# facebookresearch/MidasTouch

Measured on AMD Instinct MI355X. Metric: filter_steps_per_sec, higher is better.
Workload: dtype f64

## Files before the change

### include/midas_hip.h

```cpp
#ifndef MIDAS_HIP_H
#define MIDAS_HIP_H

#include <stdint.h>

#ifdef __cplusplus
extern "C" {
#endif

#define MIDAS_OK 0
#define MIDAS_ERR_INVALID (-1)
#define MIDAS_ERR_HIP (-2)
#define MIDAS_ERR_NOMEM (-3)
#define MIDAS_ERR_NODEVICE (-4)

#define MIDAS_F32 0
#define MIDAS_F64 1

#define MIDAS_RESAMPLE_MULTINOMIAL 0
#define MIDAS_RESAMPLE_SYSTEMATIC 1

typedef struct midas_ctx midas_ctx;
typedef struct midas_codebook midas_codebook;
typedef struct midas_tree midas_tree;

// ... 111 lines not shown
int midas_tsne_knn(midas_ctx* ctx, const void* X_dev, int32_t dtype, int64_t K, int64_t F, int64_t ld, int32_t nan_to_num,
                   int32_t k, int64_t rows_per_panel, int32_t* idx_dev, double* d2_dev);
int midas_tsne_perplexity(midas_ctx* ctx, const float* d2_dev, int64_t K, int32_t k, float perplexity, double* P_dev);
int midas_tsne_gradient(midas_ctx* ctx, int64_t K, const float* y_dev, const int64_t* crow_dev, const int32_t* col_dev,
                        const float* val_dev, float* grad_dev, double* kl_dev);
int midas_tsne_optimize(midas_ctx* ctx, int64_t K, float* y_dev, const int64_t* crow_dev, const int32_t* col_dev,
                        const float* val_dev, int32_t it, int32_t max_iter, double momentum, double learning_rate,
                        int32_t lr_float32, int32_t n_iter_check, int32_t n_iter_without_progress, double min_grad_norm,
                        double* result);

int midas_topn_pose_error(midas_ctx* ctx, int32_t B, int64_t K, const double* scores_dev, int64_t row0, int32_t n,
                          const double* feat_dev, int32_t d, double* err_dev, int32_t* idx_dev);

typedef struct midas_step_args {
    int64_t N;
    const float* poses_in_dev;
    float* poses_prop_dev;
    float* poses_out_dev;
    double* weights_dev;
    double* weights_out_dev;
    const int32_t* hint_in_dev;
    int32_t* nn_idx_dev;
    int32_t* hint_out_dev;
    int32_t* ridx_dev;
    const float* odom16_dev;
    const double* code_dev;
    const float* gt16_dev;
    double* rmse_dev;
    const float* tn_dev;
    const float* rot_dev;
    const double* u_dev;
    float u32;
    float std_t, std_r;
    uint64_t seed, step;
    double prune_thr;
    int32_t softmax;
    int32_t resample_mode;
    int32_t* status_dev;
    uint64_t* telemetry_dev;
    uint32_t* score_stamps_dev;
    uint32_t score_epoch;
} midas_step_args;

int midas_filter_step(midas_ctx* ctx, const midas_codebook* cb, const midas_tree* tree6,
                      const midas_tree* tree3, const midas_step_args* args);


typedef struct midas_lazy_args {
    int64_t N;
    const float* poses_prop_prev_dev;
    const int32_t* nn_idx_prev_dev;
    const int32_t* status_prev_dev;
    float* poses_prop_dev;
    int32_t* nn_idx_dev;
    uint8_t* valid_dev;
    int32_t* status_dev;
    double* tables_dev;
    double* scores_dev;
    double* part_rmse_dev;
    int32_t resample_prev;
    const float* poses_in_dev;
    const int32_t* hint_in_dev;
    int32_t resample_mode;
    const double* u_prev_dev;
    float u32_prev;
    uint64_t step_prev;
    int32_t* ridx_dev;
    const float* odom16_dev;
    const double* code_dev;
    const float* gt16_dev;
    const float* tn_dev;
    const float* rot_dev;
    float std_t, std_r;
    uint64_t seed, step;
    double prune_thr;
    int32_t softmax;
    uint64_t* telemetry_dev;
    uint32_t* score_stamps_dev;
    uint32_t score_epoch;
    double* rmse_dev;
    int32_t* score_list_dev;
    uint8_t* guide_dev;
} midas_lazy_args;
int64_t midas_lazy_guide_bytes(int64_t N);
int midas_lazy_guide_layout(int32_t* bins_out, int32_t* unit_out, int32_t* stride_out);
int midas_lazy_step(midas_ctx* ctx, const midas_codebook* cb, const midas_tree* tree6, const midas_tree* tree3,
                    const midas_lazy_args* args);
int midas_score_list_seed(midas_ctx* ctx, int64_t K, uint32_t* score_stamps_dev, uint32_t score_epoch, int32_t* score_list_dev,
                          int64_t N, const int32_t* nn_idx_dev);
int midas_lazy_run(midas_ctx* ctx, const midas_codebook* cb, const midas_tree* tree6, const midas_tree* tree3,
                   const midas_lazy_args* first, int32_t T, double* rmse_log_dev);

typedef struct midas_estimate_args {
    int64_t N;
    int32_t B;
    const float* poses_prop_dev;
    const double* weights_dev;
    const double* tables_dev;
    const uint8_t* valid_dev;
    int32_t softmax;
    float* centers_dev;
    float* stds_dev;
} midas_estimate_args;
int midas_pose_estimate(midas_ctx* ctx, const midas_estimate_args* args);
int midas_lazy_run_estimate(midas_ctx* ctx, const midas_codebook* cb, const midas_tree* tree6, const midas_tree* tree3,
                            const midas_lazy_args* first, int32_t T, double* rmse_log_dev,
                            float* est_centers_dev, float* est_stds_dev);

typedef struct midas_lazy_flush_args {
    int64_t N;
    const double* tables_dev;
    const uint8_t* valid_dev;
    const int32_t* nn_idx_dev;
    const float* poses_prop_dev;
    int32_t* status_dev;
    const double* part_rmse_dev;
    int32_t softmax, resample_mode;
    const double* u_dev;
    float u32;
    uint64_t seed, step;
    double* weights_dev;
    int32_t* ridx_dev;
    float* poses_out_dev;
    double* weights_out_dev;
    int32_t* hint_out_dev;
    double* rmse_dev;
} midas_lazy_flush_args;
int midas_lazy_flush(midas_ctx* ctx, const midas_lazy_flush_args* args);

int64_t midas_lazy_tables_doubles(int64_t N);
int midas_lazy_step_batch(midas_ctx* ctx, const midas_codebook* cb, const midas_tree* tree6, const midas_tree* tree3,
                          const midas_lazy_args* args, int32_t B);
int midas_lazy_flush_batch(midas_ctx* ctx, const midas_lazy_flush_args* args, int32_t B);


typedef struct midas_shard_front_args {
    int64_t N;
    int64_t slot_base;
    const float* poses_in_dev;
    float* poses_prop_dev;
    const int32_t* hint_in_dev;
    int32_t* nn_idx_dev;
    uint8_t* valid_dev;
    const float* odom16_dev;
    const double* code_dev;
    double* scores_dev;
    int32_t scores_ready;
    const float* gt16_dev;
    double* rmse_sums_dev;
    const float* tn_dev;
    const float* rot_dev;
    float std_t, std_r;
    uint64_t seed, step;
    double prune_thr;
    uint64_t* telemetry_dev;
    int32_t* status_dev;
    double* flags_dev;
    uint32_t* score_stamps_dev;
    uint32_t score_epoch;
} midas_shard_front_args;
int midas_shard_front(midas_ctx* ctx, const midas_codebook* cb, const midas_tree* tree6, const midas_tree* tree3,
                      const midas_shard_front_args* args);
int midas_shard_tail_a(midas_ctx* ctx, int64_t N, const double* scores_dev, const int32_t* nn_idx_dev,
                       const uint8_t* valid_dev, int32_t softmax, double* tables_dev, double* r1_dev, int32_t* status_dev);
typedef struct midas_shard_route_args {
    int64_t N;
// ... 222 lines not shown
```

### midastouch_amd/_lib.py

```python
from __future__ import annotations

import ctypes as C
import sys
import os
import subprocess

_HERE = os.path.dirname(os.path.abspath(__file__))
CSRC = os.path.join(_HERE, "csrc")
LIB_PATH = os.environ.get("MIDAS_HIP_LIB") or os.path.join(CSRC, "libmidas_hip.so")

MIDAS_F32, MIDAS_F64 = 0, 1
RESAMPLE_MULTINOMIAL, RESAMPLE_SYSTEMATIC = 0, 1
PROF_SLOTS = 8


class MidasError(RuntimeError):
    pass


class StepArgs(C.Structure):

    _fields_ = [
        ("N", C.c_int64),
        ("poses_in", C.c_void_p),
# ... 158 lines not shown
        ("unit_weights", C.c_int32), ("telemetry", C.c_void_p),
        ("score_stamps", C.c_void_p), ("score_epoch", C.c_uint32),
        ("host_mirror", C.c_void_p), ("grid_n", C.c_int64), ("anneal_small", C.c_int32), ("topk_ties", C.c_int32),
        ("anneal_frozen", C.c_int32), ("stream_draws", C.c_int32), ("dbscan_batched", C.c_int32),
    ]


LOOP_FRONT, LOOP_DBSCAN, LOOP_ANNEAL, LOOP_RESAMPLE = 1, 2, 4, 8
MT19937_HIST_WORDS = 20560
TOPK_TIES_INDEX, TOPK_TIES_ATEN_CPU = 0, 1
LOOP_MAX_CLUSTERS, LOOP_LOG_DOUBLES = 64, 168
LOOP_BATCH_MAX_CAP = 16384
LOOP_BATCH_WIDE_MAX_CAP = 131072
DBSCAN_BATCH_MAX_POINTS = 1 << 20
(LOOP_I_N, LOOP_I_NSET, LOOP_I_MODE, LOOP_I_K, LOOP_I_INIT, LOOP_I_VARSET, LOOP_I_KEPT, LOOP_I_DRIFT, LOOP_I_STATUS,
 LOOP_I_RAW, LOOP_I_NCL, LOOP_I_NPRES, LOOP_I_FRAME, LOOP_I_NAN, LOOP_I_ERR, LOOP_I_NDRAW) = range(16)
LOOP_ERR_NDRAW = 256
(LOOP_D_S, LOOP_D_VARPREV, LOOP_D_VAR, LOOP_D_RMSE_T, LOOP_D_RMSE_R, LOOP_D_XMAX, LOOP_D_XMIN, LOOP_D_TOTAL) = range(8)

_P, _I32, _I64, _U64, _F, _D = C.c_void_p, C.c_int32, C.c_int64, C.c_uint64, C.c_float, C.c_double
SIGNATURES = {
    "midas_ctx_create": (C.c_int, [C.c_int, _P, C.POINTER(_P)]),
    "midas_ctx_destroy": (C.c_int, [_P]),
    "midas_ctx_set_stream": (C.c_int, [_P, _P]),
    "midas_sync": (C.c_int, [_P]),
    "midas_selftest_wave_sums": (C.c_int, [_P, _P, _P]),
    "midas_scratch_reserve": (C.c_int, [_P, C.c_int64]),
    "midas_strerror": (C.c_char_p, [C.c_int]),
    "midas_last_error": (C.c_char_p, [_P]),
    "midas_version": (C.c_char_p, []),
    "midas_codebook_create": (C.c_int, [_P, _I64, _I32, _P, _I32, C.POINTER(_P)]),
    "midas_codebook_destroy": (C.c_int, [_P]),
    "midas_score": (C.c_int, [_P, _P, _I32, _P, _P]),
    "midas_score_batch": (C.c_int, [_P, _P, _I32, _P, _P]),
    "midas_score_batch_f64": (C.c_int, [_P, _P, _I32, _P, _P]),
    "midas_codebook_set_batch_precision": (C.c_int, [_P, _I32]),
    "midas_se3_feature": (C.c_int, [_P, _I64, _P, _F, _P]),
    "midas_tree_build": (C.c_int, [_P, _I32, _I64, _P, C.POINTER(_P)]),
    "midas_tree_destroy": (C.c_int, [_P]),
    "midas_tree_attach_mesh": (C.c_int, [_P, _P, _P, _P]),
    "midas_nn6": (C.c_int, [_P, _P, _I64, _P, _P, _P, _P]),
    "midas_knn6": (C.c_int, [_P, _P, _I64, _P, C.c_int32, _P, _P]),
    "midas_tree_export": (C.c_int, [_P, _P, C.c_int32, _P, _I64]),
    "midas_nn6_stats": (C.c_int, [_P, _P, _I64, _P, _P, _P, _P]),
    "midas_nn3": (C.c_int, [_P, _P, _I64, _P, _P]),
    "midas_propagate": (C.c_int, [_P, _I64, _P, _P, _P, _P, _P, _F, _F, _U64, _U64]),
    "midas_check_poses": (C.c_int, [_P, _I64, _P, _P, _P]),
    "midas_gather_f64": (C.c_int, [_P, _I64, _P, _P, _P]),
    "midas_softmax": (C.c_int, [_P, _I64, _P, _I32, _P]),
    "midas_prune": (C.c_int, [_P, _I64, _P, _P, _D, _P]),
    "midas_cdf": (C.c_int, [_P, _I64, _P, _P, _P]),
    "midas_score_list_seed": (C.c_int, [_P, _I64, _P, C.c_uint32, _P, _I64, _P]),
    "midas_mt19937_seed": (C.c_int, [_P, _U64, _P]),
    "midas_mt19937_rand64": (C.c_int, [_P, _P, _I64, _I64, _P]),
    "midas_mt19937_rand64_chunked": (C.c_int, [_P, _P, _I64, _I64, _P, _P, _P, _I32]),
    "midas_mt19937_normal32": (C.c_int, [_P, _P, _I64, _I64, _F, _F, _P, _P, _P, _P, _P, _P, _I32]),
    "midas_mt19937_draws": (C.c_int, [_P, _P, _I64, _I32, _P, _P, _P, _P, _P, _P, _I32]),
    "midas_mt19937_draws_batch": (C.c_int, [_P, _I32, _P, _I64, _I32, _P, _P, _P, _P, _P, _P, _I32]),
    "midas_mt19937_draws_counted": (C.c_int, [_P, _P, _I64, _I32, _P, _P, _P, _P, _P]),
    "midas_mt19937_draws_counted_batch": (C.c_int, [_P, _I32, _P, _I64, _I32, _P, _I64, _P, _P, _P, _P, _I64]),
    "midas_resample_search": (C.c_int, [_P, _I64, _P, _I64, _I32, _P, _F, _U64, _U64, _P]),
    "midas_gather_rows": (C.c_int, [_P, _I64, _P, _P, _P, _I32]),
    "midas_rmse": (C.c_int, [_P, _I64, _P, _P, _P]),
    "midas_topn_pose_error": (C.c_int, [_P, _I32, _I64, _P, _I64, _I32, _P, _I32, _P, _P]),
    "midas_selfsim_topn": (C.c_int, [_P, _P, _I32, _P, _I32, _I64, _P, _P]),
    "midas_selfsim_panel": (C.c_int, [_P, _P, _I64, _I64, _P, _I64]),
    "midas_selfsim_topn_f64": (C.c_int, [_P, _P, _I32, _P, _I32, _I64, _P, _P]),
    "midas_selfsim_panel_f64": (C.c_int, [_P, _P, _I64, _I64, _P, _I64]),
    "midas_tsne_knn": (C.c_int, [_P, _P, _I32, _I64, _I64, _I64, _I32, _I32, _I64, _P, _P]),
    "midas_tsne_perplexity": (C.c_int, [_P, _P, _I64, _I32, _F, _P]),
    "midas_tsne_gradient": (C.c_int, [_P, _I64, _P, _P, _P, _P, _P, _P]),
    "midas_tsne_optimize": (C.c_int, [_P, _I64, _P, _P, _P, _P, _I32, _I32, _D, _D, _I32, _I32, _I32, _D, _P]),
    "midas_cluster_centers": (C.c_int, [_P, _I64, _P, _P, _P, _P, _I32, _P, _P, _P, _P]),
    "midas_filter_step": (C.c_int, [_P, _P, _P, _P, C.POINTER(StepArgs)]),
    "midas_filter_step_batch": (C.c_int, [_P, _P, _P, _P, C.POINTER(StepArgs), _I32]),
    "midas_lazy_step": (C.c_int, [_P, _P, _P, _P, C.POINTER(LazyArgs)]),
    "midas_lazy_run": (C.c_int, [_P, _P, _P, _P, C.POINTER(LazyArgs), _I32, _P]),
    "midas_lazy_run_estimate": (C.c_int, [_P, _P, _P, _P, C.POINTER(LazyArgs), _I32, _P, _P, _P]),
    "midas_pose_estimate": (C.c_int, [_P, C.POINTER(EstimateArgs)]),
    "midas_lazy_flush": (C.c_int, [_P, C.POINTER(LazyFlushArgs)]),
    "midas_lazy_tables_doubles": (C.c_int64, [_I64]),
    "midas_lazy_guide_bytes": (C.c_int64, [_I64]),
    "midas_lazy_guide_layout": (C.c_int, [_P, _P, _P]),
    "midas_lazy_step_batch": (C.c_int, [_P, _P, _P, _P, C.POINTER(LazyArgs), _I32]),
    "midas_lazy_flush_batch": (C.c_int, [_P, C.POINTER(LazyFlushArgs), _I32]),
    "midas_loop_step": (C.c_int, [_P, _P, _P, _P, C.POINTER(LoopArgs), _I32]),
    "midas_loop_step_batch": (C.c_int, [_P, _P, _P, _P, C.POINTER(LoopArgs), _I32, _I32, _I64]),
    "midas_loop_step_batch_draws": (C.c_int, [_P, _P, _P, _P, C.POINTER(LoopArgs), _I32, _I32, _I64]),
    "midas_loop_step_batch_wide": (C.c_int, [_P, _P, _P, _P, C.POINTER(LoopArgs), _I32, _I32, _I64]),
    "midas_dbscan": (C.c_int, [_P, _I64, _P, _D, _I64, _P, _P]),
    "midas_dbscan_batch": (C.c_int, [_P, _I32, _I64, _P, _I64, _P, _D, _I64, _P, _P, _I32]),
    "midas_dbscan_points": (C.c_int, [_P, _I64, C.c_int32, _P, _D, _I64, _P, _P]),
    "midas_anneal_select": (C.c_int, [_P, _I64, _P, _I32, _I64, _P]),
    "midas_anneal_select_ties": (C.c_int, [_P, _I64, _P, _I32, _I64, _I32, _P, _P]),
    "midas_shard_front": (C.c_int, [_P, _P, _P, _P, C.POINTER(ShardFrontArgs)]),
    "midas_shard_tail_a": (C.c_int, [_P, _I64, _P, _P, _P, _I32, _P, _P, _P]),
    "midas_shard_tail_fin": (C.c_int, [_P, _I64, _P, _P, _P, _P, _I32, _P, _I32, _I64, _I32, _P, _P]),
    "midas_shard_route_count": (C.c_int, [_P, C.POINTER(ShardRouteArgs)]),
    "midas_shard_route_pack": (C.c_int, [_P, C.POINTER(ShardRouteArgs)]),
    "midas_shard_unpack": (C.c_int, [_P, _I64, _P, _P, _P, _P, _P]),
    "midas_shard_unpack_rows": (C.c_int, [_P, _I64, _P, _I32, _P, _P, _P, _P]),
    "midas_shard_unpack_fixed": (C.c_int, [_P, _I64, _P, _I64, _P, _I32, _I64, _P, _P, _P, _P, _P]),
    "midas_shard_unpack_peer": (C.c_int, [_P, _I64, _P, _P, _P, _P, _P]),
    "midas_comm_unique_id": (C.c_int, [_P, C.c_char_p, _P]),
    "midas_comm_create": (C.c_int, [_P, C.c_char_p, _P, _I32, _I32, C.POINTER(C.c_void_p)]),
    "midas_comm_destroy": (C.c_int, [_P]),
    "midas_comm_all_gather": (C.c_int, [_P, _P, _P, _I64]),
    "midas_shard_step": (C.c_int, [_P, _P, _P, _P, _P, C.POINTER(ShardStepArgs), _I32]),
    "midas_shard_run": (C.c_int, [_P, _P, _P, _P, _P, C.POINTER(ShardStepArgs), _I32]),
    "midas_shard_estimate_moments": (C.c_int, [_P, _I64, _P, _P, _P]),
    "midas_shard_estimate_finish": (C.c_int, [_P, _I64, _P, _P, _P]),
    "midas_shard_step_estimate": (C.c_int, [_P, _P, _P, _P, _P, C.POINTER(ShardStepArgs), _P, _P, _P, _P]),
    "midas_shard_run_estimate": (C.c_int, [_P, _P, _P, _P, _P, C.POINTER(ShardStepArgs), _I32, _P, _P, _P, _P]),
    "midas_peer_alloc": (C.c_int, [_P, _I64, C.POINTER(C.c_void_p), _P]),
    "midas_peer_free": (C.c_int, [_P, _P]),
    "midas_peer_open": (C.c_int, [_P, _P, C.POINTER(C.c_void_p)]),
    "midas_peer_close": (C.c_int, [_P, _P]),
    "midas_peer_probe_write": (C.c_int, [_P, _P, _I32, _I32, _I32]),
    "midas_peer_probe_check": (C.c_int, [_P, _P, _I32, _I32, _P]),
    "midas_tail_resample": (C.c_int, [_P, C.POINTER(TailResampleArgs)]),
    "midas_profile_enable": (C.c_int, [_P, _I32]),
    "midas_profile_read": (C.c_int, [_P, C.POINTER(C.c_double), C.POINTER(_I64), _I32]),
    "midas_profile_slot_name": (C.c_char_p, [_I32]),
}


def build(force: bool = False) -> str:
    srcs = [os.path.join(CSRC, f) for f in os.listdir(CSRC) if f.endswith((".hip", ".hpp"))]
    srcs.append(os.path.join(_HERE, "..", "include", "midas_hip.h"))
    stale = (not os.path.exists(LIB_PATH)) or any(os.path.getmtime(s) > os.path.getmtime(LIB_PATH) for s in srcs)
    if force or stale:
        subprocess.run(["make", "-C", CSRC, "-j4", "-s"] + (["-B"] if force else []), check=True)
    return LIB_PATH


_lib = None


def load():
    global _lib
    if _lib is not None:
        return _lib
    if not os.path.exists(LIB_PATH):
        raise MidasError(
            f"{LIB_PATH} not found: build it with `python -c 'import __graft_entry__ as g; g.build()'` "
            "(hipcc --offload-arch=gfx950). There is no CPU fallback."
        )
    import torch

    try:
        lib = C.CDLL(LIB_PATH)
    except OSError as e:
        raise MidasError(f"cannot load {LIB_PATH}: {e}") from e
    for name, (res, args) in SIGNATURES.items():
        try:
            fn = getattr(lib, name)
        except AttributeError as e:
            raise MidasError(f"{LIB_PATH} does not export {name}") from e
        fn.restype = res
        fn.argtypes = args
    _lib = lib
    return lib


def _ptr(t):
    if t is None:
# ... 79 lines not shown
```

### midastouch_amd/csrc/api.hip

```cpp
#include <cstdio>
#include <cstdlib>
#include <cstring>
#include <new>
#include <vector>

#include "api_entry.hpp"

using namespace midas;

namespace midas {
int tree_build_impl(midas_ctx* ctx, int32_t dim, int64_t K, const void* points_dev, midas_tree* out);
int attach_mesh_impl(midas_ctx* ctx, midas_tree* t6, const midas_tree* t3, const float* cb_poses_dev);
void tree_free_host(midas_tree* t);
}

struct ScratchChunk { void* p; size_t cap; };
struct ScratchState {
    std::vector<ScratchChunk> chunks;
    size_t cur = 0;
    size_t used = 0;
    size_t total = 0;
};
static ScratchState* scratch_of(midas_ctx* ctx) { return reinterpret_cast<ScratchState*>(ctx->scratch); }

// ... 27 lines not shown
    }
    *out = (char*)s->chunks[s->cur].p + s->used;
    s->used += bytes;
    return MIDAS_OK;
}

midas_scratch_pos midas_scratch_mark(midas_ctx* ctx) {
    const ScratchState* s = scratch_of(ctx);
    return {s->cur, s->used, s->total};
}

void midas_scratch_rewind(midas_ctx* ctx, const midas_scratch_pos& pos) {
    ScratchState* s = scratch_of(ctx);
    s->cur = pos.cur; s->used = pos.used; s->total = pos.total;
}

int midas_set_error(midas_ctx* ctx, int code, const char* what, const char* detail) {
    if (ctx) {
        ctx->last_error = std::string(midas_strerror(code)) + ": " + (what ? what : "") + " (" + (detail ? detail : "") + ")";
    }
    return code;
}

namespace midas {
void prof_mark(midas_ctx* ctx, int slot) {
    if (!ctx->prof || !ctx->ev_ready || slot > MIDAS_PROF_SLOTS) return;
    if (ctx->prof_only >= 0 && slot != ctx->prof_only && slot != ctx->prof_only + 1) return;
    (void)hipEventRecord(ctx->ev[slot], ctx->stream);
}
}

static const char* kSlotNames[MIDAS_PROF_SLOTS] = {
    "score_codebook", "particle_update", "tail_a", "tail_b", "", "", "", "event_pair_overhead"};

extern "C" {

MIDAS_EXPORT const char* midas_version(void) { return "midas-hip 0.1 (gfx950)"; }

MIDAS_EXPORT const char* midas_strerror(int code) {
    switch (code) {
        case MIDAS_OK: return "ok";
        case MIDAS_ERR_INVALID: return "invalid argument";
        case MIDAS_ERR_HIP: return "HIP runtime error";
        case MIDAS_ERR_NOMEM: return "out of device memory";
        case MIDAS_ERR_NODEVICE: return "no usable HIP device";
        default: return "unknown error";
    }
}

MIDAS_EXPORT const char* midas_last_error(const midas_ctx* ctx) { return ctx ? ctx->last_error.c_str() : ""; }

MIDAS_EXPORT int midas_ctx_create(int device, void* hip_stream, midas_ctx** out) {
    if (!out) return MIDAS_ERR_INVALID;
    *out = nullptr;
    int count = 0;
    if (hipGetDeviceCount(&count) != hipSuccess || count <= 0 || device < 0 || device >= count) return MIDAS_ERR_NODEVICE;
    if (hipSetDevice(device) != hipSuccess) return MIDAS_ERR_NODEVICE;
    midas_ctx* ctx = new (std::nothrow) midas_ctx();
    if (!ctx) return MIDAS_ERR_NOMEM;
    ctx->device = device;
    ctx->scratch = new (std::nothrow) ScratchState();
    ctx->stream = (hipStream_t)hip_stream;
    ctx->own_stream = false;
    if (const char* ov = getenv("MIDAS_OVERLAP")) ctx->overlap = atoi(ov) != 0;
    const char* lazy = getenv("MIDAS_LAZY_MODULES");
    if (!(lazy && lazy[0] == '1')) {
        int (*const warm[])() = {warm_score, warm_particles, warm_resample, warm_cluster, warm_topn, warm_selfsim, warm_loop,
                                 warm_dbscan, warm_dbscan_nd, warm_index_build, warm_mt19937, warm_topk_aten, warm_score_f64,
                                 warm_selfsim_f64, warm_tsne};
        for (auto w : warm)
            if (w() != 0) { (void)hipGetLastError(); }
    }
    {
        void* p = nullptr;
        const int blocks = midas::TAIL_GROUP_MAX_BLOCKS;
        if (hipMalloc(&p, (size_t)blocks * midas::TAIL_GROUP_BLOCK_BYTES) == hipSuccess && hipMemset(p, 0, (size_t)blocks * midas::TAIL_GROUP_BLOCK_BYTES) == hipSuccess &&
            hipDeviceSynchronize() == hipSuccess) {
            ctx->tail_rec = (unsigned long long*)p;
            ctx->tail_rec_blocks = blocks;
        } else {
            if (p) (void)hipFree(p);
            (void)hipGetLastError();
        }
    }
    *out = ctx;
    return MIDAS_OK;
}

MIDAS_EXPORT int midas_scratch_reserve(midas_ctx* ctx, int64_t bytes) {
    if (!ctx || bytes < 0) return MIDAS_ERR_INVALID;
    MIDAS_HIP_CHECK(ctx, hipSetDevice(ctx->device));
    ScratchState* s = scratch_of(ctx);
    size_t have = 0;
    for (const auto& c : s->chunks) have = c.cap > have ? c.cap : have;
    const size_t want = ((size_t)bytes + 255) & ~(size_t)255;
    if (s->chunks.size() == 1 && have >= want) return MIDAS_OK;
    if (s->chunks.size() >= 1 && have >= want && s->chunks[0].cap == have) return MIDAS_OK;
    MIDAS_HIP_CHECK(ctx, hipStreamSynchronize(ctx->stream));
    if (ctx->side) MIDAS_HIP_CHECK(ctx, hipStreamSynchronize(ctx->side));
    void* p = nullptr;
    const size_t cap = want > have ? want : have;
    if (hipMalloc(&p, cap) != hipSuccess) return midas_set_error(ctx, MIDAS_ERR_NOMEM, "hipMalloc(scratch reserve)", "out of device memory");
    for (auto& c : s->chunks) (void)hipFree(c.p);
    s->chunks.clear();
    s->chunks.push_back({p, cap});
    s->cur = 0; s->used = 0; s->total = 0;
    static const bool log = getenv("MIDAS_SCRATCH_LOG") != nullptr;
    if (log) fprintf(stderr, "[midas] scratch: reserved one chunk of %zu bytes\n", cap);
    return MIDAS_OK;
}

MIDAS_EXPORT int midas_ctx_destroy(midas_ctx* ctx) {
    if (!ctx) return MIDAS_OK;
    (void)hipSetDevice(ctx->device);
    (void)hipStreamSynchronize(ctx->stream);
    ScratchState* s = scratch_of(ctx);
    for (auto& c : s->chunks) (void)hipFree(c.p);
    delete s;
    if (ctx->tail_rec) (void)hipFree(ctx->tail_rec);
    if (ctx->ev_ready)
        for (auto& e : ctx->ev) (void)hipEventDestroy(e);
    if (ctx->own_stream) (void)hipStreamDestroy(ctx->stream);
    if (ctx->side) {
        (void)hipStreamSynchronize(ctx->side);
        (void)hipEventDestroy(ctx->ev_fork);
        (void)hipEventDestroy(ctx->ev_join);
        (void)hipStreamDestroy(ctx->side);
    }
    delete ctx;
    return MIDAS_OK;
}

MIDAS_EXPORT int midas_ctx_set_stream(midas_ctx* ctx, void* hip_stream) {
    if (!ctx) return MIDAS_ERR_INVALID;
    MIDAS_HIP_CHECK(ctx, hipStreamSynchronize(ctx->stream));
    if (ctx->own_stream) {
        (void)hipStreamDestroy(ctx->stream);
        ctx->own_stream = false;
    }
    ctx->stream = (hipStream_t)hip_stream;
    return MIDAS_OK;
}

MIDAS_EXPORT int midas_sync(midas_ctx* ctx) {
    if (!ctx) return MIDAS_ERR_INVALID;
    MIDAS_HIP_CHECK(ctx, hipStreamSynchronize(ctx->stream));
    return MIDAS_OK;
}

MIDAS_EXPORT int midas_codebook_create(midas_ctx* ctx, int64_t K, int32_t D, const void* emb_dev, int32_t dtype,
                                       midas_codebook** out) {
    MIDAS_ENTER(ctx);
    MIDAS_REQUIRE(ctx, out && emb_dev && K > 0 && D > 0 && (dtype == MIDAS_F32 || dtype == MIDAS_F64));
    midas_codebook* cb = new (std::nothrow) midas_codebook();
    if (!cb) return midas_set_error(ctx, MIDAS_ERR_NOMEM, "new midas_codebook", "");
    cb->ctx = ctx; cb->K = K; cb->D = D; cb->dtype = dtype; cb->emb = emb_dev; cb->norms = nullptr;
    if (hipMalloc((void**)&cb->norms, (size_t)K * sizeof(double)) != hipSuccess) {
        delete cb;
        return midas_set_error(ctx, MIDAS_ERR_NOMEM, "hipMalloc(norms)", "");
    }
    int rc = launch_row_norms(ctx, K, D, emb_dev, dtype, cb->norms);
    if (rc) { (void)hipFree(cb->norms); delete cb; return rc; }
    *out = cb;
    return MIDAS_OK;
}

MIDAS_EXPORT int midas_codebook_destroy(midas_codebook* cb) {
    if (!cb) return MIDAS_OK;
    (void)hipStreamSynchronize(cb->ctx->stream);
    (void)hipFree(cb->norms);
    delete cb;
    return MIDAS_OK;
}

MIDAS_EXPORT int midas_score(midas_ctx* ctx, const midas_codebook* cb, int32_t B, const double* codes_dev,
                             double* scores_dev) {
    MIDAS_ENTER(ctx);
    MIDAS_REQUIRE(ctx, cb && B >= 1 && codes_dev && scores_dev);
    return launch_score(ctx, cb, B, codes_dev, scores_dev);
}

MIDAS_EXPORT int midas_score_batch(midas_ctx* ctx, const midas_codebook* cb, int32_t B, const double* codes_dev,
                                   double* scores_dev) {
    MIDAS_ENTER(ctx);
    MIDAS_REQUIRE(ctx, cb && B >= 1 && codes_dev && scores_dev);
    return launch_score_batch(ctx, cb, B, codes_dev, scores_dev);
}

MIDAS_EXPORT int midas_score_batch_f64(midas_ctx* ctx, const midas_codebook* cb, int32_t B, const double* codes_dev,
                                       double* scores_dev) {
    MIDAS_ENTER(ctx);
    MIDAS_REQUIRE(ctx, cb && B >= 1 && codes_dev && scores_dev);
    return launch_score_batch_f64(ctx, cb, B, codes_dev, scores_dev);
}

MIDAS_EXPORT int midas_codebook_set_batch_precision(midas_codebook* cb, int32_t dtype) {
    if (!cb) return MIDAS_ERR_INVALID;
    midas_ctx* ctx = cb->ctx;
    MIDAS_REQUIRE(ctx, dtype == MIDAS_F32 || dtype == MIDAS_F64);
    cb->batch_precision = dtype;
    return MIDAS_OK;
}
// ... 349 lines not shown
```

### midastouch_amd/csrc/api_step.hip

```cpp
#include "api_entry.hpp"

using namespace midas;

static void prof_begin(midas_ctx* ctx) {
    if (!(ctx->prof && ctx->ev_ready)) return;
    (void)hipEventRecord(ctx->ev[6], ctx->stream);
    (void)hipEventRecord(ctx->ev[7], ctx->stream);
}
static int prof_end(midas_ctx* ctx, int lo, int hi, bool skip_slot0) {
    if (!(ctx->prof && ctx->ev_ready)) return MIDAS_OK;
    const int first = ctx->prof_only >= 0 ? ctx->prof_only : lo, last = ctx->prof_only >= 0 ? ctx->prof_only + 1 : hi;
    if (first >= lo && last <= hi) {
        MIDAS_HIP_CHECK(ctx, hipEventSynchronize(ctx->ev[last]));
        for (int i = first; i < last; ++i) {
            float ms = 0.f;
            if (i == 0 && skip_slot0) continue;
            MIDAS_HIP_CHECK(ctx, hipEventElapsedTime(&ms, ctx->ev[i], ctx->ev[i + 1]));
            ctx->prof_ms[i] += (double)ms;
        }
    } else {
        MIDAS_HIP_CHECK(ctx, hipEventSynchronize(ctx->ev[7]));
    }
    float cal = 0.f;
    MIDAS_HIP_CHECK(ctx, hipEventElapsedTime(&cal, ctx->ev[6], ctx->ev[7]));
    ctx->prof_ms[7] += (double)cal;
    ctx->prof_calls += 1;
    return MIDAS_OK;
}

extern "C" {

static int filter_step_impl(midas_ctx* ctx, const midas_codebook* cb, const midas_tree* tree6, const midas_tree* tree3,
                            const midas_step_args* args, int32_t B) {
    MIDAS_REQUIRE(ctx, cb && tree6 && tree3 && args && tree6->dim == 6 && tree3->dim == 3);
    const midas_step_args& s = *args;
    MIDAS_REQUIRE(ctx, s.N > 0 && s.poses_in_dev && s.poses_prop_dev && s.poses_out_dev && s.weights_dev &&
                           s.weights_out_dev && s.nn_idx_dev && s.hint_out_dev && s.ridx_dev && s.odom16_dev &&
                           s.code_dev && s.status_dev);
    MIDAS_REQUIRE(ctx, s.poses_prop_dev != s.poses_in_dev && s.poses_prop_dev != s.poses_out_dev);
    MIDAS_REQUIRE(ctx, (s.tn_dev == nullptr) == (s.rot_dev == nullptr));
    MIDAS_REQUIRE(ctx, tree6->K == cb->K);
    const int64_t N = s.N;
    const int npart = particle_update_blocks(N);
    void *scores, *x, *e, *valid, *pmax, *pmin, *prm = nullptr, *cdf;
    int rc;
    const size_t Bz = (size_t)B;
    if ((rc = midas_scratch(ctx, Bz * cb->K * sizeof(double), &scores))) return rc;
    if ((rc = midas_scratch(ctx, Bz * N * sizeof(double), &x))) return rc;
    if ((rc = midas_scratch(ctx, Bz * N * sizeof(double), &e))) return rc;
    if ((rc = midas_scratch(ctx, Bz * N, &valid))) return rc;
    if ((rc = midas_scratch(ctx, Bz * npart * sizeof(double), &pmax))) return rc;
    if ((rc = midas_scratch(ctx, Bz * npart * sizeof(double), &pmin))) return rc;
    if (s.gt16_dev && s.rmse_dev)
        if ((rc = midas_scratch(ctx, Bz * npart * 2 * sizeof(double), &prm))) return rc;
    if ((rc = midas_scratch(ctx, Bz * N * sizeof(double), &cdf))) return rc;
    void* lp_raw = nullptr;
    const bool mfma = B > 1 && (cb->batch_precision == MIDAS_F64 ||
                                (cb->dtype == MIDAS_F32 && cb->D % 16 == 0 && (uintptr_t)cb->emb % 16 == 0));
    const bool defer_batch = mfma && ctx->overlap;
    if ((B == 1 && ctx->overlap) || defer_batch || (B > 1 && s.score_stamps_dev))
        if ((rc = midas_scratch(ctx, Bz * N * sizeof(double), &lp_raw))) return rc;
    if (defer_batch && !ctx->side) {
        MIDAS_HIP_CHECK(ctx, hipStreamCreateWithFlags(&ctx->side, hipStreamNonBlocking));
        MIDAS_HIP_CHECK(ctx, hipEventCreateWithFlags(&ctx->ev_fork, hipEventDisableTiming));
        MIDAS_HIP_CHECK(ctx, hipEventCreateWithFlags(&ctx->ev_join, hipEventDisableTiming));
    }

    prof_begin(ctx);
    ParticleUpdateArgs pa;
    fill_particle_update(pa, s, tree6, tree3, N, s.poses_in_dev, s.hint_in_dev, (uint8_t*)valid, B == 1 ? s.score_stamps_dev : nullptr,
                         prm ? s.gt16_dev : nullptr, (double*)prm);
    pa.batch = B;
    pa.score_stride = cb->K;
    pa.scores = (const double*)scores;
    pa.x = (double*)x;
    pa.e = (double*)e;
    pa.status_reset = s.status_dev;
    pa.part_max = (double*)pmax;
    pa.part_min = (double*)pmin;
    bool defer = false;
    const bool sparse_batch = B > 1 && s.score_stamps_dev && s.score_epoch && sparse_score_ok(cb, s.code_dev);
    if (sparse_batch) {
        pa.sp.stamps = s.score_stamps_dev; pa.sp.epoch = s.score_epoch;
        pa.sp.emb = (const float*)cb->emb; pa.sp.norms = cb->norms; pa.sp.code = s.code_dev; pa.sp.scores = (double*)scores;
        pa.sp.nj = cb->D / 64;
        pa.scores = nullptr;
        prof_mark(ctx, 1);
        if ((rc = launch_particle_update(ctx, tree6, tree3, pa))) return rc;
        defer = true;
    }
    if (B == 1 && ctx->overlap) {
        prof_mark(ctx, 1);
        if ((rc = launch_frame_front(ctx, tree6, tree3, pa, cb, s.code_dev, (double*)scores, &defer))) return rc;
    }
    if (defer_batch && !sparse_batch) {
        hipStream_t main_stream = ctx->stream;
        MIDAS_HIP_CHECK(ctx, hipEventRecord(ctx->ev_fork, main_stream));
        MIDAS_HIP_CHECK(ctx, hipStreamWaitEvent(ctx->side, ctx->ev_fork, 0));
        ctx->stream = ctx->side;
        rc = launch_score_dense_batch(ctx, cb, B, s.code_dev, (double*)scores);
        ctx->stream = main_stream;
        if (rc) return rc;
        MIDAS_HIP_CHECK(ctx, hipEventRecord(ctx->ev_join, ctx->side));
        prof_mark(ctx, 1);
        pa.scores = nullptr;
        if ((rc = launch_particle_update(ctx, tree6, tree3, pa))) return rc;
        MIDAS_HIP_CHECK(ctx, hipStreamWaitEvent(main_stream, ctx->ev_join, 0));
        defer = true;
    } else if (!defer) {
        prof_mark(ctx, 0);
        if ((rc = mfma ? launch_score_dense_batch(ctx, cb, B, s.code_dev, (double*)scores)
                       : launch_score(ctx, cb, B, s.code_dev, (double*)scores)))
            return rc;
        prof_mark(ctx, 1);
        pa.sp.stamps = nullptr;
        if ((rc = launch_particle_update(ctx, tree6, tree3, pa))) return rc;
    }
    prof_mark(ctx, 2);

    StepTailArgs ta;
    fill_step_tail(ta, s);
    ta.batch = B;
    ta.npart = npart;
    ta.x = defer ? nullptr : (const double*)x;
    ta.scores = (const double*)scores;
    ta.score_stride = cb->K;
    ta.x_raw = (double*)x;
    ta.lp_raw = (double*)lp_raw;
    ta.e = (double*)e;
    ta.valid = (const uint8_t*)valid;
    ta.part_max = (const double*)pmax;
    ta.part_min = (const double*)pmin;
    ta.cdf = (double*)cdf;
    ta.part_rmse = (const double*)prm;
    if ((rc = launch_step_tail(ctx, ta, 2))) return rc;
    return prof_end(ctx, 0, 4, defer);
}

MIDAS_EXPORT int midas_filter_step(midas_ctx* ctx, const midas_codebook* cb, const midas_tree* tree6,
                                   const midas_tree* tree3, const midas_step_args* args) {
    MIDAS_ENTER(ctx);
    return filter_step_impl(ctx, cb, tree6, tree3, args, 1);
}

MIDAS_EXPORT int midas_filter_step_batch(midas_ctx* ctx, const midas_codebook* cb, const midas_tree* tree6,
                                         const midas_tree* tree3, const midas_step_args* args, int32_t B) {
    MIDAS_ENTER(ctx);
    MIDAS_REQUIRE(ctx, B >= 1 && B <= 65535);
    return filter_step_impl(ctx, cb, tree6, tree3, args, B);
}

static int lazy_step_impl(midas_ctx* ctx, const midas_codebook* cb, const midas_tree* tree6, const midas_tree* tree3,
                          const midas_lazy_args& s, double* rmse_out, int32_t B = 1, int64_t tstride = 0) {
    MIDAS_REQUIRE(ctx, s.N > 0 && ceil_div(s.N, SCAN_BLOCK) <= LAZY_MAX_BLOCKS && s.poses_prop_dev && s.nn_idx_dev && s.valid_dev &&
                           s.status_dev && s.tables_dev && (uintptr_t)s.tables_dev % 128 == 0 && s.scores_dev && s.odom16_dev && s.code_dev);
    MIDAS_REQUIRE(ctx, s.resample_prev ? (s.poses_prop_prev_dev && s.nn_idx_prev_dev && s.status_prev_dev &&
                                          s.poses_prop_prev_dev != s.poses_prop_dev && s.nn_idx_prev_dev != s.nn_idx_dev &&
                                          s.status_prev_dev != s.status_dev)
                                       : (s.poses_in_dev && s.poses_in_dev != s.poses_prop_dev));
    MIDAS_REQUIRE(ctx, (s.tn_dev == nullptr) == (s.rot_dev == nullptr));
    MIDAS_REQUIRE(ctx, s.resample_mode == MIDAS_RESAMPLE_MULTINOMIAL || s.resample_mode == MIDAS_RESAMPLE_SYSTEMATIC);
    const int64_t N = s.N;
    TailTables tb = tables_of(s.tables_dev, N);
    if (s.guide_dev && B == 1) {
        MIDAS_REQUIRE(ctx, (uintptr_t)s.guide_dev % 16 == 0);
        tb.guide = reinterpret_cast<guide_t*>(s.guide_dev);
        tb.guide_raw = tb.guide + ceil_div(N, SCAN_BLOCK) * GUIDE_STRIDE;
    }
    ParticleUpdateArgs pa;
    fill_particle_update(pa, s, tree6, tree3, N, s.poses_in_dev, s.hint_in_dev, s.valid_dev, s.score_stamps_dev,
                         (s.gt16_dev && s.part_rmse_dev) ? s.gt16_dev : nullptr, s.part_rmse_dev);
    pa.batch = B;
    pa.score_stride = cb->K;
    pa.scores = nullptr;
    pa.status_reset = s.status_dev;
    ScorePredict predict;
    if (pa.sp.stamps && s.score_list_dev && B == 1 && s.score_epoch >= 2 && N >= SCAN_CHUNK) {
        MIDAS_REQUIRE(ctx, s.score_epoch < MIDAS_EPOCH_LIMIT);
        predict = wire_score_list(pa.sp, s.score_list_dev, cb->K);
    }
    if (s.resample_prev) {
        LazyResample& r = pa.rs;
        r.enabled = true;
        r.e = tb.e; r.x_raw = tb.x_raw; r.lp = tb.lp; r.lp_raw = tb.lp_raw; r.gend = tb.gend; r.gend_raw = tb.gend_raw;
        r.ggend = tb.ggend; r.ggend_raw = tb.ggend_raw;
        r.guide = tb.guide; r.guide_raw = tb.guide_raw;
        r.bsum_e = tb.bsum_e; r.btot = tb.btot; r.btot_raw = tb.btot_raw; r.bmax = tb.bmax; r.bmin = tb.bmin;
        r.poses_prev = s.poses_prop_prev_dev; r.nn_prev = s.nn_idx_prev_dev; r.status_prev = s.status_prev_dev;
        r.ridx_out = s.ridx_dev;
        r.nb = (int)ceil_div(N, SCAN_BLOCK); r.ng = (int)ceil_div(N, SCAN_CHUNK);
        r.softmax = s.softmax; r.mode = s.resample_mode; r.u = s.u_prev_dev; r.u32 = s.u32_prev;
        r.seed = s.seed; r.step = s.step_prev;
        r.tstride = tstride;
    }
    prof_begin(ctx);
    prof_mark(ctx, 1);
    bool launched = false;
    int rc;
    if (B > 1 && !s.resample_prev) {
        MIDAS_REQUIRE(ctx, pa.sp.stamps && sparse_score_ok(cb, s.code_dev));
        pa.sp.emb = (const float*)cb->emb; pa.sp.norms = cb->norms; pa.sp.code = s.code_dev; pa.sp.scores = s.scores_dev; pa.sp.nj = cb->D / 64;
        if ((rc = launch_particle_update(ctx, tree6, tree3, pa))) return rc;
    } else {
        if ((rc = launch_frame_front(ctx, tree6, tree3, pa, cb, s.code_dev, s.scores_dev, &launched))) return rc;
        if (!launched)
            return midas_set_error(ctx, MIDAS_ERR_INVALID, "codebook", B > 1 ? "the pipelined batch step needs a float32 codebook with D in {128,256,512,1024}, score stamps and N <= 262144"
                                                                              : "the pipelined step needs a float32 codebook with D in {128,256,512,1024}");
    }
    prof_mark(ctx, 2);
    if ((rc = launch_tail_a2(ctx, N, s.scores_dev, s.nn_idx_dev, s.valid_dev, s.softmax, tb, s.status_dev, B, cb->K, true,
                             pa.gt16 ? s.part_rmse_dev : nullptr, rmse_out, B > 1 ? tstride : 0, predict.stamps ? &predict : nullptr)))
        return rc;
    prof_mark(ctx, 3);
    return prof_end(ctx, 1, 3, false);
}

MIDAS_EXPORT int midas_lazy_step(midas_ctx* ctx, const midas_codebook* cb, const midas_tree* tree6, const midas_tree* tree3,
                                 const midas_lazy_args* args) {
    MIDAS_ENTER(ctx);
    MIDAS_REQUIRE(ctx, cb && tree6 && tree3 && args && tree6->dim == 6 && tree3->dim == 3 && tree6->K == cb->K);
    return lazy_step_impl(ctx, cb, tree6, tree3, *args, (args->gt16_dev && args->part_rmse_dev) ? args->rmse_dev : nullptr);
}

static int pose_estimate_impl(midas_ctx* ctx, const midas_estimate_args& s) {
    MIDAS_REQUIRE(ctx, s.N > 0 && s.B >= 1 && s.B <= 65535 && s.poses_prop_dev && s.centers_dev && s.stds_dev &&
                           (uintptr_t)s.poses_prop_dev % 16 == 0);
    MIDAS_REQUIRE(ctx, (s.weights_dev == nullptr) != (s.tables_dev == nullptr));
    if (s.weights_dev)
        return launch_pose_estimate(ctx, s.N, s.B, s.poses_prop_dev, s.weights_dev, nullptr, 0, nullptr, s.softmax, s.centers_dev,
                                    s.stds_dev);
    MIDAS_REQUIRE(ctx, s.valid_dev && (uintptr_t)s.tables_dev % 128 == 0 && ceil_div(s.N, SCAN_BLOCK) <= LAZY_MAX_BLOCKS);
    const TailTables tb = tables_of(const_cast<double*>(s.tables_dev), s.N);
    return launch_pose_estimate(ctx, s.N, s.B, s.poses_prop_dev, nullptr, &tb, tables_doubles(s.N), s.valid_dev, s.softmax,
                                s.centers_dev, s.stds_dev);
}

MIDAS_EXPORT int midas_pose_estimate(midas_ctx* ctx, const midas_estimate_args* args) {
    MIDAS_ENTER(ctx);
    MIDAS_REQUIRE(ctx, args != nullptr);
    return pose_estimate_impl(ctx, *args);
}

static int lazy_run_impl(midas_ctx* ctx, const midas_codebook* cb, const midas_tree* tree6, const midas_tree* tree3,
                         const midas_lazy_args* first, int32_t T, double* rmse_log_dev, float* est_centers, float* est_stds) {
    MIDAS_REQUIRE(ctx, cb && tree6 && tree3 && first && tree6->dim == 6 && tree3->dim == 3 && tree6->K == cb->K && T >= 1);
    MIDAS_REQUIRE(ctx, first->poses_prop_prev_dev && first->nn_idx_prev_dev && first->status_prev_dev && !first->tn_dev &&
                           !first->rot_dev && !first->u_prev_dev);
    MIDAS_REQUIRE(ctx, !rmse_log_dev || (first->gt16_dev && first->part_rmse_dev));
    midas_lazy_args a = *first;
    if (a.score_stamps_dev) {
        const uint64_t inc = a.score_list_dev ? 2u : 1u;
        MIDAS_REQUIRE(ctx, (uint64_t)a.score_epoch + inc * (uint64_t)(T - 1) < (a.score_list_dev ? (uint64_t)MIDAS_EPOCH_LIMIT : 0xFFFFFFF0ull));
    }
    for (int32_t f = 0; f < T; ++f) {
        int rc = f ? scratch_reset(ctx) : MIDAS_OK;
        if (rc) return rc;
        rc = lazy_step_impl(ctx, cb, tree6, tree3, a, rmse_log_dev ? rmse_log_dev + 3 * f : nullptr);
        if (rc) return rc;
        if (est_centers) {
            midas_estimate_args e;
            e.N = a.N; e.B = 1; e.poses_prop_dev = a.poses_prop_dev; e.weights_dev = nullptr; e.tables_dev = a.tables_dev;
            e.valid_dev = a.valid_dev; e.softmax = a.softmax;
            e.centers_dev = est_centers + 16 * (size_t)f; e.stds_dev = est_stds + 3 * (size_t)f;
            if ((rc = pose_estimate_impl(ctx, e))) return rc;
        }
        float* pp = const_cast<float*>(a.poses_prop_prev_dev);
        int32_t* np = const_cast<int32_t*>(a.nn_idx_prev_dev);
        int32_t* sp = const_cast<int32_t*>(a.status_prev_dev);
        a.poses_prop_prev_dev = a.poses_prop_dev; a.nn_idx_prev_dev = a.nn_idx_dev; a.status_prev_dev = a.status_dev;
        a.poses_prop_dev = pp; a.nn_idx_dev = np; a.status_dev = sp;
        a.resample_prev = 1;
        a.u32_prev = -1.0f;
        a.step_prev = a.step;
        a.step += 1;
        if (a.score_stamps_dev) {
            a.score_epoch += a.score_list_dev ? 2u : 1u;
        }
        a.odom16_dev += 16;
        a.code_dev += cb->D;
        if (a.gt16_dev) a.gt16_dev += 16;
    }
    return MIDAS_OK;
}

MIDAS_EXPORT int midas_lazy_run(midas_ctx* ctx, const midas_codebook* cb, const midas_tree* tree6, const midas_tree* tree3,
                                const midas_lazy_args* first, int32_t T, double* rmse_log_dev) {
    MIDAS_ENTER(ctx);
    return lazy_run_impl(ctx, cb, tree6, tree3, first, T, rmse_log_dev, nullptr, nullptr);
}

MIDAS_EXPORT int midas_lazy_run_estimate(midas_ctx* ctx, const midas_codebook* cb, const midas_tree* tree6, const midas_tree* tree3,
                                         const midas_lazy_args* first, int32_t T, double* rmse_log_dev, float* est_centers_dev,
                                         float* est_stds_dev) {
    MIDAS_ENTER(ctx);
    MIDAS_REQUIRE(ctx, est_centers_dev && est_stds_dev);
    return lazy_run_impl(ctx, cb, tree6, tree3, first, T, rmse_log_dev, est_centers_dev, est_stds_dev);
}

static int lazy_flush_impl(midas_ctx* ctx, const midas_lazy_flush_args& s, int32_t B, int64_t tstride) {
    MIDAS_REQUIRE(ctx, s.N > 0 && s.tables_dev && s.valid_dev && s.nn_idx_dev && s.poses_prop_dev && s.status_dev && s.weights_dev &&
                           s.ridx_dev && s.poses_out_dev && s.weights_out_dev && s.hint_out_dev && s.poses_out_dev != s.poses_prop_dev);
    MIDAS_REQUIRE(ctx, s.resample_mode == MIDAS_RESAMPLE_MULTINOMIAL || s.resample_mode == MIDAS_RESAMPLE_SYSTEMATIC);
    const TailTables tb = tables_of(const_cast<double*>(s.tables_dev), s.N);
    StepTailArgs ta;
    fill_step_tail(ta, s);
    ta.batch = B;
    ta.tstride = B > 1 ? tstride : 0;
    ta.npart = 0;
    ta.x = nullptr; ta.e = nullptr; ta.cdf = nullptr; ta.part_max = nullptr; ta.part_min = nullptr;
    ta.valid = s.valid_dev;
    ta.part_rmse = (s.part_rmse_dev && s.rmse_dev) ? s.part_rmse_dev : nullptr;
    return launch_tail_b2(ctx, ta, tb);
}

MIDAS_EXPORT int midas_lazy_flush(midas_ctx* ctx, const midas_lazy_flush_args* args) {
    MIDAS_ENTER(ctx);
    MIDAS_REQUIRE(ctx, args != nullptr);
    return lazy_flush_impl(ctx, *args, 1, 0);
}

MIDAS_EXPORT int midas_score_list_seed(midas_ctx* ctx, int64_t K, uint32_t* score_stamps_dev, uint32_t score_epoch, int32_t* score_list_dev,
                                       int64_t N, const int32_t* nn_idx_dev) {
    MIDAS_ENTER(ctx);
    MIDAS_REQUIRE(ctx, K > 0 && score_stamps_dev && score_epoch >= 2 && score_epoch < MIDAS_EPOCH_LIMIT && score_list_dev && N > 0 && nn_idx_dev);
    return launch_predict_seed(ctx, N, nn_idx_dev, next_score_list(score_stamps_dev, score_epoch, score_list_dev, K));
}

MIDAS_EXPORT int64_t midas_lazy_tables_doubles(int64_t N) { return N > 0 ? tables_doubles(N) : 0; }
MIDAS_EXPORT int midas_lazy_guide_layout(int32_t* bins_out, int32_t* unit_out, int32_t* stride_out) {
    if (bins_out) *bins_out = GUIDE_BINS;
    if (unit_out) *unit_out = GUIDE_UNIT;
    if (stride_out) *stride_out = GUIDE_STRIDE;
    return MIDAS_OK;
}
MIDAS_EXPORT int64_t midas_lazy_guide_bytes(int64_t N) { return N > 0 ? 2 * ceil_div(N, SCAN_BLOCK) * (int64_t)GUIDE_STRIDE * (int64_t)sizeof(guide_t) : 0; }

MIDAS_EXPORT int midas_lazy_step_batch(midas_ctx* ctx, const midas_codebook* cb, const midas_tree* tree6, const midas_tree* tree3,
                                       const midas_lazy_args* args, int32_t B) {
    MIDAS_ENTER(ctx);
    MIDAS_REQUIRE(ctx, cb && tree6 && tree3 && args && tree6->dim == 6 && tree3->dim == 3 && tree6->K == cb->K && B >= 1);
    MIDAS_REQUIRE(ctx, args->score_stamps_dev && args->score_epoch && ceil_div(args->N, SCAN_BLOCK) <= 64 && args->N >= SCAN_CHUNK);
    return lazy_step_impl(ctx, cb, tree6, tree3, *args, (args->gt16_dev && args->part_rmse_dev) ? args->rmse_dev : nullptr, B,
                          tables_doubles(args->N));
}

MIDAS_EXPORT int midas_lazy_flush_batch(midas_ctx* ctx, const midas_lazy_flush_args* args, int32_t B) {
    MIDAS_ENTER(ctx);
    MIDAS_REQUIRE(ctx, args != nullptr && B >= 1);
    return lazy_flush_impl(ctx, *args, B, tables_doubles(args->N));
}

}
```

### midastouch_amd/csrc/front.hip

```cpp
#include "front_wave.hpp"

namespace midas {

template <bool STATS>
__global__ __launch_bounds__(64) void k_particle_update(TreeView<Kd6> t6, TreeView<Kd3> t3, ParticleUpdateArgs a) {
    __shared__ double s_cd[KD_MAX_LEVELS * 64];
    particle_update_wave<false, false, false, STATS, false, true>(t6, t3, a, blockIdx.x, gridDim.x, blockIdx.y, s_cd);
}

int launch_particle_update(midas_ctx* ctx, const midas_tree* t6, const midas_tree* t3, const ParticleUpdateArgs& a_in) {
    if (a_in.N == 0) return MIDAS_OK;
    ParticleUpdateArgs a = a_in;
    static const int ablate = getenv("MIDAS_ABLATE") ? atoi(getenv("MIDAS_ABLATE")) : 0;
    a.ablate = ablate;
    const dim3 grid((unsigned)particle_update_blocks(a.N), (unsigned)(a.batch > 1 ? a.batch : 1));
    if (ablate) hipLaunchKernelGGL(k_particle_update<true>, grid, dim3(64), 0, ctx->stream, view_of<Kd6>(t6), view_of<Kd3>(t3), a);
    else hipLaunchKernelGGL(k_particle_update<false>, grid, dim3(64), 0, ctx->stream, view_of<Kd6>(t6), view_of<Kd3>(t3), a);
    MIDAS_HIP_CHECK(ctx, hipGetLastError());
    return MIDAS_OK;
}


MD void particle_front_wave(ParticleUpdateArgs a, int64_t wave, const double* rs_lds, PuFeat* __restrict__ feat) {
    const int lane = threadIdx.x & 63;
// ... 188 lines not shown
        hits |= dpp_u32<DPP_XOR1>(hits); stops |= dpp_u32<DPP_XOR1>(stops);
        if (LPP == 4) { hits |= dpp_u32<DPP_XOR2>(hits); stops |= dpp_u32<DPP_XOR2>(stops); }
        if (live && mv < 0 && (hits | stops)) {
            const int fh = hits ? __builtin_ctz(hits) : 32, fs = stops ? __builtin_ctz(stops) : 32;
            mv = fh < fs ? 1 : 0;
        }
        mesh_coop(a.vlist, nn, q3, a.t2, lim, owner && live && mv < 0, mv);
    }
    double bestd = a.t2;
    int64_t vi = 0;
    const bool fb3 = owner && live && mv < 0;
    bool ok = wave_search<Kd3, true>(t3, q3, bestd, vi, fb3, s_cd[w]);
    if (a.telemetry) {
        const unsigned long long m = __ballot(fb3);
        if (lane == 0 && m) atomicAdd(&a.telemetry[1], (unsigned long long)__popcll(m));
    }
    if (mv >= 0) ok = mv == 1;
    if (owner && live) {
        a.nn_idx[p] = nn;
        a.valid[p] = ok ? 1 : 0;
    }
}

template <int LPP>
__global__ __launch_bounds__(256, MIDAS_NNP_OCC) void k_particle_nn_prune(TreeView<Kd6> t6, TreeView<Kd3> t3, ParticleUpdateArgs a,
                                                                          const PuFeat* __restrict__ feat) {
    particle_nn_prune_wg<LPP>(t6, t3, a, feat);
}

__global__ __launch_bounds__(256, MIDAS_NNP_OCC) void k_front_small(TreeView<Kd6> t6, TreeView<Kd3> t3, ParticleUpdateArgs a, int nwaves,
                                                                    PuFeat* __restrict__ feat) {
    if (blockIdx.y) {
        const int64_t b = blockIdx.y, o = b * a.N;
        a.n_live += b * LOOP_CTL_I;
        a.poses_in += o * 16; a.poses_prop += o * 16; a.odom16 += b * 16;
        if (a.hint_in) a.hint_in += o;
        a.nn_idx += o; a.valid += o;
        if (a.gt16) { a.gt16 += b * 16; a.part_rmse += 2 * b * nwaves; }
        a.sp.stamps += b * a.score_stride; a.sp.scores += b * a.score_stride; a.sp.code += b * (int64_t)(a.sp.nj * 64);
        a.seed += (uint64_t)b;
        if (a.tn) { a.tn += o * 3; a.rot += o * 3; }
        feat += o;
    }
    if (threadIdx.x < 64 && (int)blockIdx.x < nwaves) particle_front_wave(a, (int64_t)blockIdx.x, nullptr, feat);
    __syncthreads();
    particle_nn_prune_wg<4>(t6, t3, a, feat);
}

template <int NJ, bool LAZY>
static void launch_front_a(const FrontLaunch& L, PuFeat* feat) {
    hipLaunchKernelGGL((k_frame_front_a<float, NJ, LAZY>), L.grid, dim3(256), 0, L.ctx->stream, L.a, L.n_pu, L.nwaves, feat,
                       (const float*)L.cb->emb, L.cb->norms, L.code, L.scores, L.cb->K);
}

bool launch_front_plain(const FrontLaunch& L, const FrontForm& f) {
    return launch_if_form<0, 1, true, true>(L, f) || launch_if_form<0, 1, true, false>(L, f) || launch_if_form<0, 4, true, false>(L, f) ||
           launch_if_form<0, 1, true, false, true>(L, f);
}

int launch_frame_front(midas_ctx* ctx, const midas_tree* t6, const midas_tree* t3, const ParticleUpdateArgs& a_in,
                       const midas_codebook* cb, const double* code, double* scores, bool* launched) {
    *launched = false;
    if (a_in.N == 0 || cb->dtype != MIDAS_F32) return MIDAS_OK;
    if (a_in.batch > 1 && !(a_in.rs.enabled && a_in.rs.nb <= LAZY_WAVE_LD && a_in.sp.stamps)) return MIDAS_OK;
    if ((uintptr_t)cb->emb % 16 != 0 || (uintptr_t)code % 16 != 0) return MIDAS_OK;
    if (cb->D != 512 && cb->D != 256 && cb->D != 128 && cb->D != 1024) return MIDAS_OK;
    ParticleUpdateArgs a = a_in;
    static const int ablate = getenv("MIDAS_ABLATE") ? atoi(getenv("MIDAS_ABLATE")) : 0;
    a.ablate = ablate;
    a.scores = nullptr;
    const int nwaves = particle_update_blocks(a.N), n_pu = (nwaves + 3) / 4;
    if (a.sp.stamps) {
        a.sp.emb = (const float*)cb->emb; a.sp.norms = cb->norms; a.sp.code = code; a.sp.scores = scores; a.sp.nj = cb->D / 64;
    }
    static const int list_wgs_env = getenv("MIDAS_LIST_WAVES") ? atoi(getenv("MIDAS_LIST_WAVES")) : 1024;
    const bool use_list = a.sp.stamps && a.sp.list && a.batch <= 1 && list_wgs_env > 0;
    const char* dense_env = getenv("MIDAS_DENSE_ROWS");
    a.sp.K = cb->K;
    a.sp.dense_thr = use_list && dense_env ? atoi(dense_env) : 0;
    const unsigned grid = (unsigned)(n_pu + (a.sp.stamps ? 0 : ceil_div(cb->K, 16)));
    static const int split_env = getenv("MIDAS_SPLIT_FRONT") ? atoi(getenv("MIDAS_SPLIT_FRONT")) : 1;
    const bool split_front = a.batch <= 1 && !a.inbox.rows && (split_env >= 2 || (split_env == 1 && ((a.rs.enabled && a.N <= 512) || (!a.rs.enabled && a.N <= 2048) || (a.n_live && a.N <= 16384))));
    const int lpp = split_env == 3 ? 2 : 4;
    if (split_front && !(a.ablate & 7)) {
        a.sp.pred_tag = 0; a.sp.list = nullptr;
        void* feat;
        int rc = midas_scratch(ctx, (size_t)a.N * sizeof(PuFeat), &feat);
        if (rc) return rc;
        static const bool small_env = !(getenv("MIDAS_FRONT_SMALL") && atoi(getenv("MIDAS_FRONT_SMALL")) == 0);
        if (small_env && !a.rs.enabled && a.sp.stamps && lpp == 4) {
            hipLaunchKernelGGL(k_front_small, dim3((unsigned)ceil_div(a.N, 64)), dim3(256), 0, ctx->stream, view_of<Kd6>(t6), view_of<Kd3>(t3),
                               a, nwaves, (PuFeat*)feat);
        } else {
            const FrontLaunch L{ctx, t6, t3, a, cb, code, scores, dim3(grid), n_pu, nwaves};
            with_nj(cb->D, [&](auto nj) {
                if (a.rs.enabled) launch_front_a<decltype(nj)::value, true>(L, (PuFeat*)feat);
                else launch_front_a<decltype(nj)::value, false>(L, (PuFeat*)feat);
            });
            if (lpp == 4)
                hipLaunchKernelGGL(k_particle_nn_prune<4>, dim3((unsigned)ceil_div(a.N, 64)), dim3(256), 0, ctx->stream,
                                   view_of<Kd6>(t6), view_of<Kd3>(t3), a, (const PuFeat*)feat);
            else
                hipLaunchKernelGGL(k_particle_nn_prune<2>, dim3((unsigned)ceil_div(a.N, 128)), dim3(256), 0, ctx->stream,
                                   view_of<Kd6>(t6), view_of<Kd3>(t3), a, (const PuFeat*)feat);
        }
        MIDAS_HIP_CHECK(ctx, hipGetLastError());
        *launched = true;
        return MIDAS_OK;
    }
    static const int fw_env = getenv("MIDAS_FRONT_WAVES") ? atoi(getenv("MIDAS_FRONT_WAVES")) : 0;
    static const int wt_env = getenv("MIDAS_WAVE_TABLES") ? atoi(getenv("MIDAS_WAVE_TABLES")) : 1;
    const bool wave_tables = a.rs.enabled && a.rs.nb <= LAZY_WAVE_LD && wt_env != 0;
    const int fw = a.batch > 1 ? 1 : (a.rs.enabled && !wave_tables) ? 4 : fw_env == 1 || fw_env == 4 ? fw_env : (a.sp.stamps ? 1 : 4);
    const int n_pu_fw = (nwaves + fw - 1) / fw;
    if (!use_list) { a.sp.pred_tag = 0; a.sp.list = nullptr; }
    static const int presort_env = getenv("MIDAS_PRESORT") ? atoi(getenv("MIDAS_PRESORT")) : 1;
    if (wave_tables && fw == 1 && a.batch > 1 && !a.inbox.rows && !a.ablate && !a.n_live && presort_env != 0) {
        const int rc = launch_presort(ctx, a);
        if (rc) return rc;
    }
    const unsigned grid_fw = (unsigned)(n_pu_fw + (a.sp.stamps ? (use_list ? (list_wgs_env + fw - 1) / fw : 0) : ceil_div(cb->K, 4 * fw * MIDAS_SCORE_ROUNDS)));
    static const bool pref_env = !(getenv("MIDAS_PREF_PLAIN") && getenv("MIDAS_PREF_PLAIN")[0] == '0');
    const bool pref_plain = pref_env && !a.inbox.rows;
    const bool small_set = fw == 1 && a.N <= 131072;
    FrontForm form;
    if (a.batch > 1) form = {2, 1, false, false, false};
    else if (!a.rs.enabled) form = {0, fw, true, small_set && pref_plain, false};
    else if (!wave_tables) form = {1, 4, true, false, false};
    else form = {2, fw, true, small_set, false};
    if (a.ablate && cb->D == 512 && fw == 1 && (a.batch > 1 || !a.rs.enabled || form.pref)) {
        form.stats = true;
        if (!a.rs.enabled) form.pref = false;
    }
    const FrontLaunch L{ctx, t6, t3, a, cb, code, scores, dim3(grid_fw, (unsigned)(a.batch > 1 ? a.batch : 1)), n_pu_fw, nwaves};
    if (!(launch_front_batch(L, form) || launch_front_plain(L, form) || launch_front_folded(L, form)))
        return midas_set_error(ctx, MIDAS_ERR_INVALID, "launch_frame_front", "no kernel for this form of the front");
    MIDAS_HIP_CHECK(ctx, hipGetLastError());
    *launched = true;
    return MIDAS_OK;
}

int launch_front_small_batch(midas_ctx* ctx, const midas_tree* t6, const midas_tree* t3, const ParticleUpdateArgs& a_in,
                             const midas_codebook* cb, const double* code, double* scores, int32_t B, bool wide) {
    ParticleUpdateArgs a = a_in;
    if (!(a.n_live && a.N > 0 && (a.N <= 16384 || (wide && a.N <= MIDAS_LOOP_BATCH_WIDE_MAX_CAP)) && a.sp.stamps && !a.rs.enabled && cb->dtype == MIDAS_F32 &&
          (cb->D == 512 || cb->D == 256 || cb->D == 128 || cb->D == 1024) && (uintptr_t)cb->emb % 16 == 0 && (uintptr_t)code % 16 == 0))
        return midas_set_error(ctx, MIDAS_ERR_INVALID, "launch_front_small_batch", "no small-set front for these arguments");
    a.scores = nullptr;
    a.sp.emb = (const float*)cb->emb; a.sp.norms = cb->norms; a.sp.code = code; a.sp.scores = scores; a.sp.nj = cb->D / 64;
    a.sp.K = cb->K; a.sp.pred_tag = 0; a.sp.list = nullptr;
    a.score_stride = cb->K;
    a.batch = B;
    const int nwaves = particle_update_blocks(a.N);
    void* feat;
    const int rc = midas_scratch(ctx, (size_t)B * a.N * sizeof(PuFeat), &feat);
    if (rc) return rc;
    hipLaunchKernelGGL(k_front_small, dim3((unsigned)ceil_div(a.N, 64), (unsigned)B), dim3(256), 0, ctx->stream, view_of<Kd6>(t6),
                       view_of<Kd3>(t3), a, nwaves, (PuFeat*)feat);
    MIDAS_HIP_CHECK(ctx, hipGetLastError());
    return MIDAS_OK;
}

__global__ __launch_bounds__(256) void k_reduce_partials(int np, const double* __restrict__ pmax,
                                                         const double* __restrict__ pmin, const double* __restrict__ prm,
                                                         double* __restrict__ extrema2, double* __restrict__ rmse_sums2) {
    __shared__ double s0[4], s1[4], s2[4], s3[4];
    double a = -INFINITY, b = INFINITY, p = 0.0, q = 0.0;
    bool nan = false;
    for (int i = threadIdx.x; i < np; i += 256) {
        if (pmax) {
            double u = pmax[i], v = pmin[i];
            nan |= (u != u) || (v != v);
            a = u > a ? u : a;
            b = v < b ? v : b;
        }
        if (prm) { p += prm[2 * i]; q += prm[2 * i + 1]; }
    }
    a = wave_max(a);
    b = wave_min(b);
    p = wave_sum(p);
    q = wave_sum(q);
    const bool wnan = __any(nan);
    if ((threadIdx.x & 63) == 0) {
        const int w = threadIdx.x >> 6;
        s0[w] = wnan ? NAN : a; s1[w] = wnan ? NAN : b; s2[w] = p; s3[w] = q;
    }
    __syncthreads();
    if (threadIdx.x == 0) {
        bool bad = false;
        for (int i = 0; i < 4; ++i) {
            bad |= s0[i] != s0[i];
            a = s0[i] > a ? s0[i] : a;
            b = s1[i] < b ? s1[i] : b;
        }
        if (extrema2) {
            extrema2[0] = bad ? NAN : a;
            extrema2[1] = bad ? NAN : b;
        }
        if (rmse_sums2) {
            rmse_sums2[0] = (s2[0] + s2[1]) + (s2[2] + s2[3]);
            rmse_sums2[1] = (s3[0] + s3[1]) + (s3[2] + s3[3]);
        }
    }
}

int launch_reduce_partials(midas_ctx* ctx, int np, const double* pmax, const double* pmin, const double* prm,
                           double* extrema2, double* rmse_sums2) {
    hipLaunchKernelGGL(k_reduce_partials, dim3(1), dim3(256), 0, ctx->stream, np, pmax, pmin, prm, extrema2, rmse_sums2);
    MIDAS_HIP_CHECK(ctx, hipGetLastError());
    return MIDAS_OK;
}

// ... 4 lines not shown
```

### midastouch_amd/csrc/front_folded.hip

```cpp
#define MIDAS_FRONT_CLOCKS
#include "front_wave.hpp"

namespace midas {

bool launch_front_folded(const FrontLaunch& L, const FrontForm& f) {
    return launch_if_form<1, 4, true, false>(L, f) || launch_if_form<2, 1, true, true>(L, f) || launch_if_form<2, 1, true, false>(L, f) ||
           launch_if_form<2, 4, true, false>(L, f) || launch_if_form<2, 1, true, true, true>(L, f);
}

#if defined(MIDAS_DEBUG_CLOCKS)
int debug_ff_clocks(long long* io8192, int reset) {
    if (reset) {
        static long long zero[16384];
        return hipMemcpyToSymbol(HIP_SYMBOL(g_ff_clk), zero, sizeof(zero)) == hipSuccess ? 0 : 1;
    }
    return hipMemcpyFromSymbol(io8192, HIP_SYMBOL(g_ff_clk), 16384 * sizeof(long long)) == hipSuccess ? 0 : 1;
}
#endif
MIDAS_WARM_TU(front_folded, (k_frame_front<float, 8, 2, 1, true, true>))

}
```

### midastouch_amd/csrc/front_wave.hpp

```cpp
#pragma once
#include <type_traits>

#include "midas_internal.hpp"
#include "midas_math.hpp"
#include "score_body.hpp"
#include "peer_row.hpp"
#include "resample_search.hpp"
#include "list_scan.hpp"
#include "pose.hpp"

namespace midas {

#ifndef MIDAS_SCORE_ROUNDS
#define MIDAS_SCORE_ROUNDS 2
#endif
#ifndef MIDAS_CLAIM_HASH
#define MIDAS_CLAIM_HASH 1
#endif

constexpr int LAZY_WG_W = 3 * LAZY_MAX_BLOCKS + 8, LAZY_WG_LDS = 4 * LAZY_MAX_BLOCKS + 8;
MD void lazy_tables(const LazyResample& rs, double* rs_lds) {
    __shared__ double s_ex[12];
    const int t = threadIdx.x;
    const int b = t < rs.nb ? t : rs.nb - 1;
    const double bt = rs.btot[b], btr = rs.btot_raw[b], bs = rs.bsum_e[b], bx = rs.bmax[b], bn = rs.bmin[b];
    const int32_t status = rs.status_prev[0];
    const bool in = t < rs.nb;
    double mx = in ? bx : -INFINITY, mn = in ? bn : INFINITY;
    const bool nan = in && ((bx != bx) || (bn != bn));
    mx = wave_max_dpp(mx);
    mn = wave_min_dpp(mn);
    const bool wn = __any(nan);
    if ((t & 63) == 0) { s_ex[t >> 6] = mx; s_ex[4 + (t >> 6)] = mn; s_ex[8 + (t >> 6)] = wn ? 1.0 : 0.0; }
    __syncthreads();
    mx = s_ex[0]; mn = s_ex[4];
    double f = s_ex[8];
    for (int w = 1; w < 4; ++w) { mx = s_ex[w] > mx ? s_ex[w] : mx; mn = s_ex[4 + w] < mn ? s_ex[4 + w] : mn; f += s_ex[8 + w]; }
    if (f != 0.0) { mx = NAN; mn = NAN; }
    const bool apply = rs.softmax && !(__builtin_fabs(mx - mn) <= ISCLOSE_ATOL);
    double* s_bp = rs_lds;
    double* s_w = rs_lds + 256;
    double* s_se = rs_lds + 516;
    if (in) { s_w[t] = apply ? bt : btr; s_se[t] = bs; }
    __syncthreads();
    if (t == 0) {
        double acc = 0.0, S = 0.0;
        for (int i = 0; i < rs.nb; ++i) { s_bp[i] = acc; acc = acc + s_w[i]; S = S + s_se[i]; }
        rs_lds[512] = acc;
        rs_lds[513] = apply ? S : 1.0;
        rs_lds[514] = apply ? 1.0 : 0.0;
        rs_lds[515] = status != 0 ? 1.0 : 0.0;
    }
    __syncthreads();
    const double total = rs_lds[512];
    const double wb = in ? s_w[t] : 0.0;
    __syncthreads();
    if (in) rs_lds[LAZY_WG_W + t] = wb;
    if (in) s_w[t] = (t == rs.nb - 1) ? 1.0 : (s_bp[t] + wb) / total;
    __syncthreads();
}

constexpr int LAZY_WAVE_LD = 64, LAZY_WAVE_LDS = 3 * LAZY_WAVE_LD + 4;
struct LazyRecords { double bt, btr, bx, bn; int32_t status; };
MD LazyRecords lazy_records_load(const LazyResample& rs) {
    const int lane = threadIdx.x & 63;
    const int b = lane < rs.nb ? lane : rs.nb - 1;
    LazyRecords r;
    r.bt = rs.btot[b]; r.btr = rs.btot_raw[b]; r.bx = rs.bmax[b]; r.bn = rs.bmin[b];
    r.status = rs.status_prev[0];
    return r;
}
MD void lazy_tables_wave(const LazyResample& rs, const LazyRecords& r, double* rs_lds) {
    const int lane = threadIdx.x & 63;
    const bool in = lane < rs.nb;
    double mx = in ? r.bx : -INFINITY, mn = in ? r.bn : INFINITY;
    const bool nan = in && ((r.bx != r.bx) || (r.bn != r.bn));
    mx = wave_max_dpp(mx);
    mn = wave_min_dpp(mn);
    if (__any(nan)) { mx = NAN; mn = NAN; }
    const bool apply = rs.softmax && !(__builtin_fabs(mx - mn) <= ISCLOSE_ATOL);
    const double w = in ? (apply ? r.bt : r.btr) : 0.0;
    double* s_wb = rs_lds + 2 * LAZY_WAVE_LD + 4;
    s_wb[lane] = w;
    __builtin_amdgcn_fence(__ATOMIC_RELEASE, "wavefront");
    __builtin_amdgcn_wave_barrier();
    __builtin_amdgcn_fence(__ATOMIC_ACQUIRE, "wavefront");
    double acc = 0.0, bp = 0.0;
    for (int i0 = 0; i0 < rs.nb; i0 += 8) {
        double wv[8];
        const double2* p2 = reinterpret_cast<const double2*>(s_wb + i0);
#pragma unroll
        for (int j = 0; j < 4; ++j) { const double2 t = p2[j]; wv[2 * j] = t.x; wv[2 * j + 1] = t.y; }
#pragma unroll
        for (int j = 0; j < 8; ++j) {
            bp = lane == i0 + j ? acc : bp;
            acc = acc + wv[j];
        }
    }
    const double total = acc;
    if (in) {
        rs_lds[lane] = bp;
        rs_lds[LAZY_WAVE_LD + lane] = (lane == rs.nb - 1) ? 1.0 : (bp + w) / total;
    }
    if (lane == 0) {
        rs_lds[2 * LAZY_WAVE_LD] = total;
        rs_lds[2 * LAZY_WAVE_LD + 2] = apply ? 1.0 : 0.0;
        rs_lds[2 * LAZY_WAVE_LD + 3] = r.status != 0 ? 1.0 : 0.0;
    }
    __builtin_amdgcn_fence(__ATOMIC_RELEASE, "wavefront");
    __builtin_amdgcn_wave_barrier();
    __builtin_amdgcn_fence(__ATOMIC_ACQUIRE, "wavefront");
}

template <typename GT = const double*, typename LT = const double*, typename MID = NoMid>
MD int64_t lazy_source(const LazyResample& rs, const double* rs_lds, int64_t n, int64_t N, int ld = 256, GT gend_lds = nullptr,
                       LT lp_lds = nullptr, MID mid = MID()) {
    const double* s_bp = rs_lds;
    const double* s_end = rs_lds + ld;
    const double total = rs_lds[2 * ld];
    const bool apply = rs_lds[2 * ld + 2] != 0.0;
    const bool bad_total = !(total == total) || total == 0.0;
    if (rs_lds[2 * ld + 3] != 0.0 || bad_total) return n;
    const double* __restrict__ lp = apply ? rs.lp : rs.lp_raw;
    const double* __restrict__ gend = apply ? rs.gend : rs.gend_raw;
    double tq;
    bool upper;
    if (rs.mode == MIDAS_RESAMPLE_MULTINOMIAL) {
        tq = rs.u ? rs.u[n] : philox_uniform53((uint64_t)(n + rs.key_base), rs.seed, rs.step);
        upper = false;
    } else {
        const float r = rs.u32 >= 0.0f ? rs.u32 : philox_uniform24(rs.seed + (uint64_t)rs.traj, rs.step);
        const float off = r / (float)N;
        tq = (double)n / (double)N + (double)off;
        tq = tq >= 1.0 ? tq - 1.0 : tq;
        upper = true;
    }
    auto left_exact = [&](double c) { return upper ? (c <= tq) : (c < tq); };
    int lo = 0, hi = rs.nb;
    while (hi > lo) {
        const int mid = lo + ((hi - lo) >> 1);
        if (left_exact(s_end[mid])) lo = mid + 1; else hi = mid;
    }
    if (lo >= rs.nb) return N - 1;
    if constexpr (__is_same(LT, lds_cdp)) {
        return search_in_block_t<lds_cdp, GT>(lp_lds, gend, apply ? rs.ggend : rs.ggend_raw, lo, N, N - 1, s_bp[lo], total, tq, upper, gend_lds);
    } else {
        const guide_t* guide = apply ? rs.guide : rs.guide_raw;
        return search_in_block_t<const double*, GT, MID>(lp, gend, apply ? rs.ggend : rs.ggend_raw, lo, N, N - 1, s_bp[lo], total, tq, upper, gend_lds,
                                                         guide, guide ? rs_lds[(ld == LAZY_WAVE_LD ? 2 * LAZY_WAVE_LD + 4 : LAZY_WG_W) + lo] : 0.0, mid);
    }
}

template <bool WT = false, bool SCREEN = false, bool PREF = false, bool STATS = false, bool PRES = false, bool NANPART = false>
MD void particle_update_wave(const TreeView<Kd6>& t6, const TreeView<Kd3>& t3, ParticleUpdateArgs a, int64_t wave,
                             int nwaves, int traj, double* s_cd, double* rs_lds = nullptr) {
    const int lane = threadIdx.x & 63;
    if (a.n_live) {
        const int64_t nl = *a.n_live;
        a.N = nl < a.N ? nl : a.N;
        if (wave * 64 >= a.N && wave != 0) return;
    }
    if (traj) {
        const int64_t b = traj, o = b * a.N;
        a.poses_in += o * 16; a.poses_prop += o * 16; a.odom16 += b * 16;
        if (a.tn) { a.tn += o * 3; a.rot += o * 3; }
        if (a.hint_in) a.hint_in += o;
        a.nn_idx += o; a.valid += o;
        if (a.scores) { a.scores += b * a.score_stride; a.x += o; a.e += o; a.part_max += b * nwaves; a.part_min += b * nwaves; }
        if (a.gt16) { a.gt16 += b * 16; a.part_rmse += 2 * b * nwaves; }
        if (a.status_reset) a.status_reset += 2 * b;
        if (a.sp.stamps) {
            a.sp.stamps += b * a.score_stride; a.sp.scores += b * a.score_stride; a.sp.code += b * (int64_t)(a.sp.nj * 64);
        }
        a.slot_base += o;
        if (a.rs.enabled) {
            const int64_t ts = b * a.rs.tstride;
            a.rs.e += ts; a.rs.x_raw += ts; a.rs.lp += ts; a.rs.lp_raw += ts; a.rs.gend += ts; a.rs.gend_raw += ts;
            a.rs.ggend += ts; a.rs.ggend_raw += ts; a.rs.bsum_e += ts; a.rs.btot += ts; a.rs.btot_raw += ts; a.rs.bmax += ts; a.rs.bmin += ts;
            a.rs.poses_prev += o * 16; a.rs.nn_prev += o; a.rs.status_prev += 2 * b;
            if (a.rs.ridx_out) a.rs.ridx_out += o;
            if (a.rs.u) a.rs.u += o;
            a.rs.key_base = o;
            a.rs.traj = traj;
        }
        if (a.pre_order) { a.pre_order += o; a.pre_src += o; if (a.pre_rmse_terms) a.pre_rmse_terms += 2 * o; }
    }
    const bool presorted = PRES && a.pre_order != nullptr;
    const int64_t rank = wave * 64 + lane;
    const bool live = rank < a.N;
    int64_t n = rank;
    int32_t src_pre = 0;
    if (presorted) {
        n = a.pre_order[live ? rank : 0];
        src_pre = a.pre_src[live ? rank : 0];
    }
    if (wave == 0 && lane == 0) {
        if (a.status_reset) { a.status_reset[0] = 0; a.status_reset[1] = 0; }
        if (a.flags_reset) { a.flags_reset[0] = 0.0; a.flags_reset[1] = 0.0; }
        if (a.sp.next_count) *a.sp.next_count = 0;
    }
    unsigned long long st_nn = 0, st_mesh = 0, st_scan = 0;
    int st_rows = 0;
    const bool dense_scores = scores_dense(a.sp);
    const int ablate = STATS ? a.ablate : 0;
    long long tc[10];
    long long tp[4] = {0, 0, 0, 0};
#define MIDAS_TICK(i) do { if (STATS) tc[i] = clock64(); } while (0)
#define MIDAS_PTICK(i) do { if (STATS) tp[i] = clock64(); } while (0)
    MIDAS_TICK(0);
    const long long wall0 = STATS ? wall_clock64() : 0;
    double x = 0.0, et2 = 0.0, ang2 = 0.0;
    float R[16], f[6] = {0.f, 0.f, 0.f, 0.f, 0.f, 0.f};
#pragma unroll
    for (int i = 0; i < 16; ++i) R[i] = 0.f;
    int64_t src = n;
    float NO[16];
    if (WT) {
        float O[16];
#pragma unroll
        for (int i = 0; i < 16; ++i) O[i] = a.odom16[i];
        __builtin_amdgcn_sched_barrier(0);
        LazyRecords rec;
        if (!presorted) rec = lazy_records_load(a.rs);
        __builtin_amdgcn_sched_barrier(0);
        float tnv[3] = {0.f, 0.f, 0.f}, rotv[3] = {0.f, 0.f, 0.f};
        bool no_done = false;
        if (live) noise_draws(n, n + a.slot_base, a.tn, a.rot, a.std_t, a.std_r, a.seed, a.step, tnv, rotv);
        if (!presorted) lazy_tables_wave(a.rs, rec, rs_lds);
        MIDAS_PTICK(0);
        auto mid = [&]() { noise_apply(O, tnv, rotv, NO); no_done = true; };
        if (rs_lds && live && !presorted && !(ablate & 8)) {
            src = lazy_source(a.rs, rs_lds, n, a.N, LAZY_WAVE_LD, (const double*)nullptr, (const double*)nullptr, mid);
            if (a.rs.ridx_out) a.rs.ridx_out[n] = (int32_t)src;
        }
        if (live && !no_done) mid();
        MIDAS_PTICK(1);
    }
    if (rs_lds && live) {
        if (presorted) {
            src = src_pre;
        } else if (!WT) {
            src = (ablate & 8) ? n : lazy_source(a.rs, rs_lds, n, a.N, 256);
            if (a.rs.ridx_out) a.rs.ridx_out[n] = (int32_t)src;
        }
    }
    const float* pose_src = rs_lds ? a.rs.poses_prev : a.poses_in;
    const bool from_inbox = !WT && a.inbox.rows != nullptr;
    PeerRow row;
    if (from_inbox && live) row = peer_row_load(a.inbox.rows, n);
    const int32_t hint = !live ? -1 : from_inbox ? (int32_t)(row.head[1] & 0xFFFFFFFFull) : rs_lds ? a.rs.nn_prev[src] : a.hint_in ? a.hint_in[n] : -1;
    if (live) {
        float P[16];
        if (from_inbox) {
#pragma unroll
            for (int k = 0; k < 8; ++k) {
                P[2 * k] = __int_as_float((int)(row.pose[k] & 0xFFFFFFFFull));
                P[2 * k + 1] = __int_as_float((int)(row.pose[k] >> 32));
            }
        } else {
            load_pose(pose_src + src * 16, P);
        }
        if (WT) {
            mat4_mul(P, NO, R);
            MIDAS_PTICK(2);
        } else {
            float O[16];
#pragma unroll
            for (int i = 0; i < 16; ++i) O[i] = a.odom16[i];
            propagate_one(n, n + a.slot_base, P, O, a.tn, a.rot, a.std_t, a.std_r, a.seed, a.step, R);
        }
        store_pose(a.poses_prop + n * 16, R);
        se3_feature(R, 0.99f, 0.01f, f);
    }
    const float tq_f[3] = {R[3], R[7], R[11]};
    const FieldProbe probe = field_fetch(a.field, tq_f, live && !(ablate & 2));
    MIDAS_TICK(1);
    int32_t bi = 0;
    float bd;
    if (ablate & 1) {
        bi = hint < 0 ? 0 : hint;
    } else {
        int nscan = 0;
        const bool fb = nn6_wave<false, SCREEN>(t6, f, live, hint, bi, bd, reinterpret_cast<float*>(s_cd), nullptr, nullptr, STATS ? &nscan : nullptr,
                                                STATS ? &tc[2] : nullptr);
        MIDAS_TICK(3);
        if (a.telemetry && (ablate & 4)) {
            st_nn = __ballot(live && nscan >= NN_SOLO - 1);
            st_scan = (unsigned long long)wave_sum((double)nscan);
        }
        if (a.telemetry) {
            const unsigned long long m = __ballot(fb);
            if (lane == 0 && m) atomicAdd(&a.telemetry[0], (unsigned long long)__popcll(m));
        }
    }
    constexpr bool PRE = PREF;
    int mv = live ? field_decide(a.field, probe, a.thr) : -1;
    const bool lists_needed = __ballot(live && mv < 0) != 0;
    MeshScr pre[PRE ? 1 + MESH_BATCH : 1];
    if (PRE && a.vscr != nullptr && lists_needed) {
        const MeshScr* vs = a.vscr + (size_t)(live ? bi : 0) * MESH_REC;
#pragma unroll
        for (int j = 0; j < (PRE ? 1 + MESH_BATCH : 1); ++j) pre[j] = vs[j];
    }
    RowClaim claim{false, 0u};
    if (a.sp.stamps && !(ablate & 16)) {
        claim = claim_rows_issue(a.sp, live, bi, MIDAS_CLAIM_HASH ? reinterpret_cast<int*>(s_cd) : nullptr);
        st_rows = score_claimed_rows_nj(a.sp, claim, bi, dense_scores);
    }
    MIDAS_TICK(9);
    double q3[3] = {(double)R[3], (double)R[7], (double)R[11]};
    double best = a.t2;
    int64_t vi = 0;
    if (ablate & 2) mv = 1;
    else if (a.vlist && lists_needed) {
        double lim_lane = 0.0;
        const bool open = live && mv < 0;
        if (a.vscr) {
            const float tqf[3] = {R[3], R[7], R[11]};
// ... 5 lines not shown
            mv = mesh_list_check<false>(a.vlist, bi, q3, a.t2, a.thr, MESH_SOLO, &lim_lane);
        }
        MIDAS_TICK(4);
        if (a.telemetry && (ablate & 4)) st_mesh = __ballot(live && mv < 0);
        mesh_coop(a.vlist, bi, q3, a.t2, lim_lane, live && mv < 0, mv);
    }
    MIDAS_TICK(5);
    bool ok = wave_search<Kd3, true>(t3, q3, best, vi, live && mv < 0, s_cd);
    if (a.telemetry) {
        const unsigned long long m = __ballot(live && mv < 0);
        if (lane == 0 && m) atomicAdd(&a.telemetry[1], (unsigned long long)__popcll(m));
    }
    if (mv >= 0) ok = mv == 1;
    if (a.telemetry && st_rows && lane == 0) atomicAdd(&a.telemetry[2], (unsigned long long)st_rows);
    MIDAS_TICK(6);
    if (live) {
        a.nn_idx[n] = bi;
        if (a.scores) {
            x = a.scores[bi];
            a.x[n] = x;
            a.e[n] = exp_spec(x - 1.0);
        }
        a.valid[n] = ok ? 1 : 0;
        if (a.gt16) {
            float G[16];
#pragma unroll
            for (int i = 0; i < 16; ++i) G[i] = a.gt16[i];
            rmse_terms(R, G, et2, ang2);
        }
    }
    MIDAS_TICK(7);
    const double NEG = -INFINITY, POS = INFINITY;
    if (a.scores) {
        double mx = wave_max(live ? x : NEG), mn = wave_min(live ? x : POS);
        if (NANPART && __any(live && x != x)) { mx = NAN; mn = NAN; }
        if (lane == 0) { a.part_max[wave] = mx; a.part_min[wave] = mn; }
    }
    if (a.gt16) {
        if (presorted && a.pre_rmse_terms) {
            if (live) reinterpret_cast<double2*>(a.pre_rmse_terms)[n] = make_double2(et2, ang2);
        } else {
            et2 = wave_sum(et2);
            ang2 = wave_sum(ang2);
            if (lane == 0) { a.part_rmse[2 * wave] = et2; a.part_rmse[2 * wave + 1] = ang2; }
        }
    }
    if (STATS && a.telemetry && (ablate & 4) && lane == 0) {
        tc[8] = clock64();
        unsigned long long* w = a.telemetry + 16 + 16 * ((size_t)traj * nwaves + wave);
        w[0] += (unsigned long long)st_rows;
        w[1] = (unsigned long long)wall0;
        w[2] += (unsigned long long)__popcll(st_nn); w[4] += st_nn ? 1 : 0;
        w[3] += (unsigned long long)__popcll(st_mesh); w[5] += st_mesh ? 1 : 0;
        w[6] += st_scan;
        w[7] += (unsigned long long)(wall_clock64() - wall0);
#pragma unroll
        for (int i = 0; i < 8; ++i) {
            long long d = i == 3 ? tc[9] - tc[3] : i == 4 ? tc[5] - tc[9] : tc[i + 1] - tc[i];
            if ((ablate & 128) && i >= 4) d = !tp[0] ? 0 : i == 4 ? tp[0] - tc[0] : i == 5 ? tp[1] - tp[0] : i == 6 ? tp[2] - tp[1] : tc[1] - tp[2];
            w[8 + i] += (unsigned long long)d;
        }
    }
#undef MIDAS_TICK
#undef MIDAS_PTICK
}

#ifndef MIDAS_FRONT_OCC
#define MIDAS_FRONT_OCC 1
#endif
#ifndef MIDAS_FRONT4_OCC
#define MIDAS_FRONT4_OCC 4
#endif
#ifndef MIDAS_BATCH_OCC
#define MIDAS_BATCH_OCC 1
#endif
#if defined(MIDAS_DEBUG_CLOCKS) && defined(MIDAS_FRONT_CLOCKS)
__device__ long long g_ff_clk[16384];
#define FF_T0 const long long ff_t0_ = wall_clock64()
#define FF_END do { if (threadIdx.x == 0 && blockIdx.x < 4096) { long long* c_ = g_ff_clk + (a.step & 1) * 8192; c_[2 * blockIdx.x] = ff_t0_; c_[2 * blockIdx.x + 1] = wall_clock64(); } } while (0)
#else
#define FF_T0 do { } while (0)
#define FF_END do { } while (0)
#endif
template <typename T, int NJ, int LAZY, int FW, bool SCR = true, bool PREF = false, bool STATS = false>
__global__ __launch_bounds__(64 * FW, (!SCR && FW == 1) ? MIDAS_BATCH_OCC : (FW == 4 && LAZY == 1) ? MIDAS_FRONT4_OCC : MIDAS_FRONT_OCC) void k_frame_front(TreeView<Kd6> t6, TreeView<Kd3> t3, ParticleUpdateArgs a,
                                                         int n_pu, int nwaves, const T* __restrict__ emb,
                                                         const double* __restrict__ norms, const double* __restrict__ code,
                                                         double* __restrict__ scores, int64_t K) {
    static_assert(LAZY != 1 || FW == 4, "the workgroup-level tables take 256 threads");
    FF_T0;
    __shared__ double s_cd[FW][KD_MAX_LEVELS * 64];
    __shared__ alignas(16) double s_rs[LAZY == 1 ? LAZY_WG_LDS : LAZY == 2 ? FW * LAZY_WAVE_LDS : 8];
    const int w = threadIdx.x >> 6;
    const unsigned bx = blockIdx.x, by = blockIdx.y;
    if ((int)bx < n_pu) {
        if (LAZY == 1) lazy_tables(a.rs, s_rs);
        const int64_t wave = (int64_t)bx * FW + w;
        if (wave < nwaves) {
            constexpr bool SCREEN = FW == 1 && MIDAS_SCREEN && SCR;
            const int traj = (int)by;
            if (LAZY == 2) particle_update_wave<true, SCREEN, PREF, STATS, !SCR && !STATS>(t6, t3, a, wave, nwaves, traj, s_cd[w], s_rs + w * LAZY_WAVE_LDS);
            else particle_update_wave<false, SCREEN, PREF, STATS>(t6, t3, a, wave, nwaves, traj, s_cd[w], LAZY ? s_rs : nullptr);
        }
    } else if (a.sp.list) {
        if ((int)bx == n_pu && threadIdx.x == 0 && a.telemetry) {
            const int c = *a.sp.list_count;
            if (a.sp.dense_thr > 0 && c > a.sp.dense_thr) atomicAdd(&a.telemetry[3], (unsigned long long)a.sp.K);
            else if (c > 0) atomicAdd(&a.telemetry[3], (unsigned long long)(c < a.sp.list_cap ? c : a.sp.list_cap));
        }
        if (!(STATS && (a.ablate & 64)))
            score_list_wave<NJ>(a.sp, (int)(bx - n_pu) * FW + w, ((int)gridDim.x - n_pu) * FW);
    } else {
        const int64_t w0 = ((int64_t)(bx - n_pu) * FW + w) * MIDAS_SCORE_ROUNDS;
        if (w0 * 4 < K) score_wave_multi<T, NJ, MIDAS_SCORE_ROUNDS>(emb, norms, code, scores, K, w0);
    }
    FF_END;
}

struct alignas(16) PuFeat { float f[6]; int32_t hint; int32_t pad; };
static_assert(sizeof(PuFeat) == 32, "two 16-byte pieces per particle");

template <class F>
void with_nj(int32_t D, F&& f) {
    switch (D) {
        case 512: f(std::integral_constant<int, 8>()); break;
        case 256: f(std::integral_constant<int, 4>()); break;
        case 128: f(std::integral_constant<int, 2>()); break;
        default: f(std::integral_constant<int, 16>()); break;
    }
}
template <int NJ, int LAZY, int FW, bool SCR, bool PREF, bool STATS>
void launch_front_kernel(const FrontLaunch& L) {
    hipLaunchKernelGGL((k_frame_front<float, NJ, LAZY, FW, SCR, PREF, STATS>), L.grid, dim3(64 * FW), 0, L.ctx->stream, view_of<Kd6>(L.t6),
                       view_of<Kd3>(L.t3), L.a, L.n_pu, L.nwaves, (const float*)L.cb->emb, L.cb->norms, L.code, L.scores, L.cb->K);
}
template <int LAZY, int FW, bool SCR, bool PREF, bool STATS = false>
bool launch_if_form(const FrontLaunch& L, const FrontForm& f) {
    if (f.lazy != LAZY || f.fw != FW || f.scr != SCR || f.pref != PREF || f.stats != STATS) return false;
    if constexpr (STATS) launch_front_kernel<8, LAZY, FW, SCR, PREF, true>(L);
    else with_nj(L.cb->D, [&](auto nj) { launch_front_kernel<decltype(nj)::value, LAZY, FW, SCR, PREF, false>(L); });
    return true;
}

}
```

### midastouch_amd/csrc/midas_internal.hpp

```cpp
#pragma once
#include <hip/hip_runtime.h>
#include <stdint.h>

#include <cmath>
#include <string>

#include "../../include/midas_hip.h"

namespace midas {

struct alignas(16) Box6 { float lo[6], hi[6]; };
struct alignas(16) Point6 { float c[6]; int32_t idx; int32_t pad; };
struct alignas(16) Box3 { double lo[3], hi[3]; };
struct alignas(16) Point3 { double c[3]; int64_t idx; };

struct Kd6 {
    using T = float;
    using Box = Box6;
    using Point = Point6;
    static constexpr int DIM = 6;
};
struct Kd3 {
    using T = double;
    using Box = Box3;
    using Point = Point3;
    static constexpr int DIM = 3;
};

constexpr int LEAF_CAP = 16;
constexpr int KD_MAX_LEVELS = 10;

struct alignas(16) Nbr6 { float c[6]; int32_t idx; float rho; };
#ifndef MIDAS_NBR_M
#define MIDAS_NBR_M 512
#endif
constexpr int NBR_M = MIDAS_NBR_M;
constexpr int NBR_REC = NBR_M + 1;

struct alignas(16) MeshRec { double c[3]; float rho; int32_t pad; };
struct alignas(16) MeshScr { float c[3]; float rho; };
constexpr int MESH_M = 256;
constexpr int MESH_REC = MESH_M + 1;

struct MeshField {
    const float* d = nullptr;
    float lo[3] = {0.f, 0.f, 0.f};
    float h = 0.f, inv_h = 0.f;
    int32_t n[3] = {0, 0, 0};
    float expand = 0.f;
};

template <class KD>
struct TreeView {
    const typename KD::Box* boxes;
    const typename KD::Point* pts;
    const int32_t* inv_perm;
    const Nbr6* nbrs;
    const float* rho_out;
    const int32_t* twin;
    int32_t levels;
    int64_t K;
};


}

struct midas_ctx {
    int device = 0;
    hipStream_t stream = nullptr;
    bool own_stream = false;
    void* scratch = nullptr;
    size_t scratch_bytes = 0;
    std::string last_error;
    bool prof = false;
    int prof_only = -1;
    hipEvent_t ev[MIDAS_PROF_SLOTS + 1] = {};
    bool ev_ready = false;
    double prof_ms[MIDAS_PROF_SLOTS] = {};
    int64_t prof_calls = 0;
    bool overlap = true;
    hipStream_t side = nullptr;
    hipEvent_t ev_fork = nullptr, ev_join = nullptr;
    unsigned long long* tail_rec = nullptr;
    int tail_rec_blocks = 0;
    uint32_t tail_tag = 0;
};

struct midas_codebook {
    midas_ctx* ctx;
    int64_t K;
    int32_t D;
    int32_t dtype;
    const void* emb;
    double* norms;
    int32_t batch_precision = MIDAS_F32;
};

struct midas_tree {
    midas_ctx* ctx;
    int32_t dim;
    int64_t K;
    int32_t levels;
    void* boxes;
    void* pts;
    int32_t* inv_perm;
    void* nbrs;
    float* rho_out;
    int32_t* twin;
    void* vlist;
    void* vscr;
    const midas_tree* vlist_mesh;
    void* host;
    midas::MeshField field;
};

int midas_set_error(midas_ctx* ctx, int code, const char* what, const char* detail);

#define MIDAS_HIP_CHECK(ctx, expr)                                                     \
    do {                                                                               \
        hipError_t _e = (expr);                                                        \
        if (_e != hipSuccess) return midas_set_error((ctx), MIDAS_ERR_HIP, #expr, hipGetErrorString(_e)); \
    } while (0)

#define LAUNCH_CHECK(ctx) MIDAS_HIP_CHECK(ctx, hipGetLastError())

#define MIDAS_REQUIRE(ctx, cond)                                                       \
    do {                                                                               \
        if (!(cond)) return midas_set_error((ctx), MIDAS_ERR_INVALID, #cond, "invalid argument"); \
    } while (0)

#define MIDAS_WARM_TU(name, kernel)                                                          \
    int warm_##name() {                                                                      \
        hipFuncAttributes attr;                                                              \
        return (int)hipFuncGetAttributes(&attr, reinterpret_cast<const void*>(&kernel));     \
    }
#define MIDAS_WARM_DECL(name) int warm_##name();
namespace midas {
MIDAS_WARM_DECL(score) MIDAS_WARM_DECL(particles) MIDAS_WARM_DECL(resample) MIDAS_WARM_DECL(cluster) MIDAS_WARM_DECL(topn)
MIDAS_WARM_DECL(selfsim) MIDAS_WARM_DECL(loop) MIDAS_WARM_DECL(dbscan) MIDAS_WARM_DECL(dbscan_nd) MIDAS_WARM_DECL(index_build)
MIDAS_WARM_DECL(mt19937) MIDAS_WARM_DECL(topk_aten) MIDAS_WARM_DECL(score_f64) MIDAS_WARM_DECL(selfsim_f64)
MIDAS_WARM_DECL(tsne)
}

int midas_scratch(midas_ctx* ctx, size_t bytes, void** out);
struct midas_scratch_pos { size_t cur, used, total; };
midas_scratch_pos midas_scratch_mark(midas_ctx* ctx);
void midas_scratch_rewind(midas_ctx* ctx, const midas_scratch_pos& pos);

namespace midas {

enum : int {
    LOOP_I_N = MIDAS_LOOP_I_N, LOOP_I_NSET = MIDAS_LOOP_I_NSET, LOOP_I_MODE = MIDAS_LOOP_I_MODE, LOOP_I_K = MIDAS_LOOP_I_K,
    LOOP_I_INIT = MIDAS_LOOP_I_INIT, LOOP_I_VARSET = MIDAS_LOOP_I_VARSET, LOOP_I_KEPT = MIDAS_LOOP_I_KEPT,
    LOOP_I_DRIFT = MIDAS_LOOP_I_DRIFT, LOOP_I_STATUS = MIDAS_LOOP_I_STATUS, LOOP_I_RAW = MIDAS_LOOP_I_RAW,
    LOOP_I_NCL = MIDAS_LOOP_I_NCL, LOOP_I_NPRES = MIDAS_LOOP_I_NPRES, LOOP_I_FRAME = MIDAS_LOOP_I_FRAME,
    LOOP_I_NAN = MIDAS_LOOP_I_NAN, LOOP_I_ERR = MIDAS_LOOP_I_ERR, LOOP_I_NDRAW = MIDAS_LOOP_I_NDRAW,
    LOOP_D_S = MIDAS_LOOP_D_S, LOOP_D_VARPREV = MIDAS_LOOP_D_VARPREV, LOOP_D_VAR = MIDAS_LOOP_D_VAR,
    LOOP_D_RMSE_T = MIDAS_LOOP_D_RMSE_T, LOOP_D_RMSE_R = MIDAS_LOOP_D_RMSE_R, LOOP_D_XMAX = MIDAS_LOOP_D_XMAX,
    LOOP_D_XMIN = MIDAS_LOOP_D_XMIN, LOOP_D_TOTAL = MIDAS_LOOP_D_TOTAL,
    LOOP_MAX_CLUSTERS = MIDAS_LOOP_MAX_CLUSTERS,
    LOOP_CTL_I = 32, LOOP_CTL_D = 16,
};

constexpr int SCAN_CHUNK = 16;
constexpr int SCAN_TPB = 256;
constexpr int SCAN_BLOCK = SCAN_CHUNK * SCAN_TPB;
#ifndef MIDAS_GUIDE_BINS
#define MIDAS_GUIDE_BINS 2048
#endif
#ifndef MIDAS_GUIDE_UNIT
#define MIDAS_GUIDE_UNIT 8
#endif
typedef uint16_t guide_t;
constexpr int GUIDE_BINS = MIDAS_GUIDE_BINS, GUIDE_STRIDE = GUIDE_BINS + 16, GUIDE_UNIT = MIDAS_GUIDE_UNIT;
constexpr double GUIDE_WIDTH = 1.0 / GUIDE_BINS;
constexpr int TAIL_GUIDE_LDS = GUIDE_BINS / 2 + 8;
static_assert((GUIDE_BINS & (GUIDE_BINS - 1)) == 0 && GUIDE_BINS >= 2048, "bins: a power of two, eight or more per chunk");
static_assert(GUIDE_UNIT == 16 || GUIDE_UNIT == 8 || GUIDE_UNIT == 4, "units: whole chunks, halves or quarters");

constexpr int TAIL_GROUP_MAX_BLOCKS = 128;
constexpr size_t TAIL_GROUP_BLOCK_BYTES = 2 * 16 * 16 * 8;

inline int64_t ceil_div(int64_t a, int64_t b) { return (a + b - 1) / b; }

int launch_row_norms(midas_ctx* ctx, int64_t K, int32_t D, const void* emb, int32_t dtype, double* norms);
int launch_score(midas_ctx* ctx, const midas_codebook* cb, int32_t B, const double* codes, double* scores);
int launch_score_batch(midas_ctx* ctx, const midas_codebook* cb, int32_t B, const double* codes, double* scores);
int launch_score_batch_f64(midas_ctx* ctx, const midas_codebook* cb, int32_t B, const double* codes, double* scores);
int launch_score_dense_batch(midas_ctx* ctx, const midas_codebook* cb, int32_t B, const double* codes, double* scores);

int launch_se3_feature(midas_ctx* ctx, int64_t N, const float* poses, float w, float* feat6);
int launch_propagate(midas_ctx* ctx, int64_t N, const float* in, float* out, const float* odom,
                     const float* tn, const float* rot, float std_t, float std_r, uint64_t seed, uint64_t step);
int launch_check_poses(midas_ctx* ctx, int64_t N, const float* poses, uint8_t* flag, int32_t* count);
int launch_nn6(midas_ctx* ctx, const midas_tree* t, int64_t N, const float* feat6, const int32_t* hint,
               int32_t* idx, float* d2);
int launch_nn3(midas_ctx* ctx, const midas_tree* t, int64_t N, const float* poses, double* dist);
int launch_nn6_stats(midas_ctx* ctx, const midas_tree* t, int64_t N, const float* feat6, const int32_t* hint,
                     int32_t* leaves, int32_t* nodes);
int launch_rmse(midas_ctx* ctx, int64_t N, const float* poses, const float* gt16, double* out2);
constexpr int LAZY_MAX_BLOCKS = 256;
struct LazyResample {
    bool enabled = false;
    const double *e, *x_raw, *lp, *lp_raw, *gend, *gend_raw;
    const double *ggend, *ggend_raw;
    const guide_t *guide = nullptr, *guide_raw = nullptr;
    const double *bsum_e, *btot, *btot_raw, *bmax, *bmin;
    const float* poses_prev;
    const int32_t* nn_prev;
    const int32_t* status_prev;
    int32_t* ridx_out;
    int nb, ng;
    int32_t softmax, mode;
    const double* u;
    float u32;
    uint64_t seed, step;
    int64_t tstride = 0;
    int64_t key_base = 0;
    int32_t traj = 0;
};

struct SparseScore {
    uint32_t* stamps = nullptr;
    uint32_t epoch = 0;
    const float* emb = nullptr;
    const double* norms = nullptr;
    const double* code = nullptr;
    double* scores = nullptr;
    int nj = 0;
    uint32_t pred_tag = 0;
    const int32_t* list = nullptr;
    const int32_t* list_count = nullptr;
    int32_t* next_count = nullptr;
    int32_t list_cap = 0;
    int32_t dense_thr = 0;
    int64_t K = 0;
};
#ifndef MIDAS_PRED_CHANCES
#define MIDAS_PRED_CHANCES 3
#endif
constexpr uint32_t PRED_SECOND = 0xC0000000u;
constexpr uint32_t PRED_AGE1 = 0x40000000u;
constexpr uint32_t MIDAS_EPOCH_LIMIT = 0x3FFFFFF0u;
struct ScorePredict {
    uint32_t* stamps = nullptr;
    uint32_t epoch = 0;
    int64_t K = 0;
    int32_t* list = nullptr;
    int32_t* count = nullptr;
};

struct PeerInboxSrc {
    const char* rows = nullptr;
    long long flag_off = 0;
    unsigned long long tag = 0;
    int G = 0, rank = 0;
    char* const* peers = nullptr;
    int32_t* status = nullptr;
};

struct ParticleUpdateArgs {
    int64_t N;
    const float* poses_in;
    float* poses_prop;
    const float* odom16;
    const float* tn;
    const float* rot;
    float std_t, std_r;
    uint64_t seed, step;
    const int32_t* n_live = nullptr;
    int64_t slot_base = 0;
    int32_t batch = 1;
    int64_t score_stride = 0;
    const int32_t* hint_in;
    int32_t* nn_idx;
    const double* scores;
    double* x;
    double* e;
    uint8_t* valid;
    double t2;
    double thr;
    const MeshRec* vlist;
    const MeshScr* vscr = nullptr;
    MeshField field;
    double* part_max;
    double* part_min;
    const float* gt16;
    double* part_rmse;
    int ablate = 0;
    unsigned long long* telemetry = nullptr;
    int32_t* status_reset = nullptr;
    double* flags_reset = nullptr;
    LazyResample rs;
    SparseScore sp;
    PeerInboxSrc inbox;
    const int32_t* pre_order = nullptr;
    const int32_t* pre_src = nullptr;
    double* pre_rmse_terms = nullptr;
};
int particle_update_blocks(int64_t N);
bool index_build_on_host();
int build_neighbour_graph_device(midas_ctx* ctx, midas_tree* t);
int build_vertex_screen(midas_ctx* ctx, midas_tree* t6);
int build_vertex_lists_device(midas_ctx* ctx, midas_tree* t6, const midas_tree* t3, const float* cb_poses_dev);
int launch_knn6(midas_ctx* ctx, const midas_tree* t, int64_t N, const float* feat6, int32_t k, int32_t* idx, float* d2);
int launch_frame_front(midas_ctx* ctx, const midas_tree* t6, const midas_tree* t3, const ParticleUpdateArgs& a,
                       const midas_codebook* cb, const double* code, double* scores, bool* launched);
int launch_particle_update(midas_ctx* ctx, const midas_tree* t6, const midas_tree* t3, const ParticleUpdateArgs& a);
int launch_front_small_batch(midas_ctx* ctx, const midas_tree* t6, const midas_tree* t3, const ParticleUpdateArgs& a,
                             const midas_codebook* cb, const double* code, double* scores, int32_t B, bool wide = false);
struct FrontForm { int lazy, fw; bool scr, pref, stats; };
struct FrontLaunch {
    midas_ctx* ctx; const midas_tree *t6, *t3; const ParticleUpdateArgs& a; const midas_codebook* cb; const double* code; double* scores;
    dim3 grid; int n_pu, nwaves;
};
bool launch_front_plain(const FrontLaunch& L, const FrontForm& f);
bool launch_front_folded(const FrontLaunch& L, const FrontForm& f);
bool launch_front_batch(const FrontLaunch& L, const FrontForm& f);
int launch_presort(midas_ctx* ctx, ParticleUpdateArgs& a);

inline double squared_threshold(double thr) {
    if (!(thr >= 0.0)) return -1.0;
    if (std::isinf(thr)) return INFINITY;
    double t = thr * thr;
    while (std::sqrt(t) > thr) t = std::nextafter(t, 0.0);
    while (std::sqrt(std::nextafter(t, INFINITY)) <= thr) t = std::nextafter(t, INFINITY);
    return t;
}

template <class FrameArgs>
inline void fill_particle_update(ParticleUpdateArgs& pa, const FrameArgs& s, const midas_tree* t6, const midas_tree* t3, int64_t N,
                                 const float* poses_in, const int32_t* hint_in, uint8_t* valid, uint32_t* stamps, const float* gt16,
                                 double* part_rmse) {
    pa.N = N;
    pa.poses_in = poses_in;
    pa.poses_prop = s.poses_prop_dev;
    pa.odom16 = s.odom16_dev;
    pa.tn = s.tn_dev;
    pa.rot = s.rot_dev;
    pa.std_t = s.std_t;
    pa.std_r = s.std_r;
    pa.seed = s.seed;
    pa.step = s.step;
    pa.hint_in = hint_in;
    pa.nn_idx = s.nn_idx_dev;
    pa.valid = valid;
    pa.t2 = squared_threshold(s.prune_thr);
    pa.thr = s.prune_thr;
    pa.vlist = (t6->vlist && t6->vlist_mesh == t3) ? (const MeshRec*)t6->vlist : nullptr;
    pa.vscr = pa.vlist ? (const MeshScr*)t6->vscr : nullptr;
    pa.field = t3->field;
    pa.telemetry = (unsigned long long*)s.telemetry_dev;
    pa.gt16 = gt16;
    pa.part_rmse = part_rmse;
    if (stamps && s.score_epoch) { pa.sp.stamps = stamps; pa.sp.epoch = s.score_epoch; }
}

inline ScorePredict next_score_list(uint32_t* stamps, uint32_t epoch, int32_t* lists, int64_t K) {
    const int par = (int)((epoch >> 1) & 1u) ^ 1;
    ScorePredict p;
    p.stamps = stamps; p.epoch = epoch; p.K = K;
    p.count = lists + par;
    p.list = lists + 2 + (int64_t)par * K;
    return p;
}
inline ScorePredict wire_score_list(SparseScore& sp, int32_t* lists, int64_t K) {
    const int par = (int)((sp.epoch >> 1) & 1u);
    sp.pred_tag = sp.epoch - 1u;
    sp.list_count = lists + par;
    sp.list = lists + 2 + (int64_t)par * K;
    sp.list_cap = (int32_t)(K < 0x7fffffff ? K : 0x7fffffff);
    sp.next_count = lists + (par ^ 1);
    return next_score_list(sp.stamps, sp.epoch, lists, K);
}

int launch_gather_f64(midas_ctx* ctx, int64_t N, const double* table, const int32_t* idx, double* out);
int launch_softmax(midas_ctx* ctx, int64_t N, const double* x, int32_t softmax, double* w);
int launch_prune(midas_ctx* ctx, int64_t N, double* w, const double* dist, double thr, int32_t* nvalid);
int launch_cdf(midas_ctx* ctx, int64_t N, const double* w, double* cdf, int32_t* status);
int launch_search(midas_ctx* ctx, int64_t N, const double* cdf, int64_t M, int32_t mode, const double* u,
                  float u32, uint64_t seed, uint64_t step, int32_t* idx);
int launch_gather_rows(midas_ctx* ctx, int64_t M, const int32_t* idx, const void* src, void* dst, int32_t row_bytes);
int launch_selftest_wave_sums(midas_ctx* ctx, const double* in64, double* out256);
int launch_tail_a(midas_ctx* ctx, int64_t N, const double* x, const uint8_t* valid, int np, int pstride,
                  const double* pmax_all, const double* pmin_all, int32_t softmax, double* e_io, double* lp_out,
                  double* block_sums_e, double* block_totals_em, double* flags_out, int32_t* flag, int32_t* status,
                  int batch = 1);

struct StepTailArgs {
    int32_t batch = 1;
    int64_t N;
    int npart;
    const double* x;
    double* e;
    const uint8_t* valid;
    const double* part_max;
    const double* part_min;
    int32_t softmax;
    double* weights;
    double* cdf;
    int32_t* status;
    int32_t mode;
    const double* u;
    float u32;
    uint64_t seed, step;
    int32_t* ridx;
    const float* poses_prop;
    float* poses_out;
    double* weights_out;
    const int32_t* nn_idx;
    int32_t* hint_out;
    const double* part_rmse;
    double* rmse_out;
    const double* scores = nullptr;
    double* x_raw = nullptr;
    double* lp_raw = nullptr;
    int64_t score_stride = 0;
    int64_t tstride = 0;
};
template <class TailFrameArgs>
inline void fill_step_tail(StepTailArgs& ta, const TailFrameArgs& s) {
    ta.N = s.N;
    ta.softmax = s.softmax;
    ta.weights = s.weights_dev;
    ta.status = s.status_dev;
    ta.mode = s.resample_mode;
    ta.u = s.u_dev;
    ta.u32 = s.u32;
    ta.seed = s.seed;
    ta.step = s.step;
    ta.ridx = s.ridx_dev;
    ta.poses_prop = s.poses_prop_dev;
    ta.poses_out = s.poses_out_dev;
    ta.weights_out = s.weights_out_dev;
    ta.nn_idx = s.nn_idx_dev;
    ta.hint_out = s.hint_out_dev;
    ta.rmse_out = s.rmse_dev;
}
struct TailTables {
    double *e, *x_raw, *lp, *lp_raw, *gend, *gend_raw;
    double *bsum_e, *btot, *btot_raw, *bmax, *bmin;
    double *ggend, *ggend_raw;
    guide_t *guide = nullptr, *guide_raw = nullptr;
};
int launch_tail_a2(midas_ctx* ctx, int64_t N, const double* scores, const int32_t* nn_idx, const uint8_t* valid,
                   int32_t softmax, const TailTables& tb, int32_t* status, int batch = 1, int64_t score_stride = 0,
                   bool padded_tables = false, const double* part_rmse = nullptr, double* rmse_out = nullptr, int64_t tstride = 0,
                   const ScorePredict* predict = nullptr);
int launch_predict_seed(midas_ctx* ctx, int64_t N, const int32_t* idx, const ScorePredict& pr);
int launch_shard_tail_a(midas_ctx* ctx, int64_t N, const double* scores, const int32_t* nn_idx, const uint8_t* valid,
                        int32_t softmax, const TailTables& tb, double* r1, int32_t* status, const double* part_rmse = nullptr,
                        const ScorePredict* predict = nullptr);
int launch_tail_b2(midas_ctx* ctx, const StepTailArgs& a, const TailTables& tb);
int launch_step_tail(midas_ctx* ctx, const StepTailArgs& a, int prof_slot_base);
int debug_tb2_clocks(long long* out16);
int debug_ta_clocks(long long* out16);
int debug_tg_clocks(long long* io64, int reset);
int debug_tg_waves(long long* out4096);

int launch_tail_fin(midas_ctx* ctx, int64_t N, const double* e, const double* x_raw, const double* lp, const double* lp_raw,
                    const uint8_t* valid, double* weights, double* cdf_io, int G, int nb, const double* r1_all, int rank,
                    double n_total, int32_t softmax, double* rmse_out, int32_t* status);
int launch_tail_resample(midas_ctx* ctx, const midas_tail_resample_args& r);
struct PeerRouteSync { const char* inbox; long long flag_off; unsigned long long tag; };
int launch_shard_route(midas_ctx* ctx, const midas_shard_route_args& r, const TailTables& tb, bool pack, const PeerRouteSync* sync = nullptr);
int launch_shard_unpack(midas_ctx* ctx, int64_t N, const void* recv, int32_t* ridx, float* poses_out, double* weights_out,
                        int32_t* hint_out, int32_t dest = -1);
int launch_shard_unpack_peer(midas_ctx* ctx, int64_t N, const void* inbox, int32_t* ridx, float* poses_out, double* weights_out,
                             int32_t* hint_out);
int launch_peer_flag_write(midas_ctx* ctx, void* const* peers, int G, int rank, int64_t flag_off, uint64_t tag);
int launch_shard_unpack_peer_wait(midas_ctx* ctx, int64_t N, const void* inbox, int32_t* ridx, float* poses_out, double* weights_out,
                                  int32_t* hint_out, int G, int64_t flag_off, uint64_t tag, int32_t* status, void* const* peers, int rank);
int launch_peer_probe(midas_ctx* ctx, void* const* peers, const void* inbox, int G, int rank, int nonce, int32_t* ok);

int debug_ff_clocks(long long* io8192, int reset);
int launch_reduce_partials(midas_ctx* ctx, int np, const double* pmax, const double* pmin, const double* prm,
                           double* extrema2, double* rmse_sums2);

int launch_cluster_centers(midas_ctx* ctx, int64_t N, const float* poses, const double* w64, const float* w32,
                           const int64_t* labels, int32_t C, const int64_t* label_values, float* centers, float* stds,
                           int64_t* counts);

int launch_pose_estimate(midas_ctx* ctx, int64_t N, int32_t B, const float* poses, const double* w64, const TailTables* tb,
                         int64_t tstride, const uint8_t* valid, int32_t softmax, float* centers, float* stds);

constexpr int ESTIMATE_PART_DOUBLES = 36;
int launch_shard_estimate_moments(midas_ctx* ctx, int64_t N, const float* poses, const double* w64, double* part);
int launch_shard_estimate_finish(midas_ctx* ctx, int64_t nblocks, const double* part_all, float* center, float* stds);

struct LoopWeightsArgs;
int launch_loop_cluster(midas_ctx* ctx, int64_t cap, const int32_t* ctl_i, const float* poses, const double* w64,
                        const int32_t* labels, double* part, float* centers, float* stds, int64_t* counts, double* rot,
                        const LoopWeightsArgs* weights = nullptr,
                        int32_t B = 1);

int launch_loop_step(midas_ctx* ctx, const midas_codebook* cb, const midas_tree* t6, const midas_tree* t3,
                     const midas_loop_args& a, int32_t phases);
int launch_loop_step_batch(midas_ctx* ctx, const midas_codebook* cb, const midas_tree* t6, const midas_tree* t3,
                           const midas_loop_args& a, int32_t phases, int32_t B, int64_t log_stride,
                           bool wide = false);

struct LoopGrid {
    int64_t cap;
    int32_t B = 1;
    int32_t slice = 0;
    int32_t lp_stride = 0;
    int64_t log_stride = 0;
    double* clocks = nullptr;
    unsigned nbcap() const { return (unsigned)ceil_div(cap, SCAN_BLOCK); }
    unsigned by() const { return (unsigned)B; }
    bool batch() const { return slice != 0; }
};
inline int32_t loop_bound(int64_t n) { return (int32_t)(n < (1 << 30) ? n : (1 << 30)); }
bool loop_weights_mergeable(int32_t phases);
int loop_weights_phase(midas_ctx* ctx, const midas_loop_args& s, const LoopGrid& g, int64_t K, bool rmse, bool merged, LoopWeightsArgs& wa);
struct LoopMoments { float *cen, *sd; int64_t* cnt; double* rot; };
enum class LoopAnneal {
    frozen,
    aten_walk,
    small,
    select
};
inline LoopAnneal loop_anneal_regime(bool frozen, bool aten, bool small) {
    return frozen ? LoopAnneal::frozen : aten ? LoopAnneal::aten_walk : small ? LoopAnneal::small : LoopAnneal::select;
}
int loop_anneal_phase(midas_ctx* ctx, const midas_loop_args& s, const LoopGrid& g, const LoopMoments& m, LoopAnneal regime);
int launch_loop_decide(midas_ctx* ctx, const midas_loop_args& s, const LoopGrid& g, const LoopMoments& m, uint32_t* hist,
                       int32_t* sel_state, int32_t frozen, int32_t aten_order);
int launch_anneal_small(midas_ctx* ctx, const LoopGrid& g, int32_t* ctl_i, double* ctl_d, const LoopMoments* m, float* centers_out,
                        float* stds_out, int32_t floor_n, const double* w, int32_t* src);
int loop_resample_phase(midas_ctx* ctx, const midas_loop_args& s, const LoopGrid& g, int64_t cap2);
// ... 49 lines not shown
```

### midastouch_amd/csrc/resample_search.hpp

```cpp
#pragma once
#include "midas_internal.hpp"
#include <type_traits>

namespace midas {

typedef const __attribute__((address_space(3))) double* lds_cdp;
struct NoMid { MD void operator()() const {} };
template <typename LPT, typename GT, typename MID = NoMid>
MD int64_t search_in_block_t(LPT lp, const double* __restrict__ gend, const double* __restrict__ ggend,
                             int b, int64_t N, int64_t one_slot, double bp, double total, double tq, bool upper, GT gend_lds,
                             const guide_t* __restrict__ guide = nullptr, double Wb = 0.0, MID mid = MID()) {
    const double sg = total < 0.0 ? -1.0 : 1.0;
    const double tt = sg * (tq * total), sbp = sg * bp;
    auto left = [&](double v_) { const double c = fma_(sg, v_, sbp); return upper ? (c <= tt) : (c < tt); };
    auto left_exact = [&](double c) { return upper ? (c <= tq) : (c < tq); };
    const int64_t b_lo = (int64_t)b << 12, b_hi = b_lo + SCAN_BLOCK < N ? b_lo + SCAN_BLOCK : N;
    constexpr bool LP_LDS = __is_same(LPT, lds_cdp);
    auto cdfv = [&](int64_t i, double lpv) { return (i == one_slot) ? 1.0 : (bp + lpv) / total; };
    auto finish = [&](auto uc, int64_t s0, bool two) -> int64_t {
        constexpr int U = decltype(uc)::value;
        double v[U], v2[U];
        auto fetch_to = [&](LPT p, double* d) {
            if constexpr (LP_LDS) {
#pragma unroll
                for (int j = 0; j < U; ++j) d[j] = p[j];
            } else {
                const double2* p2 = reinterpret_cast<const double2*>(p);
#pragma unroll
                for (int j = 0; j < U / 2; ++j) { const double2 w = p2[j]; d[2 * j] = w.x; d[2 * j + 1] = w.y; }
            }
        };
        double v_prev = lp[s0 > b_lo ? s0 - 1 : b_lo];
        fetch_to(lp + s0, v);
        if (two) {
            fetch_to(lp + s0 + U, v2);
#pragma unroll
            for (int j = 0; j < U; ++j) asm volatile("" : "+v"(v2[j]));
        }
        asm volatile("" : "+v"(v_prev));
        int lim = (int)(b_hi - s0);
        int pos = 0;
#pragma unroll
        for (int j = 0; j < U; ++j) pos += (j < lim && left(v[j])) ? 1 : 0;
        if (two && pos == U) {
            v_prev = v[U - 1];
            s0 += U;
            lim -= U;
            pos = 0;
#pragma unroll
            for (int j = 0; j < U; ++j) { v[j] = v2[j]; pos += (j < lim && left(v[j])) ? 1 : 0; }
        }
        int64_t l2 = s0 + pos;
        double vm = v_prev, vp = 0.0;
#pragma unroll
        for (int j = 0; j < U; ++j) { vm = (j == pos - 1) ? v[j] : vm; vp = (j == pos) ? v[j] : vp; }
        bool walk = l2 >= b_hi;
        if (!walk) {
            if (l2 > b_lo) walk |= !left_exact(cdfv(l2 - 1, vm));
            walk |= pos >= U || left_exact(cdfv(l2, vp));
        }
        if (walk) {
            if (l2 >= b_hi) l2 = b_hi - 1;
            while (l2 > b_lo) {
                if (left_exact(cdfv(l2 - 1, lp[l2 - 1]))) break;
                --l2;
            }
            while (l2 < b_hi - 1) {
                if (!left_exact(cdfv(l2, lp[l2]))) break;
                ++l2;
            }
        }
        return l2;
    };
    if constexpr (!LP_LDS) {
        if (guide && Wb > 0.0 && total > 0.0 && Wb < INFINITY) {
            const double x = tq * total - bp, q = Wb * GUIDE_WIDTH;
            const double kf = x * ((double)GUIDE_BINS * __builtin_amdgcn_rcp(Wb));
            int k = kf > 0.0 ? (kf < (double)(GUIDE_BINS - 1) ? (int)kf : GUIDE_BINS - 1) : 0;
            if (k > 0 && x < (double)k * q) --k;
            if (k < GUIDE_BINS - 1 && x >= (double)(k + 1) * q) ++k;
            const guide_t* g = guide + (int64_t)b * GUIDE_STRIDE + k;
            const int uA = g[0], uB = g[1];
            __builtin_amdgcn_sched_barrier(0);
            mid();
            __builtin_amdgcn_sched_barrier(0);
            if (uB >= uA && uB - uA <= 1 && (int64_t)uB * GUIDE_UNIT < b_hi - b_lo)
                return finish(std::integral_constant<int, GUIDE_UNIT>(), b_lo + (int64_t)uA * GUIDE_UNIT, uB != uA);
        }
    }
    double v[SCAN_CHUNK];
    auto fetch16 = [&](const double* __restrict__ p) {
        const double2* p2 = reinterpret_cast<const double2*>(p);
#pragma unroll
        for (int j = 0; j < 8; ++j) { const double2 w = p2[j]; v[2 * j] = w.x; v[2 * j + 1] = w.y; }
    };
    const int n_chunks = (int)((b_hi - b_lo + SCAN_CHUNK - 1) >> 4), n_groups = (n_chunks + 15) >> 4;
    int64_t cidx;
    if (gend_lds) {
        int lo = (int)(b_lo >> 4), hi = lo + n_chunks - 1;
        while (lo < hi) {
            const int mid = lo + ((hi - lo) >> 1);
            if (left(gend_lds[mid])) lo = mid + 1; else hi = mid;
        }
        cidx = lo;
    } else {
        fetch16(ggend + (int64_t)b * 16);
        int g = 0;
#pragma unroll
        for (int j = 0; j < 16; ++j) g += (j < n_groups && left(v[j])) ? 1 : 0;
        g = g < n_groups ? g : n_groups - 1;
        const int64_t c0 = (b_lo >> 4) + 16 * g;
        fetch16(gend + c0);
        const int n_in_group = n_chunks - 16 * g < 16 ? n_chunks - 16 * g : 16;
        int c = 0;
#pragma unroll
        for (int j = 0; j < 16; ++j) c += (j < n_in_group && left(v[j])) ? 1 : 0;
        c = c < n_in_group ? c : n_in_group - 1;
        cidx = c0 + c;
    }
    return finish(std::integral_constant<int, SCAN_CHUNK>(), cidx << 4, false);
}

MD int64_t search_in_block(const double* __restrict__ lp, const double* __restrict__ gend, const double* __restrict__ ggend,
                           int b, int64_t N, int64_t one_slot, double bp, double total, double tq, bool upper) {
    return search_in_block_t<const double*, const double*>(lp, gend, ggend, b, N, one_slot, bp, total, tq, upper, (const double*)nullptr);
}

}
```

### midastouch_amd/csrc/tail.hip

```cpp
#include "midas_internal.hpp"
#include "midas_math.hpp"
#include "tail_sums.hpp"
#include "tail_block.hpp"
#include "tail_group.hpp"

namespace midas {


MD int pad16(int i) { return i + (i >> 4); }

MD void scan_variant(const double* val, const uint8_t* okm, int64_t base, int64_t N, double* s_a, double* s_m,
                     double* s_gtot, double* __restrict__ lp_out, double* __restrict__ gend_out,
                     double* __restrict__ ggend_out, double& W_all, double& W_masked, bool& nan) {
    const int t = threadIdx.x;
#pragma unroll
    for (int k = 0; k < SCAN_CHUNK; ++k) {
        const int s = k * 256 + t;
        const bool in = base + s < N;
        const double v = in ? val[k] : 0.0;
        const double m = in ? v * (okm[k] ? 1.0 : 0.0) : 0.0;
        nan |= m != m;
        s_a[pad16(s)] = v;
        s_m[pad16(s)] = m;
    }
// ... 149 lines not shown
}

__global__ __launch_bounds__(256) void k_predict_mark(int64_t N, const int32_t* __restrict__ idx, uint32_t* __restrict__ stamps, int64_t K, uint32_t epoch) {
    const int64_t n = (int64_t)blockIdx.x * 256 + threadIdx.x;
    if (n >= N) return;
    const int32_t r = idx[n];
    if (r >= 0 && r < K) stamps[r] = epoch;
}
__global__ __launch_bounds__(256) void k_predict_scan(ScorePredict pr) {
    __shared__ int s_wt[8];
    predict_scan(pr, (int)blockIdx.x, s_wt);
}

static int predict_blocks(const ScorePredict* predict) { return predict ? (int)ceil_div(predict->K, 256 * PREDICT_PER_THREAD) : 0; }

int launch_predict_seed(midas_ctx* ctx, int64_t N, const int32_t* idx, const ScorePredict& pr) {
    MIDAS_HIP_CHECK(ctx, hipMemsetAsync(pr.count, 0, sizeof(int32_t), ctx->stream));
    hipLaunchKernelGGL(k_predict_mark, dim3((unsigned)ceil_div(N, 256)), dim3(256), 0, ctx->stream, N, idx, pr.stamps, pr.K, pr.epoch);
    hipLaunchKernelGGL(k_predict_scan, dim3((unsigned)predict_blocks(&pr)), dim3(256), 0, ctx->stream, pr);
    MIDAS_HIP_CHECK(ctx, hipGetLastError());
    return MIDAS_OK;
}

MD void frame_rmse(const double* __restrict__ part_rmse, int nrm, int64_t N, double* s_red, double* __restrict__ rmse_out, bool rmse_raw,
                   bool stamp, bool reused = false) {
    const int t = threadIdx.x;
    double p = 0.0, q = 0.0;
    for (int k = t; k < nrm; k += 256) { p += part_rmse[2 * k]; q += part_rmse[2 * k + 1]; }
    p = wave_sum_ordered(p);
    q = wave_sum_ordered(q);
    if (reused) __syncthreads();
    if ((t & 63) == 0) { s_red[t >> 6] = p; s_red[4 + (t >> 6)] = q; }
    __syncthreads();
    if (t == 0) {
        p = (s_red[0] + s_red[1]) + (s_red[2] + s_red[3]);
        q = (s_red[4] + s_red[5]) + (s_red[6] + s_red[7]);
        if (rmse_raw) {
            rmse_out[0] = p;
            rmse_out[1] = q;
            return;
        }
        rmse_out[0] = __builtin_sqrt(p / (double)N);
        rmse_out[1] = __builtin_sqrt(q / (double)N);
        if (stamp) rmse_out[2] = (double)wall_clock64() * 0.01;
    }
}

__global__ __launch_bounds__(256) void k_tail_a2d(int64_t N, const double* __restrict__ scores, const int32_t* __restrict__ nn_idx,
                                                  const uint8_t* __restrict__ valid, int32_t softmax, TailTables tb, bool padded,
                                                  int32_t* __restrict__ status, double* __restrict__ flags_out,
                                                  const double* __restrict__ part_rmse, int nrm, double* __restrict__ rmse_out,
                                                  int64_t score_stride = 0, int64_t tstride = 0, int nb_tail = 0x7fffffff,
                                                  ScorePredict pr = ScorePredict(), bool rmse_raw = false) {
    __shared__ double s_gtot[32];
    __shared__ double s_red[24];
    __shared__ uint32_t s_gh[TAIL_GUIDE_LDS];
    if ((int)blockIdx.x >= nb_tail) {
        predict_scan(pr, (int)blockIdx.x - nb_tail, reinterpret_cast<int*>(s_red));
        return;
    }
    if (blockIdx.y) {
        const int64_t b = blockIdx.y, o = b * N, ts = b * tstride;
        scores += b * score_stride; nn_idx += o; valid += o; status += 2 * b;
        tb.e += ts; tb.x_raw += ts; tb.lp += ts; tb.lp_raw += ts; tb.gend += ts; tb.gend_raw += ts; tb.ggend += ts; tb.ggend_raw += ts;
        tb.bsum_e += ts; tb.btot += ts; tb.btot_raw += ts; tb.bmax += ts; tb.bmin += ts;
        if (part_rmse) { part_rmse += 2 * b * nrm; rmse_out += 3 * b; }
        tb.guide = nullptr; tb.guide_raw = nullptr;
    }
    int kept = 0;
    bool nan = false;
    tail_a_direct(N, (int)blockIdx.x, scores, nn_idx, valid, softmax, tb, padded, s_gtot, s_red, kept, nan, tb.guide ? s_gh : nullptr);
    const int t = threadIdx.x;
    if (t == 0) {
        if (nan) atomicOr(&status[0], 2);
        if (kept) atomicAdd(&status[1], kept);
        if (flags_out) {
            if (nan) atomicAdd(&flags_out[0], 1.0);
            if (kept) atomicAdd(&flags_out[1], (double)kept);
        }
    }
    if (rmse_out && blockIdx.x == 0) frame_rmse(part_rmse, nrm, N, s_red, rmse_out, rmse_raw, true, true);
}

__global__ __launch_bounds__(256) void k_tail_a3(TailGroupArgs a, int ngroups, int nwg, const double* __restrict__ part_rmse, int nrm,
                                                 double* __restrict__ rmse_out, bool rmse_raw, ScorePredict pr) {
    __shared__ double s_E[4][2 * TG_GROUP / GUIDE_UNIT];
    __shared__ double s_red[24];
    int b = (int)blockIdx.x;
    const int t = threadIdx.x;
    if (b < nwg) {
        const int wv = __builtin_amdgcn_readfirstlane(t >> 6), G = 4 * b + wv;
        if (G < ngroups) tail_group_wave(a, G, s_E[wv]);
        return;
    }
    b -= nwg;
    if (rmse_out) {
        if (b == 0) {
            TG_SPAN(2048, wall_clock64());
            frame_rmse(part_rmse, nrm, a.N, s_red, rmse_out, rmse_raw, true);
            TG_SPAN(2049, wall_clock64());
            return;
        }
        b -= 1;
    }
    predict_scan(pr, b, reinterpret_cast<int*>(s_red));
}

static int tail_resident_workgroups(midas_ctx* ctx) {
    static int cap_dev[64] = {};
    const int di = ctx->device >= 0 && ctx->device < 64 ? ctx->device : 0;
    if (!cap_dev[di] || ctx->device != di) {
        hipDeviceProp_t prop;
        const int ncu = (hipGetDeviceProperties(&prop, ctx->device) == hipSuccess && prop.multiProcessorCount > 0) ? prop.multiProcessorCount : 0;
        int occ = 0;
        if (hipOccupancyMaxActiveBlocksPerMultiprocessor(&occ, (const void*)k_tail_a3, 256, 0) != hipSuccess) { occ = 0; (void)hipGetLastError(); }
        cap_dev[di] = ncu * occ > 0 ? ncu * occ : -1;
    }
    return cap_dev[di];
}
static bool tail_grouped_ok(midas_ctx* ctx, int64_t N, const int32_t* nn_idx, const uint8_t* valid, const TailTables& tb, int extra) {
    const char* env = getenv("MIDAS_TAIL_GROUPED");
    const bool on = !(env && env[0] == '0');
    if (!on || !ctx->tail_rec || N < SCAN_CHUNK || ceil_div(N, SCAN_BLOCK) > ctx->tail_rec_blocks) return false;
    if ((ceil_div(N, TG_GROUP) + 3) / 4 + 1 + extra > tail_resident_workgroups(ctx)) return false;
    const uintptr_t al = (uintptr_t)nn_idx | (uintptr_t)tb.e | (uintptr_t)tb.x_raw | (uintptr_t)tb.lp | (uintptr_t)tb.lp_raw;
    return (al & 15) == 0 && ((uintptr_t)valid & 3) == 0;
}
static int launch_tail_a3(midas_ctx* ctx, int64_t N, const double* scores, const int32_t* nn_idx, const uint8_t* valid, int32_t softmax,
                          const TailTables& tb, bool padded, int32_t* status, double* flags_out, const double* part_rmse, double* rmse_out,
                          bool rmse_raw, const ScorePredict* predict) {
    TailGroupArgs a;
    a.N = N; a.scores = scores; a.nn_idx = nn_idx; a.valid = valid; a.softmax = softmax; a.tb = tb; a.padded = padded;
    a.status = status; a.flags_out = flags_out; a.rec = ctx->tail_rec;
    if (++ctx->tail_tag == 0) ctx->tail_tag = 1;
    a.tag = ctx->tail_tag;
    const int ngroups = (int)ceil_div(N, TG_GROUP), nwg = (ngroups + 3) / 4;
    hipLaunchKernelGGL(k_tail_a3, dim3((unsigned)(nwg + (rmse_out ? 1 : 0) + predict_blocks(predict))), dim3(256), 0, ctx->stream, a, ngroups, nwg, part_rmse,
                       particle_update_blocks(N), rmse_out, rmse_raw, predict ? *predict : ScorePredict());
    LAUNCH_CHECK(ctx);
    return MIDAS_OK;
}

int launch_tail_a2(midas_ctx* ctx, int64_t N, const double* scores, const int32_t* nn_idx, const uint8_t* valid,
                   int32_t softmax, const TailTables& tb, int32_t* status, int batch, int64_t score_stride, bool padded_tables,
                   const double* part_rmse, double* rmse_out, int64_t tstride, const ScorePredict* predict) {
    const int nb = (int)ceil_div(N, SCAN_BLOCK);
    const ScorePredict* list = predict && predict->stamps && predict->list && batch <= 1 ? predict : nullptr;
    if (list && N < SCAN_CHUNK) return midas_set_error(ctx, MIDAS_ERR_INVALID, "score_list", "the prediction list needs the direct tail kernel (N >= 16)");
    if (batch <= 1 && tail_grouped_ok(ctx, N, nn_idx, valid, tb, predict_blocks(list)))
        return launch_tail_a3(ctx, N, scores, nn_idx, valid, softmax, tb, padded_tables, status, nullptr, part_rmse,
                              part_rmse ? rmse_out : (double*)nullptr, false, list);
    if ((batch <= 1 || tstride > 0) && N >= SCAN_CHUNK) {
        hipLaunchKernelGGL(k_tail_a2d, dim3((unsigned)(nb + predict_blocks(list)), (unsigned)(batch > 1 ? batch : 1)), dim3(256), 0, ctx->stream, N, scores, nn_idx,
                           valid, softmax, tb, padded_tables, status, (double*)nullptr, part_rmse, particle_update_blocks(N),
                           part_rmse ? rmse_out : (double*)nullptr, score_stride, tstride, nb, list ? *list : ScorePredict());
        LAUNCH_CHECK(ctx);
        return MIDAS_OK;
    }
    if (tb.guide && batch <= 1) {
        MIDAS_HIP_CHECK(ctx, hipMemsetAsync(tb.guide, 0xFF, (size_t)nb * GUIDE_STRIDE * sizeof(guide_t), ctx->stream));
        if (tb.guide_raw) MIDAS_HIP_CHECK(ctx, hipMemsetAsync(tb.guide_raw, 0xFF, (size_t)nb * GUIDE_STRIDE * sizeof(guide_t), ctx->stream));
    }
    hipLaunchKernelGGL(k_tail_a2, dim3((unsigned)nb, (unsigned)(batch > 1 ? batch : 1)), dim3(256), 0, ctx->stream, N, scores, nn_idx, valid, softmax, tb.e, tb.x_raw,
                       tb.lp, tb.lp_raw, tb.gend, tb.gend_raw, tb.ggend, tb.ggend_raw, tb.bsum_e, tb.btot, tb.btot_raw, tb.bmax, tb.bmin,
                       status, nullptr, score_stride);
    LAUNCH_CHECK(ctx);
    return MIDAS_OK;
}

int launch_shard_tail_a(midas_ctx* ctx, int64_t N, const double* scores, const int32_t* nn_idx, const uint8_t* valid,
                        int32_t softmax, const TailTables& tb, double* r1, int32_t* status, const double* part_rmse,
                        const ScorePredict* predict) {
    const int nb = (int)ceil_div(N, SCAN_BLOCK);
    const ScorePredict* list = predict && predict->stamps && predict->list ? predict : nullptr;
    if ((part_rmse || list) && N < SCAN_CHUNK)
        return midas_set_error(ctx, MIDAS_ERR_INVALID, "shard tail", "rmse sums / prediction list in the tail need the direct tail kernel (N >= 16)");
    if (N >= SCAN_CHUNK) {
        TailTables t = tb;
        t.bsum_e = r1; t.btot = r1 + nb; t.btot_raw = r1 + 2 * nb; t.bmax = r1 + 3 * nb; t.bmin = r1 + 4 * nb;
        if (tail_grouped_ok(ctx, N, nn_idx, valid, t, predict_blocks(list)))
            return launch_tail_a3(ctx, N, scores, nn_idx, valid, softmax, t, true, status, r1 + 5 * nb, part_rmse,
                                  part_rmse ? r1 + 5 * nb + 2 : (double*)nullptr, true, list);
        hipLaunchKernelGGL(k_tail_a2d, dim3((unsigned)(nb + predict_blocks(list))), dim3(256), 0, ctx->stream, N, scores, nn_idx, valid, softmax, t, true,
                           status, r1 + 5 * nb, part_rmse, particle_update_blocks(N), part_rmse ? r1 + 5 * nb + 2 : (double*)nullptr,
                           (int64_t)0, (int64_t)0, nb, list ? *list : ScorePredict(), true);
        LAUNCH_CHECK(ctx);
        return MIDAS_OK;
    }
    if (tb.guide)
        MIDAS_HIP_CHECK(ctx, hipMemsetAsync(tb.guide, 0xFF, (size_t)2 * nb * GUIDE_STRIDE * sizeof(guide_t), ctx->stream));
    hipLaunchKernelGGL(k_tail_a2, dim3((unsigned)nb), dim3(256), 0, ctx->stream, N, scores, nn_idx, valid, softmax, tb.e, tb.x_raw,
                       tb.lp, tb.lp_raw, tb.gend, tb.gend_raw, tb.ggend, tb.ggend_raw, r1, r1 + nb, r1 + 2 * nb, r1 + 3 * nb, r1 + 4 * nb,
                       status, r1 + 5 * nb, 0);
    LAUNCH_CHECK(ctx);
    return MIDAS_OK;
}

MD double cdf_at(const double* __restrict__ lp, const double* s_bp, double total, int64_t i, int64_t N) {
    return (i == N - 1) ? 1.0 : (s_bp[i >> 12] + lp[i]) / total;
}

struct TailBArgs {
    int64_t N;
    int nb;
    const double* e;
    const uint8_t* valid;
    const double* lp;
    const double* block_sums_e;
    const double* block_totals_em;
    const int32_t* flag;
    int32_t* status;
    double* weights;
    int32_t mode;
    const double* u;
    float u32;
    uint64_t seed, step;
    int32_t* ridx;
    const float* poses_prop;
    float* poses_out;
    double* weights_out;
    const int32_t* nn_idx;
    int32_t* hint_out;
    const double* part_rmse;
    int nrm;
    double* rmse_out;
    int64_t slot_base;
};

__global__ __launch_bounds__(256) void k_tail_b(TailBArgs a) {
    __shared__ double s_bp[TB_MAX_BLOCKS];
    __shared__ double s_end[TB_MAX_BLOCKS];
    __shared__ double s_tot[2];
    if (blockIdx.y) {
        const int64_t b = blockIdx.y, o = b * a.N;
        a.e += o; a.valid += o; a.lp += o; a.block_sums_e += b * a.nb; a.block_totals_em += b * a.nb;
        a.flag += b; a.status += 2 * b; a.weights += o;
        if (a.u) a.u += o;
        a.ridx += o; a.poses_prop += o * 16; a.poses_out += o * 16; a.weights_out += o; a.nn_idx += o; a.hint_out += o;
        if (a.part_rmse) { a.part_rmse += 2 * b * a.nrm; a.rmse_out += 2 * b; }
        a.slot_base += o;
    }
    const bool apply = a.flag[0] != 0;
    for (int b = threadIdx.x; b < a.nb; b += 256) { s_bp[b] = a.block_totals_em[b]; s_end[b] = apply ? a.block_sums_e[b] : 0.0; }
    __syncthreads();
    if (threadIdx.x == 0) {
        double acc = 0.0;
        for (int b = 0; b < a.nb; ++b) { const double w = s_bp[b]; s_bp[b] = acc; acc = acc + w; }
        s_tot[0] = acc;
        double S = 1.0;
        if (apply) {
            S = 0.0;
            for (int b = 0; b < a.nb; ++b) S = S + s_end[b];
        }
        s_tot[1] = S;
    }
    __syncthreads();
    const double total = s_tot[0], S = s_tot[1];
// ... 418 lines not shown
```

### midastouch_amd/csrc/tail_group.hpp

```cpp
#pragma once
#include "midas_internal.hpp"
#include "midas_math.hpp"
#include "tail_block.hpp"

namespace midas {

#ifdef MIDAS_DEBUG_CLOCKS
extern __device__ long long g_tg_clk[64];
extern __device__ long long g_tg_w[8192];
#define TG_CLK(k) do { tg_clk_[k] = wall_clock64(); } while (0)
#define TG_CLK_ARG , long long* tg_clk_
#define TG_CLK_PASS , tg_clk_
#define TG_SPAN(slot, t_) do { if ((threadIdx.x & 63) == 0 && (slot) < 4096) g_tg_w[(a.tag & 1) * 4096 + (slot)] = (t_); } while (0)
#else
#define TG_CLK(k) do { } while (0)
#define TG_CLK_ARG
#define TG_CLK_PASS
#define TG_SPAN(slot, t_) do { } while (0)
#endif

constexpr int TG_GROUP = 256;
constexpr int TG_VALUES = 5;
constexpr int TG_REC_WORDS = 16;
constexpr int TG_ROUNDS = 2;
constexpr size_t TG_BLOCK_WORDS = (size_t)TG_ROUNDS * 16 * TG_REC_WORDS;
constexpr long long TG_WAIT_TICKS = 20000000ll;

struct TailGroupArgs {
    int64_t N;
    const double* scores;
    const int32_t* nn_idx;
    const uint8_t* valid;
    int32_t softmax;
    TailTables tb;
    bool padded;
    int32_t* status;
    double* flags_out;
    unsigned long long* rec;
    uint32_t tag;
};

MD uint64_t tg_key(uint32_t tag, int round, int i) {
    return ((((uint64_t)tag << 8) | (uint64_t)((round << 4) | i)) + 1ull) * 0x9E3779B97F4A7C15ull;
}
MD double readlane_d(double v, int l) {
    const uint64_t b = (uint64_t)__double_as_longlong(v);
    return double_of((uint32_t)__builtin_amdgcn_readlane((int)(uint32_t)b, l), (uint32_t)__builtin_amdgcn_readlane((int)(uint32_t)(b >> 32), l));
}
MD double shfl_d(double v, int l) {
    const uint64_t b = (uint64_t)__double_as_longlong(v);
    return double_of((uint32_t)__shfl((int)(uint32_t)b, l), (uint32_t)__shfl((int)(uint32_t)(b >> 32), l));
}

typedef unsigned int tg_u32x4 __attribute__((ext_vector_type(4)));
MD void tg_store16(unsigned long long* p, uint64_t lo, uint64_t hi) {
    tg_u32x4 v;
    v.x = (unsigned)lo; v.y = (unsigned)(lo >> 32); v.z = (unsigned)hi; v.w = (unsigned)(hi >> 32);
    asm volatile("global_store_dwordx4 %0, %1, off sc1" : : "v"(p), "v"(v) : "memory");
}
MD void tg_load80(const unsigned long long* p, uint64_t* w) {
    tg_u32x4 v0, v1, v2, v3, v4;
    asm volatile("global_load_dwordx4 %0, %5, off sc1\n\t"
                 "global_load_dwordx4 %1, %5, off offset:16 sc1\n\t"
                 "global_load_dwordx4 %2, %5, off offset:32 sc1\n\t"
                 "global_load_dwordx4 %3, %5, off offset:48 sc1\n\t"
                 "global_load_dwordx4 %4, %5, off offset:64 sc1\n\t"
                 "s_waitcnt vmcnt(0)"
                 : "=&v"(v0), "=&v"(v1), "=&v"(v2), "=&v"(v3), "=&v"(v4) : "v"(p) : "memory");
    const tg_u32x4 v[5] = {v0, v1, v2, v3, v4};
#pragma unroll
    for (int i = 0; i < 5; ++i) {
        w[2 * i] = (uint64_t)v[i].x | ((uint64_t)v[i].y << 32);
        w[2 * i + 1] = (uint64_t)v[i].z | ((uint64_t)v[i].w << 32);
    }
}

struct TGBlock {
    double W, Wa, mx, mn;
    int kept;
    bool vnan, late;
};

MD TGBlock tg_variant(const TailGroupArgs& a, int G, int round, const double* v, unsigned ok4, double gmx, double gmn, int gkept,
                      bool gxnan, double* __restrict__ lp_out, double* __restrict__ gend_out, double* __restrict__ ggend_out,
                      guide_t* __restrict__ guide_out, double* s_E TG_CLK_ARG) {
    const int lane = threadIdx.x & 63, c = lane >> 2, k = lane & 3;
    const int blk = G >> 4, g = G & 15;
    const int64_t N = a.N, bbase = (int64_t)blk * SCAN_BLOCK, s0 = (int64_t)G * TG_GROUP + 4 * lane;
    const int64_t left_n = N - bbase;
    const int nch = left_n >= SCAN_BLOCK ? SCAN_TPB : (int)((left_n + SCAN_CHUNK - 1) >> 4);
    const int ngb = (nch + 15) >> 4;
    double m[4];
    bool vnan = false, negw = false;
#pragma unroll
    for (int j = 0; j < 4; ++j) {
        m[j] = v[j] * ((ok4 >> j) & 1u ? 1.0 : 0.0);
        vnan |= m[j] != m[j];
        negw |= m[j] < 0.0;
    }
    vnan = __any(vnan ? 1 : 0) != 0;
    negw = __any(negw ? 1 : 0) != 0;
    double cm = 0.0, ca = 0.0, L[4] = {0.0, 0.0, 0.0, 0.0}, endm = 0.0, enda = 0.0;
#pragma unroll
    for (int s = 0; s < 4; ++s) {
        const double r0 = cm + m[0], r1 = r0 + m[1], r2 = r1 + m[2], r3 = r2 + m[3];
        const double q3 = (((ca + v[0]) + v[1]) + v[2]) + v[3];
        if (k == s) { L[0] = r0; L[1] = r1; L[2] = r2; L[3] = r3; endm = r3; enda = q3; }
        if (s < 3) {
            const double um = dpp_move<0x111>(r3), ua = dpp_move<0x111>(q3);
            if (k == s + 1) { cm = um; ca = ua; }
        }
    }
    double accm = 0.0, acca = 0.0, TP = 0.0;
#pragma unroll
    for (int J = 0; J < 16; ++J) {
        if (c == J) TP = accm;
        accm = accm + readlane_d(endm, 4 * J + 3);
        acca = acca + readlane_d(enda, 4 * J + 3);
    }
    const double tm = accm, ta = acca;
    TG_CLK(4 + 6 * round);
    unsigned long long* rec_b = a.rec + ((size_t)blk * TG_ROUNDS + round) * 16 * TG_REC_WORDS;
    {
        const uint64_t meta = (uint64_t)(unsigned)gkept | ((uint64_t)(gxnan ? 1 : 0) << 16) | ((uint64_t)(vnan ? 1 : 0) << 17) | ((uint64_t)(negw ? 1 : 0) << 18);
        const uint64_t v0 = lane == 0 ? (uint64_t)__double_as_longlong(tm) : lane == 1 ? (uint64_t)__double_as_longlong(ta)
                          : lane == 2 ? (uint64_t)__double_as_longlong(gmx) : lane == 3 ? (uint64_t)__double_as_longlong(gmn) : meta;
        if (lane < TG_VALUES) tg_store16(rec_b + g * TG_REC_WORDS + 2 * lane, v0, v0 ^ tg_key(a.tag, round, lane));
    }
    uint64_t w[2 * TG_VALUES];
    bool late = false;
    {
        const unsigned long long* rp = rec_b + (lane < ngb ? lane : 0) * TG_REC_WORDS;
        const long long t0 = wall_clock64();
        for (;;) {
            tg_load80(rp, w);
            bool ok = true;
#pragma unroll
            for (int i = 0; i < TG_VALUES; ++i) ok &= (w[2 * i] ^ w[2 * i + 1]) == tg_key(a.tag, round, i);
            if (__all((ok || lane >= ngb) ? 1 : 0)) break;
            if (wall_clock64() - t0 > TG_WAIT_TICKS) { late = true; break; }
        }
    }
    TG_CLK(5 + 6 * round);
    const bool have = lane < ngb;
    const double vtm = have ? __longlong_as_double((long long)w[0]) : 0.0, vta = have ? __longlong_as_double((long long)w[2]) : 0.0;
    double mx = have ? __longlong_as_double((long long)w[4]) : -INFINITY, mn = have ? __longlong_as_double((long long)w[6]) : INFINITY;
    uint32_t kp = have ? ((uint32_t)w[8] & 0xFFFFu) : 0u, fl = have ? ((uint32_t)w[8] >> 16) : 0u;
#define MIDAS_ROW_REDUCE(v, OP)                                                     \
    { auto t_ = dpp_move<0xB1>(v); v = OP(v, t_); } { auto t_ = dpp_move<0x4E>(v); v = OP(v, t_); } \
    { auto t_ = dpp_move<0x141>(v); v = OP(v, t_); } { auto t_ = dpp_move<0x140>(v); v = OP(v, t_); }
    MIDAS_ROW_REDUCE(mx, dpp_max_)
    MIDAS_ROW_REDUCE(mn, dpp_min_)
#undef MIDAS_ROW_REDUCE
    kp += dpp_move<0xB1>(kp, kp); kp += dpp_move<0x4E>(kp, kp); kp += dpp_move<0x141>(kp, kp); kp += dpp_move<0x140>(kp, kp);
    fl |= dpp_move<0xB1>(fl, fl); fl |= dpp_move<0x4E>(fl, fl); fl |= dpp_move<0x141>(fl, fl); fl |= dpp_move<0x140>(fl, fl);
    mx = readlane_d(mx, 0);
    mn = readlane_d(mn, 0);
    const int kept = __builtin_amdgcn_readlane((int)kp, 0);
    const unsigned flags = (unsigned)__builtin_amdgcn_readlane((int)fl, 0);
    double GP = 0.0, GPn = 0.0, W = 0.0, Wa = 0.0;
#pragma unroll
    for (int j = 0; j < 16; ++j) {
        GP = j == g ? W : GP;
        W = W + readlane_d(vtm, j);
        GPn = j == g ? W : GPn;
    }
    if (g == 0) {
#pragma unroll
        for (int j = 0; j < 16; ++j) Wa = Wa + readlane_d(vta, j);
    }
    if (flags & 1u) { mx = NAN; mn = NAN; }
    const bool b_vnan = (flags & 2u) != 0, b_negw = (flags & 4u) != 0;
    double out[4];
#pragma unroll
    for (int j = 0; j < 4; ++j) out[j] = GP + (TP + L[j]);
    const int64_t npad = (N + SCAN_CHUNK - 1) & ~(int64_t)(SCAN_CHUNK - 1);
    if (s0 + 4 <= N || (a.padded && s0 < npad)) {
        double2* o2 = reinterpret_cast<double2*>(lp_out + s0);
        o2[0] = make_double2(out[0], out[1]);
        o2[1] = make_double2(out[2], out[3]);
    } else {
#pragma unroll
        for (int j = 0; j < 4; ++j)
            if (s0 + j < N) lp_out[s0 + j] = out[j];
    }
    if (k == 3 && (int64_t)G * TG_GROUP + 16 * c < N) gend_out[(int64_t)G * 16 + c] = out[3];
    if (lane == 63) ggend_out[(int64_t)blk * 16 + g] = out[3];
    if (g == ngb - 1 && lane > g && lane < 16) ggend_out[(int64_t)blk * 16 + lane] = readlane_d(out[3], 63);
    TG_CLK(6 + 6 * round);
    if (guide_out) {
        constexpr int UPG = TG_GROUP / GUIDE_UNIT;
        constexpr int UPC = SCAN_CHUNK / GUIDE_UNIT;
        guide_t* gt = guide_out + (int64_t)blk * GUIDE_STRIDE;
        const bool plain = !b_negw && !b_vnan && W > 0.0 && W < (double)INFINITY;
        const unsigned maxu = plain ? (unsigned)(nch * UPC - 1) : 0xFFFFu;
        if (!plain) {
            const int share = (GUIDE_BINS + ngb - 1) / ngb, k0 = g * share, k1 = g == ngb - 1 ? GUIDE_BINS : (k0 + share < GUIDE_BINS ? k0 + share : GUIDE_BINS);
            for (int kk = k0 + lane; kk < k1; kk += 64) gt[kk] = (guide_t)0xFFFFu;
        } else {
            const double q = W * GUIDE_WIDTH, rq = (double)GUIDE_BINS * __builtin_amdgcn_rcp(W);
            auto first_beyond = [&](double x) {
                const double kf = x * rq;
                int kk = kf > 0.0 ? (kf < (double)GUIDE_BINS ? (int)kf + 1 : GUIDE_BINS) : 0;
                if (kk > 0 && (double)(kk - 1) * q > x) --kk;
                if (kk < GUIDE_BINS && (double)kk * q <= x) ++kk;
                return __builtin_amdgcn_readfirstlane(kk);
            };
            const int k_lo = g == 0 ? 0 : first_beyond(GP), k_hi = g == ngb - 1 ? GUIDE_BINS : first_beyond(GPn);
            int nu = UPC * (nch - 16 * g);
            nu = nu > UPG ? UPG : nu;
            constexpr int LPU = GUIDE_UNIT / 4;
            if ((lane & (LPU - 1)) == LPU - 1) s_E[lane / LPU] = out[3];
            __builtin_amdgcn_fence(__ATOMIC_RELEASE, "wavefront");
            __builtin_amdgcn_wave_barrier();
            __builtin_amdgcn_fence(__ATOMIC_ACQUIRE, "wavefront");
            const unsigned below = (unsigned)(UPG * g);
            constexpr int Q = UPG / 8;
            double eq[8];
#pragma unroll
            for (int i = 0; i < 8; ++i) eq[i] = readlane_d(out[3], (i + 1) * Q * LPU - 1);
            constexpr int BPL = 4;
            for (int kb = k_lo; kb < k_hi; kb += 64 * BPL) {
                int lo[BPL];
                double edge[BPL];
#pragma unroll
                for (int i = 0; i < BPL; ++i) {
                    edge[i] = (double)(kb + lane + 64 * i) * q;
                    int l = ((8 * Q <= nu) & (eq[7] < edge[i])) ? 8 * Q : 0;
                    const bool h4 = (l == 0) & (4 * Q <= nu) & (eq[3] < edge[i]);
                    l = h4 ? 4 * Q : l;
                    const double e2 = h4 ? eq[5] : eq[1];
                    const bool h2 = (l < 8 * Q) & (l + 2 * Q <= nu) & (e2 < edge[i]);
                    l = h2 ? l + 2 * Q : l;
                    const double e1 = h4 ? (h2 ? eq[6] : eq[4]) : (h2 ? eq[2] : eq[0]);
                    l = ((l < 8 * Q) & (l + Q <= nu) & (e1 < edge[i])) ? l + Q : l;
                    lo[i] = l;
                }
#pragma unroll
                for (int step = Q / 2; step > 0; step >>= 1) {
                    double e[BPL];
#pragma unroll
                    for (int i = 0; i < BPL; ++i) e[i] = s_E[(lo[i] + step - 1) & (2 * UPG - 1)];
#pragma unroll
                    for (int i = 0; i < BPL; ++i) lo[i] += ((lo[i] + step <= nu) & (e[i] < edge[i])) ? step : 0;
                }
#pragma unroll
                for (int i = 0; i < BPL; ++i) {
                    const int kk = kb + lane + 64 * i;
                    const unsigned e = below + (unsigned)lo[i];
                    if (kk < k_hi) gt[kk] = (guide_t)(e < maxu ? e : maxu);
                }
            }
        }
        if (g == ngb - 1 && lane == 0) gt[GUIDE_BINS] = (guide_t)maxu;
    }
    TG_CLK(7 + 6 * round);
    TGBlock r;
    r.W = W; r.Wa = Wa; r.mx = mx; r.mn = mn; r.kept = kept; r.vnan = b_vnan; r.late = late;
    return r;
}

MD void tail_group_wave(const TailGroupArgs& a, int G, double* s_E) {
    const int lane = threadIdx.x & 63;
    const int blk = G >> 4, g = G & 15;
    const int64_t N = a.N, s0 = (int64_t)G * TG_GROUP + 4 * lane;
    const TailTables& tb = a.tb;
#ifdef MIDAS_DEBUG_CLOCKS
    long long tg_clk_[16] = {0, 0, 0, 0, 0, 0, 0, 0, 0, 0, 0, 0, 0, 0, 0, 0};
#endif
    TG_CLK(0);
    int32_t nn[4] = {0, 0, 0, 0};
    unsigned ok4 = 0, in4 = 0;
    if (s0 + 4 <= N) {
        const int4 n4 = *reinterpret_cast<const int4*>(a.nn_idx + s0);
        const uint32_t vb = *reinterpret_cast<const uint32_t*>(a.valid + s0);
        nn[0] = n4.x; nn[1] = n4.y; nn[2] = n4.z; nn[3] = n4.w;
        ok4 = ((vb & 0xFFu) ? 1u : 0u) | ((vb & 0xFF00u) ? 2u : 0u) | ((vb & 0xFF0000u) ? 4u : 0u) | ((vb & 0xFF000000u) ? 8u : 0u);
        in4 = 0xFu;
    } else {
#pragma unroll
        for (int j = 0; j < 4; ++j)
            if (s0 + j < N) {
                nn[j] = a.nn_idx[s0 + j];
                ok4 |= a.valid[s0 + j] != 0 ? (1u << j) : 0u;
                in4 |= 1u << j;
            }
    }
    double x[4];
#pragma unroll
    for (int j = 0; j < 4; ++j) x[j] = a.scores[nn[j]];
    TG_CLK(1);
    double mx = -INFINITY, mn = INFINITY;
    bool xnan = false;
#pragma unroll
    for (int j = 0; j < 4; ++j) {
        const bool in = (in4 >> j) & 1u;
        x[j] = in ? x[j] : 0.0;
        xnan |= in && x[j] != x[j];
        mx = in && x[j] > mx ? x[j] : mx;
        mn = in && x[j] < mn ? x[j] : mn;
    }
    mx = wave_max_dpp(mx);
    mn = wave_min_dpp(mn);
    const int gkept = wave_isum_dpp(__popc(ok4));
    const bool gxnan = __any(xnan ? 1 : 0) != 0;
    TG_CLK(2);
    const int64_t npad = (N + SCAN_CHUNK - 1) & ~(int64_t)(SCAN_CHUNK - 1);
    auto store4 = [&](double* __restrict__ o, const double* val) {
        if (s0 + 4 <= N || (a.padded && s0 < npad)) {
            double2* o2 = reinterpret_cast<double2*>(o + s0);
            o2[0] = make_double2(val[0], val[1]);
            o2[1] = make_double2(val[2], val[3]);
        } else {
#pragma unroll
            for (int j = 0; j < 4; ++j)
                if (s0 + j < N) o[s0 + j] = val[j];
        }
    };
    const bool need_soft = a.softmax != 0;
    TGBlock r0;
    bool close = false, late = false, nan = false;
    if (need_soft) {
        double e[4];
#pragma unroll
        for (int j = 0; j < 4; ++j) e[j] = exp_spec(x[j] - 1.0);
        TG_CLK(3);
        store4(tb.e, e);
#pragma unroll
        for (int j = 0; j < 4; ++j) e[j] = (in4 >> j) & 1u ? e[j] : 0.0;
        r0 = tg_variant(a, G, 0, e, ok4, mx, mn, gkept, gxnan, tb.lp, tb.gend, tb.ggend, tb.guide, s_E TG_CLK_PASS);
        close = __builtin_fabs(r0.mx - r0.mn) <= ISCLOSE_ATOL;
        late |= r0.late;
        nan = r0.vnan;
        if (g == 0 && lane == 0) { tb.bsum_e[blk] = r0.Wa; tb.btot[blk] = r0.W; }
    }
    const bool need_raw = !need_soft || close;
    if (need_raw) {
        store4(tb.x_raw, x);
        const TGBlock r1 = tg_variant(a, G, need_soft ? 1 : 0, x, ok4, mx, mn, gkept, gxnan, tb.lp_raw, tb.gend_raw, tb.ggend_raw, tb.guide_raw, s_E TG_CLK_PASS);
        late |= r1.late;
        if (!need_soft) { r0 = r1; nan = r1.vnan; }
        if (g == 0 && lane == 0) tb.btot_raw[blk] = r1.W;
    } else if (g == 0 && lane == 0) {
        tb.btot_raw[blk] = 0.0;
    }
    if (g == 0 && lane == 0) {
        tb.bmax[blk] = r0.mx;
        tb.bmin[blk] = r0.mn;
        if (nan) atomicOr(&a.status[0], 2);
        if (r0.kept) atomicAdd(&a.status[1], r0.kept);
        if (a.flags_out) {
            if (nan) atomicAdd(&a.flags_out[0], 1.0);
            if (r0.kept) atomicAdd(&a.flags_out[1], (double)r0.kept);
        }
    }
    if (late && lane == 0) atomicOr(&a.status[0], 16);
#ifdef MIDAS_DEBUG_CLOCKS
    TG_SPAN(2 * G, tg_clk_[0]);
    TG_SPAN(2 * G + 1, wall_clock64());
    if (lane == 0 && (G == 0 || G == 200))
        for (int i = 0; i < 8; ++i) g_tg_clk[(G ? 24 : 8) + i] = tg_clk_[i];
#endif
}

}
```

Baseline: 28020.

## Build global CDF guide table in tail and precompute lazy resample header

Adds a CDF-based guide mode for lazy resampling. The tail kernel waits on a cross-block record buffer (tail_rec2), folds the block totals, writes a lazy header, and fills a global uniform-width CDF guide. In the next front kernel, particles read this header directly instead of rebuilding per-wave tables, and they issue guide loads ahead of the search. The aim is to shorten per-particle source search and table setup. In exchange it adds a spin-wait with a timeout across blocks in the tail and more template variants.

```diff
diff --git a/include/midas_hip.h b/include/midas_hip.h
--- a/include/midas_hip.h
+++ b/include/midas_hip.h
@@ -217,6 +217,9 @@
     int32_t* score_list_dev;
     uint8_t* guide_dev;
 } midas_lazy_args;
+int midas_lazy_header_read(midas_ctx* ctx, double* out_host);
+int32_t midas_guide_cdf_bin(double tq, double total, int32_t nb);
+int32_t midas_guide_cdf_first_beyond(double x, double total, int32_t nb);
 int64_t midas_lazy_guide_bytes(int64_t N);
 int midas_lazy_guide_layout(int32_t* bins_out, int32_t* unit_out, int32_t* stride_out);
 int midas_lazy_step(midas_ctx* ctx, const midas_codebook* cb, const midas_tree* tree6, const midas_tree* tree3,
diff --git a/midastouch_amd/_lib.py b/midastouch_amd/_lib.py
--- a/midastouch_amd/_lib.py
+++ b/midastouch_amd/_lib.py
@@ -264,6 +264,9 @@
     "midas_lazy_tables_doubles": (C.c_int64, [_I64]),
     "midas_lazy_guide_bytes": (C.c_int64, [_I64]),
     "midas_lazy_guide_layout": (C.c_int, [_P, _P, _P]),
+    "midas_lazy_header_read": (C.c_int, [_P, _P]),
+    "midas_guide_cdf_bin": (C.c_int32, [_D, _D, _I32]),
+    "midas_guide_cdf_first_beyond": (C.c_int32, [_D, _D, _I32]),
     "midas_lazy_step_batch": (C.c_int, [_P, _P, _P, _P, C.POINTER(LazyArgs), _I32]),
     "midas_lazy_flush_batch": (C.c_int, [_P, C.POINTER(LazyFlushArgs), _I32]),
     "midas_loop_step": (C.c_int, [_P, _P, _P, _P, C.POINTER(LoopArgs), _I32]),
diff --git a/midastouch_amd/csrc/api.hip b/midastouch_amd/csrc/api.hip
--- a/midastouch_amd/csrc/api.hip
+++ b/midastouch_amd/csrc/api.hip
@@ -133,6 +133,15 @@
             if (p) (void)hipFree(p);
             (void)hipGetLastError();
         }
+        const size_t rec2 = 64 * 16 * sizeof(unsigned long long), hdr = 256 * sizeof(double);
+        p = nullptr;
+        if (ctx->tail_rec && hipMalloc(&p, rec2 + hdr) == hipSuccess && hipMemset(p, 0, rec2 + hdr) == hipSuccess && hipDeviceSynchronize() == hipSuccess) {
+            ctx->tail_rec2 = (unsigned long long*)p;
+            ctx->lazy_hdr = reinterpret_cast<double*>((char*)p + rec2);
+        } else {
+            if (p) (void)hipFree(p);
+            (void)hipGetLastError();
+        }
     }
     *out = ctx;
     return MIDAS_OK;
@@ -169,6 +178,7 @@
     for (auto& c : s->chunks) (void)hipFree(c.p);
     delete s;
     if (ctx->tail_rec) (void)hipFree(ctx->tail_rec);
+    if (ctx->tail_rec2) (void)hipFree(ctx->tail_rec2);
     if (ctx->ev_ready)
         for (auto& e : ctx->ev) (void)hipEventDestroy(e);
     if (ctx->own_stream) (void)hipStreamDestroy(ctx->stream);
diff --git a/midastouch_amd/csrc/api_step.hip b/midastouch_amd/csrc/api_step.hip
--- a/midastouch_amd/csrc/api_step.hip
+++ b/midastouch_amd/csrc/api_step.hip
@@ -1,4 +1,5 @@
 #include "api_entry.hpp"
+#include "lazy_header.hpp"
 
 using namespace midas;
 
@@ -151,7 +152,7 @@
 }
 
 static int lazy_step_impl(midas_ctx* ctx, const midas_codebook* cb, const midas_tree* tree6, const midas_tree* tree3,
-                          const midas_lazy_args& s, double* rmse_out, int32_t B = 1, int64_t tstride = 0) {
+                          const midas_lazy_args& s, double* rmse_out, int32_t B = 1, int64_t tstride = 0, int guide_cdf = 0) {
     MIDAS_REQUIRE(ctx, s.N > 0 && ceil_div(s.N, SCAN_BLOCK) <= LAZY_MAX_BLOCKS && s.poses_prop_dev && s.nn_idx_dev && s.valid_dev &&
                            s.status_dev && s.tables_dev && (uintptr_t)s.tables_dev % 128 == 0 && s.scores_dev && s.odom16_dev && s.code_dev);
     MIDAS_REQUIRE(ctx, s.resample_prev ? (s.poses_prop_prev_dev && s.nn_idx_prev_dev && s.status_prev_dev &&
@@ -192,6 +193,10 @@
         r.softmax = s.softmax; r.mode = s.resample_mode; r.u = s.u_prev_dev; r.u32 = s.u32_prev;
         r.seed = s.seed; r.step = s.step_prev;
         r.tstride = tstride;
+        if (B == 1 && r.guide && ctx->cdf_tables == (const void*)tb.lp && ctx->lazy_hdr && r.nb <= 64) {
+            r.guide_cdf = 1;
+            r.hdr = ctx->lazy_hdr;
+        }
     }
     prof_begin(ctx);
     prof_mark(ctx, 1);
@@ -209,7 +214,8 @@
     }
     prof_mark(ctx, 2);
     if ((rc = launch_tail_a2(ctx, N, s.scores_dev, s.nn_idx_dev, s.valid_dev, s.softmax, tb, s.status_dev, B, cb->K, true,
-                             pa.gt16 ? s.part_rmse_dev : nullptr, rmse_out, B > 1 ? tstride : 0, predict.stamps ? &predict : nullptr)))
+                             pa.gt16 ? s.part_rmse_dev : nullptr, rmse_out, B > 1 ? tstride : 0, predict.stamps ? &predict : nullptr,
+                             B == 1 ? guide_cdf : 0)))
         return rc;
     prof_mark(ctx, 3);
     return prof_end(ctx, 1, 3, false);
@@ -219,7 +225,7 @@
                                  const midas_lazy_args* args) {
     MIDAS_ENTER(ctx);
     MIDAS_REQUIRE(ctx, cb && tree6 && tree3 && args && tree6->dim == 6 && tree3->dim == 3 && tree6->K == cb->K);
-    return lazy_step_impl(ctx, cb, tree6, tree3, *args, (args->gt16_dev && args->part_rmse_dev) ? args->rmse_dev : nullptr);
+    return lazy_step_impl(ctx, cb, tree6, tree3, *args, (args->gt16_dev && args->part_rmse_dev) ? args->rmse_dev : nullptr, 1, 0, 1);
 }
 
 static int pose_estimate_impl(midas_ctx* ctx, const midas_estimate_args& s) {
@@ -255,7 +261,7 @@
     for (int32_t f = 0; f < T; ++f) {
         int rc = f ? scratch_reset(ctx) : MIDAS_OK;
         if (rc) return rc;
-        rc = lazy_step_impl(ctx, cb, tree6, tree3, a, rmse_log_dev ? rmse_log_dev + 3 * f : nullptr);
+        rc = lazy_step_impl(ctx, cb, tree6, tree3, a, rmse_log_dev ? rmse_log_dev + 3 * f : nullptr, 1, 0, 1);
         if (rc) return rc;
         if (est_centers) {
             midas_estimate_args e;
@@ -333,6 +339,21 @@
     if (stride_out) *stride_out = GUIDE_STRIDE;
     return MIDAS_OK;
 }
+MIDAS_EXPORT int midas_lazy_header_read(midas_ctx* ctx, double* out_host) {
+    MIDAS_ENTER(ctx);
+    MIDAS_REQUIRE(ctx, out_host && ctx->lazy_hdr && ctx->cdf_tables);
+    MIDAS_HIP_CHECK(ctx, hipStreamSynchronize(ctx->stream));
+    MIDAS_HIP_CHECK(ctx, hipMemcpy(out_host, ctx->lazy_hdr, LAZY_WAVE_LDS * sizeof(double), hipMemcpyDeviceToHost));
+    return MIDAS_OK;
+}
+MIDAS_EXPORT int32_t midas_guide_cdf_bin(double tq, double total, int32_t nb) {
+    const int bins = guide_cdf_bins(nb);
+    return guide_cdf_settle(guide_cdf_bin0(tq, bins), tq * total, guide_cdf_width(total, bins), bins);
+}
+MIDAS_EXPORT int32_t midas_guide_cdf_first_beyond(double x, double total, int32_t nb) {
+    const int bins = guide_cdf_bins(nb);
+    return guide_first_beyond(x, guide_cdf_width(total, bins), (double)bins / total, bins);
+}
 MIDAS_EXPORT int64_t midas_lazy_guide_bytes(int64_t N) { return N > 0 ? 2 * ceil_div(N, SCAN_BLOCK) * (int64_t)GUIDE_STRIDE * (int64_t)sizeof(guide_t) : 0; }
 
 MIDAS_EXPORT int midas_lazy_step_batch(midas_ctx* ctx, const midas_codebook* cb, const midas_tree* tree6, const midas_tree* tree3,
diff --git a/midastouch_amd/csrc/front.hip b/midastouch_amd/csrc/front.hip
--- a/midastouch_amd/csrc/front.hip
+++ b/midastouch_amd/csrc/front.hip
@@ -294,7 +294,9 @@
     static const int split_env = getenv("MIDAS_SPLIT_FRONT") ? atoi(getenv("MIDAS_SPLIT_FRONT")) : 1;
     const bool split_front = a.batch <= 1 && !a.inbox.rows && (split_env >= 2 || (split_env == 1 && ((a.rs.enabled && a.N <= 512) || (!a.rs.enabled && a.N <= 2048) || (a.n_live && a.N <= 16384))));
     const int lpp = split_env == 3 ? 2 : 4;
+    auto drop_cdf_guide = [&]() { a.rs.guide = nullptr; a.rs.guide_raw = nullptr; a.rs.guide_cdf = 0; a.rs.hdr = nullptr; };
     if (split_front && !(a.ablate & 7)) {
+        if (a.rs.guide_cdf) drop_cdf_guide();
         a.sp.pred_tag = 0; a.sp.list = nullptr;
         void* feat;
         int rc = midas_scratch(ctx, (size_t)a.N * sizeof(PuFeat), &feat);
@@ -323,6 +325,7 @@
     static const int fw_env = getenv("MIDAS_FRONT_WAVES") ? atoi(getenv("MIDAS_FRONT_WAVES")) : 0;
     static const int wt_env = getenv("MIDAS_WAVE_TABLES") ? atoi(getenv("MIDAS_WAVE_TABLES")) : 1;
     const bool wave_tables = a.rs.enabled && a.rs.nb <= LAZY_WAVE_LD && wt_env != 0;
+    if (a.rs.guide_cdf && (!wave_tables || a.batch > 1)) drop_cdf_guide();
     const int fw = a.batch > 1 ? 1 : (a.rs.enabled && !wave_tables) ? 4 : fw_env == 1 || fw_env == 4 ? fw_env : (a.sp.stamps ? 1 : 4);
     const int n_pu_fw = (nwaves + fw - 1) / fw;
     if (!use_list) { a.sp.pred_tag = 0; a.sp.list = nullptr; }
@@ -339,7 +342,7 @@
     if (a.batch > 1) form = {2, 1, false, false, false};
     else if (!a.rs.enabled) form = {0, fw, true, small_set && pref_plain, false};
     else if (!wave_tables) form = {1, 4, true, false, false};
-    else form = {2, fw, true, small_set, false};
+    else form = {2, fw, true, small_set, false, a.rs.guide_cdf != 0};
     if (a.ablate && cb->D == 512 && fw == 1 && (a.batch > 1 || !a.rs.enabled || form.pref)) {
         form.stats = true;
         if (!a.rs.enabled) form.pref = false;
diff --git a/midastouch_amd/csrc/front_folded.hip b/midastouch_amd/csrc/front_folded.hip
--- a/midastouch_amd/csrc/front_folded.hip
+++ b/midastouch_amd/csrc/front_folded.hip
@@ -5,7 +5,9 @@
 
 bool launch_front_folded(const FrontLaunch& L, const FrontForm& f) {
     return launch_if_form<1, 4, true, false>(L, f) || launch_if_form<2, 1, true, true>(L, f) || launch_if_form<2, 1, true, false>(L, f) ||
-           launch_if_form<2, 4, true, false>(L, f) || launch_if_form<2, 1, true, true, true>(L, f);
+           launch_if_form<2, 4, true, false>(L, f) || launch_if_form<2, 1, true, true, true>(L, f) ||
+           launch_if_form<2, 1, true, true, false, true>(L, f) || launch_if_form<2, 1, true, false, false, true>(L, f) ||
+           launch_if_form<2, 4, true, false, false, true>(L, f) || launch_if_form<2, 1, true, true, true, true>(L, f);
 }
 
 #if defined(MIDAS_DEBUG_CLOCKS)
diff --git a/midastouch_amd/csrc/front_wave.hpp b/midastouch_amd/csrc/front_wave.hpp
--- a/midastouch_amd/csrc/front_wave.hpp
+++ b/midastouch_amd/csrc/front_wave.hpp
@@ -6,6 +6,7 @@
 #include "score_body.hpp"
 #include "peer_row.hpp"
 #include "resample_search.hpp"
+#include "lazy_header.hpp"
 #include "list_scan.hpp"
 #include "pose.hpp"
 
@@ -60,7 +61,6 @@
     __syncthreads();
 }
 
-constexpr int LAZY_WAVE_LD = 64, LAZY_WAVE_LDS = 3 * LAZY_WAVE_LD + 4;
 struct LazyRecords { double bt, btr, bx, bn; int32_t status; };
 MD LazyRecords lazy_records_load(const LazyResample& rs) {
     const int lane = threadIdx.x & 63;
@@ -112,6 +112,21 @@
     __builtin_amdgcn_fence(__ATOMIC_ACQUIRE, "wavefront");
 }
 
+MD double lazy_draw(const LazyResample& rs, int64_t n, int64_t N, bool& upper) {
+    double tq;
+    if (rs.mode == MIDAS_RESAMPLE_MULTINOMIAL) {
+        tq = rs.u ? rs.u[n] : philox_uniform53((uint64_t)(n + rs.key_base), rs.seed, rs.step);
+        upper = false;
+    } else {
+        const float r = rs.u32 >= 0.0f ? rs.u32 : philox_uniform24(rs.seed + (uint64_t)rs.traj, rs.step);
+        const float off = r / (float)N;
+        tq = (double)n / (double)N + (double)off;
+        tq = tq >= 1.0 ? tq - 1.0 : tq;
+        upper = true;
+    }
+    return tq;
+}
+
 template <typename GT = const double*, typename LT = const double*, typename MID = NoMid>
 MD int64_t lazy_source(const LazyResample& rs, const double* rs_lds, int64_t n, int64_t N, int ld = 256, GT gend_lds = nullptr,
                        LT lp_lds = nullptr, MID mid = MID()) {
@@ -123,18 +138,8 @@
     if (rs_lds[2 * ld + 3] != 0.0 || bad_total) return n;
     const double* __restrict__ lp = apply ? rs.lp : rs.lp_raw;
     const double* __restrict__ gend = apply ? rs.gend : rs.gend_raw;
-    double tq;
     bool upper;
-    if (rs.mode == MIDAS_RESAMPLE_MULTINOMIAL) {
-        tq = rs.u ? rs.u[n] : philox_uniform53((uint64_t)(n + rs.key_base), rs.seed, rs.step);
-        upper = false;
-    } else {
-        const float r = rs.u32 >= 0.0f ? rs.u32 : philox_uniform24(rs.seed + (uint64_t)rs.traj, rs.step);
-        const float off = r / (float)N;
-        tq = (double)n / (double)N + (double)off;
-        tq = tq >= 1.0 ? tq - 1.0 : tq;
-        upper = true;
-    }
+    const double tq = lazy_draw(rs, n, N, upper);
     auto left_exact = [&](double c) { return upper ? (c <= tq) : (c < tq); };
     int lo = 0, hi = rs.nb;
     while (hi > lo) {
@@ -151,7 +156,42 @@
     }
 }
 
-template <bool WT = false, bool SCREEN = false, bool PREF = false, bool STATS = false, bool PRES = false, bool NANPART = false>
+MD void guide_ahead_load(const LazyResample& rs, double tq, int& k0, uint32_t& wa, uint32_t& wb) {
+    k0 = guide_cdf_bin0(tq, guide_cdf_bins(rs.nb));
+    const guide_t* gp = rs.guide + k0;
+    __builtin_memcpy(&wa, gp - (k0 > 0 ? 1 : 0), 4);
+    __builtin_memcpy(&wb, gp + 1, 4);
+}
+MD int64_t lazy_source_cdf(const LazyResample& rs, const double* rs_lds, int64_t n, int64_t N, double tq, bool upper, int k0, uint32_t wa,
+                           uint32_t wb, bool& fell) {
+    const int e0 = (int)(wa & 0xFFFFu), e1 = k0 > 0 ? (int)(wa >> 16) : e0, e2 = (int)(wb & 0xFFFFu), e3 = (int)(wb >> 16);
+    constexpr int ld = LAZY_WAVE_LD;
+    const double* s_bp = rs_lds;
+    const double* s_end = rs_lds + ld;
+    const double total = rs_lds[2 * ld];
+    const bool apply = rs_lds[2 * ld + 2] != 0.0;
+    const bool bad_total = !(total == total) || total == 0.0;
+    if (rs_lds[2 * ld + 3] != 0.0 || bad_total) return n;
+    auto left_exact = [&](double c) { return upper ? (c <= tq) : (c < tq); };
+    int lo = 0, hi = rs.nb;
+    while (hi > lo) {
+        const int mid = lo + ((hi - lo) >> 1);
+        if (left_exact(s_end[mid])) lo = mid + 1; else hi = mid;
+    }
+    if (lo >= rs.nb) return N - 1;
+    int uA = 0xFFFF, uB = 0xFFFF;
+    if (total > 0.0 && total < INFINITY) {
+        const int bins = guide_cdf_bins(rs.nb);
+        const int d = guide_cdf_settle(k0, tq * total, guide_cdf_width(total, bins), bins) - k0;
+        uA = d < 0 ? e0 : d > 0 ? e2 : e1;
+        uB = d < 0 ? e1 : d > 0 ? e3 : e2;
+    }
+    return search_in_block_t<const double*, const double*, NoMid>(apply ? rs.lp : rs.lp_raw, apply ? rs.gend : rs.gend_raw, apply ? rs.ggend : rs.ggend_raw,
+                                                                   lo, N, N - 1, s_bp[lo], total, tq, upper, (const double*)nullptr, nullptr, 0.0, NoMid(),
+                                                                   uA, uB, &fell);
+}
+
+template <bool WT = false, bool SCREEN = false, bool PREF = false, bool STATS = false, bool PRES = false, bool NANPART = false, bool CDF = false>
 MD void particle_update_wave(const TreeView<Kd6>& t6, const TreeView<Kd3>& t3, ParticleUpdateArgs a, int64_t wave,
                              int nwaves, int traj, double* s_cd, double* rs_lds = nullptr) {
     const int lane = threadIdx.x & 63;
@@ -220,20 +260,68 @@
 #pragma unroll
         for (int i = 0; i < 16; ++i) O[i] = a.odom16[i];
         __builtin_amdgcn_sched_barrier(0);
+        constexpr bool cdf = CDF && !PRES;
         LazyRecords rec;
-        if (!presorted) rec = lazy_records_load(a.rs);
+        double h_bp = 0.0, h_end = 0.0, h_total = 0.0, h_apply = 0.0;
+        int32_t h_status = 0;
+        double g_tq = 0.0;
+        bool g_upper = false;
+        int g_k0 = 0;
+        uint32_t g_wa = 0xFFFFFFFFu, g_wb = 0xFFFFFFFFu;
+        const bool ahead = cdf && a.rs.u == nullptr;
+        if (cdf) {
+            const int hb = lane < a.rs.nb ? lane : a.rs.nb - 1;
+            h_bp = a.rs.hdr[hb]; h_end = a.rs.hdr[LAZY_WAVE_LD + hb];
+            h_total = a.rs.hdr[2 * LAZY_WAVE_LD]; h_apply = a.rs.hdr[2 * LAZY_WAVE_LD + 2];
+            h_status = a.rs.status_prev[0];
+            if (ahead) {
+                g_tq = lazy_draw(a.rs, live ? n : 0, a.N, g_upper);
+                guide_ahead_load(a.rs, g_tq, g_k0, g_wa, g_wb);
+            }
+        } else if (!presorted) {
+            rec = lazy_records_load(a.rs);
+        }
         __builtin_amdgcn_sched_barrier(0);
         float tnv[3] = {0.f, 0.f, 0.f}, rotv[3] = {0.f, 0.f, 0.f};
         bool no_done = false;
         if (live) noise_draws(n, n + a.slot_base, a.tn, a.rot, a.std_t, a.std_r, a.seed, a.step, tnv, rotv);
-        if (!presorted) lazy_tables_wave(a.rs, rec, rs_lds);
-        MIDAS_PTICK(0);
         auto mid = [&]() { noise_apply(O, tnv, rotv, NO); no_done = true; };
-        if (rs_lds && live && !presorted && !(ablate & 8)) {
-            src = lazy_source(a.rs, rs_lds, n, a.N, LAZY_WAVE_LD, (const double*)nullptr, (const double*)nullptr, mid);
-            if (a.rs.ridx_out) a.rs.ridx_out[n] = (int32_t)src;
-        }
-        if (live && !no_done) mid();
+        if (cdf) {
+            if (live) mid();
+            __builtin_amdgcn_sched_barrier(0);
+            asm volatile("" : "+v"(g_wa), "+v"(g_wb), "+v"(h_status), "+v"(NO[0]), "+v"(NO[5]), "+v"(NO[10]), "+v"(NO[3]), "+v"(NO[7]), "+v"(NO[11]));
+            if (lane < a.rs.nb) { rs_lds[lane] = h_bp; rs_lds[LAZY_WAVE_LD + lane] = h_end; }
+            if (lane == 0) {
+                rs_lds[2 * LAZY_WAVE_LD] = h_total;
+                rs_lds[2 * LAZY_WAVE_LD + 2] = h_apply;
+                rs_lds[2 * LAZY_WAVE_LD + 3] = h_status != 0 ? 1.0 : 0.0;
+            }
+            __builtin_amdgcn_fence(__ATOMIC_RELEASE, "wavefront");
+            __builtin_amdgcn_wave_barrier();
+            __builtin_amdgcn_fence(__ATOMIC_ACQUIRE, "wavefront");
+            MIDAS_PTICK(0);
+            if (!ahead) {
+                g_tq = lazy_draw(a.rs, live ? n : 0, a.N, g_upper);
+                guide_ahead_load(a.rs, g_tq, g_k0, g_wa, g_wb);
+            }
+            bool fell = false;
+            if (live && !(ablate & 8)) {
+                src = lazy_source_cdf(a.rs, rs_lds, n, a.N, g_tq, g_upper, g_k0, g_wa, g_wb, fell);
+                if (a.rs.ridx_out) a.rs.ridx_out[n] = (int32_t)src;
+            }
+            if (a.telemetry) {
+                const unsigned long long m = __ballot(fell);
+                if (lane == 0 && m) atomicAdd(&a.telemetry[4], (unsigned long long)__popcll(m));
+            }
+        } else {
+            if (!presorted) lazy_tables_wave(a.rs, rec, rs_lds);
+            MIDAS_PTICK(0);
+            if (rs_lds && live && !presorted && !(ablate & 8)) {
+                src = lazy_source(a.rs, rs_lds, n, a.N, LAZY_WAVE_LD, (const double*)nullptr, (const double*)nullptr, mid);
+                if (a.rs.ridx_out) a.rs.ridx_out[n] = (int32_t)src;
+            }
+            if (live && !no_done) mid();
+        }
         MIDAS_PTICK(1);
     }
     if (rs_lds && live) {
@@ -405,7 +493,7 @@
 #define FF_T0 do { } while (0)
 #define FF_END do { } while (0)
 #endif
-template <typename T, int NJ, int LAZY, int FW, bool SCR = true, bool PREF = false, bool STATS = false>
+template <typename T, int NJ, int LAZY, int FW, bool SCR = true, bool PREF = false, bool STATS = false, bool CDF = false>
 __global__ __launch_bounds__(64 * FW, (!SCR && FW == 1) ? MIDAS_BATCH_OCC : (FW == 4 && LAZY == 1) ? MIDAS_FRONT4_OCC : MIDAS_FRONT_OCC) void k_frame_front(TreeView<Kd6> t6, TreeView<Kd3> t3, ParticleUpdateArgs a,
                                                          int n_pu, int nwaves, const T* __restrict__ emb,
                                                          const double* __restrict__ norms, const double* __restrict__ code,
@@ -422,7 +510,7 @@
         if (wave < nwaves) {
             constexpr bool SCREEN = FW == 1 && MIDAS_SCREEN && SCR;
             const int traj = (int)by;
-            if (LAZY == 2) particle_update_wave<true, SCREEN, PREF, STATS, !SCR && !STATS>(t6, t3, a, wave, nwaves, traj, s_cd[w], s_rs + w * LAZY_WAVE_LDS);
+            if (LAZY == 2) particle_update_wave<true, SCREEN, PREF, STATS, !SCR && !STATS, false, CDF>(t6, t3, a, wave, nwaves, traj, s_cd[w], s_rs + w * LAZY_WAVE_LDS);
             else particle_update_wave<false, SCREEN, PREF, STATS>(t6, t3, a, wave, nwaves, traj, s_cd[w], LAZY ? s_rs : nullptr);
         }
     } else if (a.sp.list) {
@@ -452,16 +540,16 @@
         default: f(std::integral_constant<int, 16>()); break;
     }
 }
-template <int NJ, int LAZY, int FW, bool SCR, bool PREF, bool STATS>
+template <int NJ, int LAZY, int FW, bool SCR, bool PREF, bool STATS, bool CDF = false>
 void launch_front_kernel(const FrontLaunch& L) {
-    hipLaunchKernelGGL((k_frame_front<float, NJ, LAZY, FW, SCR, PREF, STATS>), L.grid, dim3(64 * FW), 0, L.ctx->stream, view_of<Kd6>(L.t6),
+    hipLaunchKernelGGL((k_frame_front<float, NJ, LAZY, FW, SCR, PREF, STATS, CDF>), L.grid, dim3(64 * FW), 0, L.ctx->stream, view_of<Kd6>(L.t6),
                        view_of<Kd3>(L.t3), L.a, L.n_pu, L.nwaves, (const float*)L.cb->emb, L.cb->norms, L.code, L.scores, L.cb->K);
 }
-template <int LAZY, int FW, bool SCR, bool PREF, bool STATS = false>
+template <int LAZY, int FW, bool SCR, bool PREF, bool STATS = false, bool CDF = false>
 bool launch_if_form(const FrontLaunch& L, const FrontForm& f) {
-    if (f.lazy != LAZY || f.fw != FW || f.scr != SCR || f.pref != PREF || f.stats != STATS) return false;
-    if constexpr (STATS) launch_front_kernel<8, LAZY, FW, SCR, PREF, true>(L);
-    else with_nj(L.cb->D, [&](auto nj) { launch_front_kernel<decltype(nj)::value, LAZY, FW, SCR, PREF, false>(L); });
+    if (f.lazy != LAZY || f.fw != FW || f.scr != SCR || f.pref != PREF || f.stats != STATS || f.cdf != CDF) return false;
+    if constexpr (STATS) launch_front_kernel<8, LAZY, FW, SCR, PREF, true, CDF>(L);
+    else with_nj(L.cb->D, [&](auto nj) { launch_front_kernel<decltype(nj)::value, LAZY, FW, SCR, PREF, false, CDF>(L); });
     return true;
 }
 
diff --git a/midastouch_amd/csrc/lazy_header.hpp b/midastouch_amd/csrc/lazy_header.hpp
--- /dev/null
+++ b/midastouch_amd/csrc/lazy_header.hpp
@@ -0,0 +1,75 @@
+#pragma once
+#include "midas_internal.hpp"
+#include "midas_math.hpp"
+
+namespace midas {
+
+constexpr int LAZY_WAVE_LD = 64, LAZY_WAVE_LDS = 3 * LAZY_WAVE_LD + 4;
+
+struct LazyFold { double bp, w, total; bool apply; };
+
+MD LazyFold lazy_fold_wave(int nb, bool softmax, double bt, double btr, double bx, double bn, double* s_wb) {
+    const int lane = threadIdx.x & 63;
+    const bool in = lane < nb;
+    double mx = in ? bx : -INFINITY, mn = in ? bn : INFINITY;
+    const bool nan = in && ((bx != bx) || (bn != bn));
+    mx = wave_max_dpp(mx);
+    mn = wave_min_dpp(mn);
+    if (__any(nan)) { mx = NAN; mn = NAN; }
+    LazyFold f;
+    f.apply = softmax && !(__builtin_fabs(mx - mn) <= ISCLOSE_ATOL);
+    f.w = in ? (f.apply ? bt : btr) : 0.0;
+    s_wb[lane] = f.w;
+    __builtin_amdgcn_fence(__ATOMIC_RELEASE, "wavefront");
+    __builtin_amdgcn_wave_barrier();
+    __builtin_amdgcn_fence(__ATOMIC_ACQUIRE, "wavefront");
+    double acc = 0.0, bp = 0.0;
+    for (int i0 = 0; i0 < nb; i0 += 8) {
+        double wv[8];
+        const double2* p2 = reinterpret_cast<const double2*>(s_wb + i0);
+#pragma unroll
+        for (int j = 0; j < 4; ++j) { const double2 t = p2[j]; wv[2 * j] = t.x; wv[2 * j + 1] = t.y; }
+#pragma unroll
+        for (int j = 0; j < 8; ++j) {
+            bp = lane == i0 + j ? acc : bp;
+            acc = acc + wv[j];
+        }
+    }
+    f.bp = bp;
+    f.total = acc;
+    return f;
+}
+
+MD void lazy_header_store(const LazyFold& f, int nb, bool status_bad, double* dst) {
+    const int lane = threadIdx.x & 63;
+    if (lane < nb) {
+        dst[lane] = f.bp;
+        dst[LAZY_WAVE_LD + lane] = (lane == nb - 1) ? 1.0 : (f.bp + f.w) / f.total;
+    }
+    if (lane == 0) {
+        dst[2 * LAZY_WAVE_LD] = f.total;
+        dst[2 * LAZY_WAVE_LD + 2] = f.apply ? 1.0 : 0.0;
+        dst[2 * LAZY_WAVE_LD + 3] = status_bad ? 1.0 : 0.0;
+    }
+}
+
+__host__ __device__ inline int guide_cdf_bins(int nb) { return nb * GUIDE_BINS; }
+__host__ __device__ inline double guide_cdf_width(double total, int bins) { return total / (double)bins; }
+__host__ __device__ inline int guide_cdf_bin0(double tq, int bins) {
+    const double kf = tq * (double)bins;
+    return kf > 0.0 ? (kf < (double)(bins - 1) ? (int)kf : bins - 1) : 0;
+}
+__host__ __device__ inline int guide_cdf_settle(int k, double x, double q, int bins) {
+    if (k > 0 && x < (double)k * q) --k;
+    else if (k < bins - 1 && x >= (double)(k + 1) * q) ++k;
+    return k;
+}
+__host__ __device__ inline int guide_first_beyond(double x, double q, double rq, int bins) {
+    const double kf = x * rq;
+    int kk = kf > 0.0 ? (kf < (double)bins ? (int)kf + 1 : bins) : 0;
+    if (kk > 0 && (double)(kk - 1) * q > x) --kk;
+    if (kk < bins && (double)kk * q <= x) ++kk;
+    return kk;
+}
+
+}
diff --git a/midastouch_amd/csrc/midas_internal.hpp b/midastouch_amd/csrc/midas_internal.hpp
--- a/midastouch_amd/csrc/midas_internal.hpp
+++ b/midastouch_amd/csrc/midas_internal.hpp
@@ -84,6 +84,9 @@
     unsigned long long* tail_rec = nullptr;
     int tail_rec_blocks = 0;
     uint32_t tail_tag = 0;
+    unsigned long long* tail_rec2 = nullptr;
+    double* lazy_hdr = nullptr;
+    const void* cdf_tables = nullptr;
 };
 
 struct midas_codebook {
@@ -205,6 +208,8 @@
     const double *e, *x_raw, *lp, *lp_raw, *gend, *gend_raw;
     const double *ggend, *ggend_raw;
     const guide_t *guide = nullptr, *guide_raw = nullptr;
+    int32_t guide_cdf = 0;
+    const double* hdr = nullptr;
     const double *bsum_e, *btot, *btot_raw, *bmax, *bmin;
     const float* poses_prev;
     const int32_t* nn_prev;
@@ -309,7 +314,7 @@
 int launch_particle_update(midas_ctx* ctx, const midas_tree* t6, const midas_tree* t3, const ParticleUpdateArgs& a);
 int launch_front_small_batch(midas_ctx* ctx, const midas_tree* t6, const midas_tree* t3, const ParticleUpdateArgs& a,
                              const midas_codebook* cb, const double* code, double* scores, int32_t B, bool wide = false);
-struct FrontForm { int lazy, fw; bool scr, pref, stats; };
+struct FrontForm { int lazy, fw; bool scr, pref, stats; bool cdf = false; };
 struct FrontLaunch {
     midas_ctx* ctx; const midas_tree *t6, *t3; const ParticleUpdateArgs& a; const midas_codebook* cb; const double* code; double* scores;
     dim3 grid; int n_pu, nwaves;
@@ -446,7 +451,7 @@
 int launch_tail_a2(midas_ctx* ctx, int64_t N, const double* scores, const int32_t* nn_idx, const uint8_t* valid,
                    int32_t softmax, const TailTables& tb, int32_t* status, int batch = 1, int64_t score_stride = 0,
                    bool padded_tables = false, const double* part_rmse = nullptr, double* rmse_out = nullptr, int64_t tstride = 0,
-                   const ScorePredict* predict = nullptr);
+                   const ScorePredict* predict = nullptr, int guide_cdf = 0);
 int launch_predict_seed(midas_ctx* ctx, int64_t N, const int32_t* idx, const ScorePredict& pr);
 int launch_shard_tail_a(midas_ctx* ctx, int64_t N, const double* scores, const int32_t* nn_idx, const uint8_t* valid,
                         int32_t softmax, const TailTables& tb, double* r1, int32_t* status, const double* part_rmse = nullptr,
diff --git a/midastouch_amd/csrc/resample_search.hpp b/midastouch_amd/csrc/resample_search.hpp
--- a/midastouch_amd/csrc/resample_search.hpp
+++ b/midastouch_amd/csrc/resample_search.hpp
@@ -9,7 +9,8 @@
 template <typename LPT, typename GT, typename MID = NoMid>
 MD int64_t search_in_block_t(LPT lp, const double* __restrict__ gend, const double* __restrict__ ggend,
                              int b, int64_t N, int64_t one_slot, double bp, double total, double tq, bool upper, GT gend_lds,
-                             const guide_t* __restrict__ guide = nullptr, double Wb = 0.0, MID mid = MID()) {
+                             const guide_t* __restrict__ guide = nullptr, double Wb = 0.0, MID mid = MID(),
+                             int cuA = -1, int cuB = -1, bool* fell = nullptr) {
     const double sg = total < 0.0 ? -1.0 : 1.0;
     const double tt = sg * (tq * total), sbp = sg * bp;
     auto left = [&](double v_) { const double c = fma_(sg, v_, sbp); return upper ? (c <= tt) : (c < tt); };
@@ -73,7 +74,11 @@
         return l2;
     };
     if constexpr (!LP_LDS) {
-        if (guide && Wb > 0.0 && total > 0.0 && Wb < INFINITY) {
+        if (cuA >= 0) {
+            if (cuB >= cuA && cuB - cuA <= 1 && (int64_t)cuA * GUIDE_UNIT >= b_lo && (int64_t)cuB * GUIDE_UNIT < b_hi)
+                return finish(std::integral_constant<int, GUIDE_UNIT>(), (int64_t)cuA * GUIDE_UNIT, cuB != cuA);
+            if (fell) *fell = true;
+        } else if (guide && Wb > 0.0 && total > 0.0 && Wb < INFINITY) {
             const double x = tq * total - bp, q = Wb * GUIDE_WIDTH;
             const double kf = x * ((double)GUIDE_BINS * __builtin_amdgcn_rcp(Wb));
             int k = kf > 0.0 ? (kf < (double)(GUIDE_BINS - 1) ? (int)kf : GUIDE_BINS - 1) : 0;
diff --git a/midastouch_amd/csrc/tail.hip b/midastouch_amd/csrc/tail.hip
--- a/midastouch_amd/csrc/tail.hip
+++ b/midastouch_amd/csrc/tail.hip
@@ -255,15 +255,17 @@
     if (rmse_out && blockIdx.x == 0) frame_rmse(part_rmse, nrm, N, s_red, rmse_out, rmse_raw, true, true);
 }
 
+template <bool CDF>
 __global__ __launch_bounds__(256) void k_tail_a3(TailGroupArgs a, int ngroups, int nwg, const double* __restrict__ part_rmse, int nrm,
                                                  double* __restrict__ rmse_out, bool rmse_raw, ScorePredict pr) {
-    __shared__ double s_E[4][2 * TG_GROUP / GUIDE_UNIT];
+    __shared__ alignas(16) double s_E[4][2 * TG_GROUP / GUIDE_UNIT];
+    static_assert(2 * TG_GROUP / GUIDE_UNIT >= LAZY_WAVE_LD, "the CDF form folds the block totals through a wave's s_E");
     __shared__ double s_red[24];
     int b = (int)blockIdx.x;
     const int t = threadIdx.x;
     if (b < nwg) {
         const int wv = __builtin_amdgcn_readfirstlane(t >> 6), G = 4 * b + wv;
-        if (G < ngroups) tail_group_wave(a, G, s_E[wv]);
+        if (G < ngroups) tail_group_wave<CDF>(a, G, s_E[wv]);
         return;
     }
     b -= nwg;
@@ -286,7 +288,7 @@
         hipDeviceProp_t prop;
         const int ncu = (hipGetDeviceProperties(&prop, ctx->device) == hipSuccess && prop.multiProcessorCount > 0) ? prop.multiProcessorCount : 0;
         int occ = 0;
-        if (hipOccupancyMaxActiveBlocksPerMultiprocessor(&occ, (const void*)k_tail_a3, 256, 0) != hipSuccess) { occ = 0; (void)hipGetLastError(); }
+        if (hipOccupancyMaxActiveBlocksPerMultiprocessor(&occ, (const void*)k_tail_a3<false>, 256, 0) != hipSuccess) { occ = 0; (void)hipGetLastError(); }
         cap_dev[di] = ncu * occ > 0 ? ncu * occ : -1;
     }
     return cap_dev[di];
@@ -301,28 +303,39 @@
 }
 static int launch_tail_a3(midas_ctx* ctx, int64_t N, const double* scores, const int32_t* nn_idx, const uint8_t* valid, int32_t softmax,
                           const TailTables& tb, bool padded, int32_t* status, double* flags_out, const double* part_rmse, double* rmse_out,
-                          bool rmse_raw, const ScorePredict* predict) {
+                          bool rmse_raw, const ScorePredict* predict, bool cdf = false) {
     TailGroupArgs a;
+    a.cdf = cdf ? 1 : 0; a.rec2 = ctx->tail_rec2; a.hdr = ctx->lazy_hdr;
     a.N = N; a.scores = scores; a.nn_idx = nn_idx; a.valid = valid; a.softmax = softmax; a.tb = tb; a.padded = padded;
     a.status = status; a.flags_out = flags_out; a.rec = ctx->tail_rec;
     if (++ctx->tail_tag == 0) ctx->tail_tag = 1;
     a.tag = ctx->tail_tag;
     const int ngroups = (int)ceil_div(N, TG_GROUP), nwg = (ngroups + 3) / 4;
-    hipLaunchKernelGGL(k_tail_a3, dim3((unsigned)(nwg + (rmse_out ? 1 : 0) + predict_blocks(predict))), dim3(256), 0, ctx->stream, a, ngroups, nwg, part_rmse,
-                       particle_update_blocks(N), rmse_out, rmse_raw, predict ? *predict : ScorePredict());
+    const dim3 grid((unsigned)(nwg + (rmse_out ? 1 : 0) + predict_blocks(predict)));
+    if (cdf) hipLaunchKernelGGL(k_tail_a3<true>, grid, dim3(256), 0, ctx->stream, a, ngroups, nwg, part_rmse, particle_update_blocks(N), rmse_out, rmse_raw,
+                                predict ? *predict : ScorePredict());
+    else hipLaunchKernelGGL(k_tail_a3<false>, grid, dim3(256), 0, ctx->stream, a, ngroups, nwg, part_rmse, particle_update_blocks(N), rmse_out, rmse_raw,
+                            predict ? *predict : ScorePredict());
     LAUNCH_CHECK(ctx);
     return MIDAS_OK;
 }
 
 int launch_tail_a2(midas_ctx* ctx, int64_t N, const double* scores, const int32_t* nn_idx, const uint8_t* valid,
                    int32_t softmax, const TailTables& tb, int32_t* status, int batch, int64_t score_stride, bool padded_tables,
-                   const double* part_rmse, double* rmse_out, int64_t tstride, const ScorePredict* predict) {
+                   const double* part_rmse, double* rmse_out, int64_t tstride, const ScorePredict* predict, int guide_cdf) {
     const int nb = (int)ceil_div(N, SCAN_BLOCK);
+    ctx->cdf_tables = nullptr;
     const ScorePredict* list = predict && predict->stamps && predict->list && batch <= 1 ? predict : nullptr;
     if (list && N < SCAN_CHUNK) return midas_set_error(ctx, MIDAS_ERR_INVALID, "score_list", "the prediction list needs the direct tail kernel (N >= 16)");
-    if (batch <= 1 && tail_grouped_ok(ctx, N, nn_idx, valid, tb, predict_blocks(list)))
-        return launch_tail_a3(ctx, N, scores, nn_idx, valid, softmax, tb, padded_tables, status, nullptr, part_rmse,
-                              part_rmse ? rmse_out : (double*)nullptr, false, list);
+    if (batch <= 1 && tail_grouped_ok(ctx, N, nn_idx, valid, tb, predict_blocks(list))) {
+        const char* env = getenv("MIDAS_GUIDE_CDF");
+        const bool want = guide_cdf != 0 && env && env[0] == '1';
+        const bool cdf = want && tb.guide && nb <= LAZY_WAVE_LD && padded_tables && ctx->tail_rec2 && ((uintptr_t)tb.guide & 1) == 0;
+        const int rc = launch_tail_a3(ctx, N, scores, nn_idx, valid, softmax, tb, padded_tables, status, nullptr, part_rmse,
+                                      part_rmse ? rmse_out : (double*)nullptr, false, list, cdf);
+        if (rc == MIDAS_OK && cdf) ctx->cdf_tables = tb.lp;
+        return rc;
+    }
     if ((batch <= 1 || tstride > 0) && N >= SCAN_CHUNK) {
         hipLaunchKernelGGL(k_tail_a2d, dim3((unsigned)(nb + predict_blocks(list)), (unsigned)(batch > 1 ? batch : 1)), dim3(256), 0, ctx->stream, N, scores, nn_idx,
                            valid, softmax, tb, padded_tables, status, (double*)nullptr, part_rmse, particle_update_blocks(N),
@@ -346,6 +359,7 @@
                         const ScorePredict* predict) {
     const int nb = (int)ceil_div(N, SCAN_BLOCK);
     const ScorePredict* list = predict && predict->stamps && predict->list ? predict : nullptr;
+    ctx->cdf_tables = nullptr;
     if ((part_rmse || list) && N < SCAN_CHUNK)
         return midas_set_error(ctx, MIDAS_ERR_INVALID, "shard tail", "rmse sums / prediction list in the tail need the direct tail kernel (N >= 16)");
     if (N >= SCAN_CHUNK) {
diff --git a/midastouch_amd/csrc/tail_group.hpp b/midastouch_amd/csrc/tail_group.hpp
--- a/midastouch_amd/csrc/tail_group.hpp
+++ b/midastouch_amd/csrc/tail_group.hpp
@@ -2,6 +2,7 @@
 #include "midas_internal.hpp"
 #include "midas_math.hpp"
 #include "tail_block.hpp"
+#include "lazy_header.hpp"
 
 namespace midas {
 
@@ -38,6 +39,9 @@
     double* flags_out;
     unsigned long long* rec;
     uint32_t tag;
+    int32_t cdf = 0;
+    unsigned long long* rec2 = nullptr;
+    double* hdr = nullptr;
 };
 
 MD uint64_t tg_key(uint32_t tag, int round, int i) {
@@ -79,11 +83,70 @@
     double W, Wa, mx, mn;
     int kept;
     bool vnan, late;
+    bool negw;
+    double GP, GPn, end;
 };
 
+MD void tg_guide_fill(guide_t* __restrict__ gt, int bins, bool plain, double q, double rq, double lo, double hi, bool first, bool last,
+                      int part, int nparts, unsigned below, int nu, unsigned maxu, double end3, double* s_E) {
+    const int lane = threadIdx.x & 63;
+    constexpr int UPG = TG_GROUP / GUIDE_UNIT;
+    if (!plain) {
+        const int share = (bins + nparts - 1) / nparts, k0 = part * share < bins ? part * share : bins,
+                  k1 = part == nparts - 1 ? bins : (k0 + share < bins ? k0 + share : bins);
+        for (int kk = k0 + lane; kk < k1; kk += 64) gt[kk] = (guide_t)0xFFFFu;
+    } else {
+        const int k_lo = first ? 0 : __builtin_amdgcn_readfirstlane(guide_first_beyond(lo, q, rq, bins)),
+                  k_hi = last ? bins : __builtin_amdgcn_readfirstlane(guide_first_beyond(hi, q, rq, bins));
+        constexpr int LPU = GUIDE_UNIT / 4;
+        if ((lane & (LPU - 1)) == LPU - 1) s_E[lane / LPU] = end3;
+        __builtin_amdgcn_fence(__ATOMIC_RELEASE, "wavefront");
+        __builtin_amdgcn_wave_barrier();
+        __builtin_amdgcn_fence(__ATOMIC_ACQUIRE, "wavefront");
+        constexpr int Q = UPG / 8;
+        double eq[8];
+#pragma unroll
+        for (int i = 0; i < 8; ++i) eq[i] = readlane_d(end3, (i + 1) * Q * LPU - 1);
+        constexpr int BPL = 4;
+        for (int kb = k_lo; kb < k_hi; kb += 64 * BPL) {
+            int lo_[BPL];
+            double edge[BPL];
+#pragma unroll
+            for (int i = 0; i < BPL; ++i) {
+                edge[i] = (double)(kb + lane + 64 * i) * q;
+                int l = ((8 * Q <= nu) & (eq[7] < edge[i])) ? 8 * Q : 0;
+                const bool h4 = (l == 0) & (4 * Q <= nu) & (eq[3] < edge[i]);
+                l = h4 ? 4 * Q : l;
+                const double e2 = h4 ? eq[5] : eq[1];
+                const bool h2 = (l < 8 * Q) & (l + 2 * Q <= nu) & (e2 < edge[i]);
+                l = h2 ? l + 2 * Q : l;
+                const double e1 = h4 ? (h2 ? eq[6] : eq[4]) : (h2 ? eq[2] : eq[0]);
+                l = ((l < 8 * Q) & (l + Q <= nu) & (e1 < edge[i])) ? l + Q : l;
+                lo_[i] = l;
+            }
+#pragma unroll
+            for (int step = Q / 2; step > 0; step >>= 1) {
+                double e[BPL];
+#pragma unroll
+                for (int i = 0; i < BPL; ++i) e[i] = s_E[(lo_[i] + step - 1) & (2 * UPG - 1)];
+#pragma unroll
+                for (int i = 0; i < BPL; ++i) lo_[i] += ((lo_[i] + step <= nu) & (e[i] < edge[i])) ? step : 0;
+            }
+#pragma unroll
+            for (int i = 0; i < BPL; ++i) {
+                const int kk = kb + lane + 64 * i;
+                const unsigned e = below + (unsigned)lo_[i];
+                if (kk < k_hi) gt[kk] = (guide_t)(e < maxu ? e : maxu);
+            }
+        }
+    }
+    if (last && lane == 0) gt[bins] = (guide_t)maxu;
+}
+
+template <bool CDF>
 MD TGBlock tg_variant(const TailGroupArgs& a, int G, int round, const double* v, unsigned ok4, double gmx, double gmn, int gkept,
                       bool gxnan, double* __restrict__ lp_out, double* __restrict__ gend_out, double* __restrict__ ggend_out,
-                      guide_t* __restrict__ guide_out, double* s_E TG_CLK_ARG) {
+                      guide_t* __restrict__ guide_out, double* s_E, bool raw_variant, const TGBlock* prev TG_CLK_ARG) {
     const int lane = threadIdx.x & 63, c = lane >> 2, k = lane & 3;
     const int blk = G >> 4, g = G & 15;
     const int64_t N = a.N, bbase = (int64_t)blk * SCAN_BLOCK, s0 = (int64_t)G * TG_GROUP + 4 * lane;
@@ -171,6 +234,18 @@
     }
     if (flags & 1u) { mx = NAN; mn = NAN; }
     const bool b_vnan = (flags & 2u) != 0, b_negw = (flags & 4u) != 0;
+    if (CDF && g == 0) {
+        const double bmx = prev ? prev->mx : mx, bmn = prev ? prev->mn : mn;
+        const bool last_round = raw_variant || !(__builtin_fabs(bmx - bmn) <= ISCLOSE_ATOL);
+        if (last_round) {
+            const bool bad = b_vnan || b_negw;
+            const uint64_t fl2 = raw_variant ? (uint64_t)((prev && (prev->vnan || prev->negw)) ? 1 : 0) | (uint64_t)(bad ? 2 : 0) : (uint64_t)(bad ? 1 : 0);
+            const double wsoft = raw_variant ? (prev ? prev->W : 0.0) : W, wraw = raw_variant ? W : 0.0;
+            const uint64_t v0 = lane == 0 ? (uint64_t)__double_as_longlong(wsoft) : lane == 1 ? (uint64_t)__double_as_longlong(wraw)
+                              : lane == 2 ? (uint64_t)__double_as_longlong(bmx) : lane == 3 ? (uint64_t)__double_as_longlong(bmn) : fl2;
+            if (lane < TG_VALUES) tg_store16(a.rec2 + (size_t)blk * TG_REC_WORDS + 2 * lane, v0, v0 ^ tg_key(a.tag, 2, lane));
+        }
+    }
     double out[4];
 #pragma unroll
     for (int j = 0; j < 4; ++j) out[j] = GP + (TP + L[j]);
@@ -257,9 +332,11 @@
     TG_CLK(7 + 6 * round);
     TGBlock r;
     r.W = W; r.Wa = Wa; r.mx = mx; r.mn = mn; r.kept = kept; r.vnan = b_vnan; r.late = late;
+    r.negw = b_negw; r.GP = GP; r.GPn = GPn; r.end = out[3];
     return r;
 }
 
+template <bool CDF>
 MD void tail_group_wave(const TailGroupArgs& a, int G, double* s_E) {
     const int lane = threadIdx.x & 63;
     const int blk = G >> 4, g = G & 15;
@@ -318,7 +395,7 @@
         }
     };
     const bool need_soft = a.softmax != 0;
-    TGBlock r0;
+    TGBlock r0, rs = {}, rr = {};
     bool close = false, late = false, nan = false;
     if (need_soft) {
         double e[4];
@@ -328,7 +405,8 @@
         store4(tb.e, e);
 #pragma unroll
         for (int j = 0; j < 4; ++j) e[j] = (in4 >> j) & 1u ? e[j] : 0.0;
-        r0 = tg_variant(a, G, 0, e, ok4, mx, mn, gkept, gxnan, tb.lp, tb.gend, tb.ggend, tb.guide, s_E TG_CLK_PASS);
+        r0 = tg_variant<CDF>(a, G, 0, e, ok4, mx, mn, gkept, gxnan, tb.lp, tb.gend, tb.ggend, CDF ? nullptr : tb.guide, s_E, false, nullptr TG_CLK_PASS);
+        rs = r0;
         close = __builtin_fabs(r0.mx - r0.mn) <= ISCLOSE_ATOL;
         late |= r0.late;
         nan = r0.vnan;
@@ -337,7 +415,9 @@
     const bool need_raw = !need_soft || close;
     if (need_raw) {
         store4(tb.x_raw, x);
-        const TGBlock r1 = tg_variant(a, G, need_soft ? 1 : 0, x, ok4, mx, mn, gkept, gxnan, tb.lp_raw, tb.gend_raw, tb.ggend_raw, tb.guide_raw, s_E TG_CLK_PASS);
+        const TGBlock r1 = tg_variant<CDF>(a, G, need_soft ? 1 : 0, x, ok4, mx, mn, gkept, gxnan, tb.lp_raw, tb.gend_raw, tb.ggend_raw,
+                                      CDF ? nullptr : tb.guide_raw, s_E, true, need_soft ? &rs : nullptr TG_CLK_PASS);
+        rr = r1;
         late |= r1.late;
         if (!need_soft) { r0 = r1; nan = r1.vnan; }
         if (g == 0 && lane == 0) tb.btot_raw[blk] = r1.W;
@@ -354,12 +434,54 @@
             if (r0.kept) atomicAdd(&a.flags_out[1], (double)r0.kept);
         }
     }
+    if constexpr (CDF) {
+        const int nb = (int)((N + SCAN_BLOCK - 1) >> 12), ngroups = (int)((N + TG_GROUP - 1) / TG_GROUP);
+        uint64_t w[2 * TG_VALUES];
+        {
+            const unsigned long long* rp = a.rec2 + (size_t)(lane < nb ? lane : 0) * TG_REC_WORDS;
+            const long long t0 = wall_clock64();
+            for (;;) {
+                tg_load80(rp, w);
+                bool ok = true;
+#pragma unroll
+                for (int i = 0; i < TG_VALUES; ++i) ok &= (w[2 * i] ^ w[2 * i + 1]) == tg_key(a.tag, 2, i);
+                if (__all((ok || lane >= nb) ? 1 : 0)) break;
+                if (wall_clock64() - t0 > TG_WAIT_TICKS) { late = true; break; }
+                __builtin_amdgcn_s_sleep(4);
+            }
+        }
+        TG_CLK(14);
+        const LazyFold f = lazy_fold_wave(nb, need_soft, __longlong_as_double((long long)w[0]), __longlong_as_double((long long)w[2]),
+                                          __longlong_as_double((long long)w[4]), __longlong_as_double((long long)w[6]), s_E);
+        if (G == 0 && !late) {
+            lazy_header_store(f, nb, false, a.hdr);
+            if (lane < nb) a.hdr[2 * LAZY_WAVE_LD + 4 + lane] = f.w;
+        }
+        const bool bad = __any((lane < nb && ((uint32_t)w[8] & (f.apply ? 1u : 2u))) ? 1 : 0) != 0;
+        const bool plain = !late && !bad && f.total > 0.0 && f.total < (double)INFINITY;
+        const TGBlock& rv = f.apply ? rs : rr;
+        const double BP = readlane_d(f.bp, blk);
+        constexpr int UPG = TG_GROUP / GUIDE_UNIT, UPC = SCAN_CHUNK / GUIDE_UNIT;
+        const int bins = guide_cdf_bins(nb);
+        const int64_t left_n = N - (int64_t)blk * SCAN_BLOCK;
+        const int nch = left_n >= SCAN_BLOCK ? SCAN_TPB : (int)((left_n + SCAN_CHUNK - 1) >> 4);
+        int nu = UPC * (nch - 16 * g);
+        nu = nu > UPG ? UPG : nu;
+        const unsigned maxu = plain ? (unsigned)(((N + SCAN_CHUNK - 1) >> 4) * UPC - 1) : 0xFFFFu;
+        tg_guide_fill(tb.guide, bins, plain, guide_cdf_width(f.total, bins), (double)bins * __builtin_amdgcn_rcp(f.total), BP + rv.GP, BP + rv.GPn,
+                      G == 0, G == ngroups - 1, G, ngroups, (unsigned)(blk * (SCAN_BLOCK / GUIDE_UNIT) + UPG * g), nu, maxu, BP + rv.end, s_E);
+        TG_CLK(15);
+    }
     if (late && lane == 0) atomicOr(&a.status[0], 16);
 #ifdef MIDAS_DEBUG_CLOCKS
     TG_SPAN(2 * G, tg_clk_[0]);
     TG_SPAN(2 * G + 1, wall_clock64());
     if (lane == 0 && (G == 0 || G == 200))
         for (int i = 0; i < 8; ++i) g_tg_clk[(G ? 24 : 8) + i] = tg_clk_[i];
+    if (lane == 0 && (G == 0 || G == 200) && CDF) {
+        g_tg_clk[(G ? 32 : 16)] = tg_clk_[14];
+        g_tg_clk[(G ? 32 : 16) + 1] = tg_clk_[15];
+    }
 #endif
 }
 
```

After: 27860. Within noise of the previous version (-0.6%).
